# matiasrodlo/arxiv-rag

Measured on AMD Instinct MI355X. Metric: chunks embedded/sec + QPS@top-10, all-mpnet-base-v2 768-d, 1/2/4/8 MI355X, higher is better.
Workload: dtype bf16

## Files before the change

arxiv_rag_amd/_lib.py:

```python
from __future__ import annotations

import ctypes as C
import os
from pathlib import Path

_HERE = Path(__file__).resolve().parent
LIB_PATH = Path(os.environ.get("ARX_LIB", _HERE / "libarx_hip.so"))

K_CLASSES = ["search_groupmax", "gemm_qkv", "gemm_oproj", "gemm_fc1", "gemm_fc2", "attention",
             "layernorm", "embed", "pool", "search_select", "search_rescore", "gemm_raw"]


class EncoderConfigC(C.Structure):
    _fields_ = [(n, C.c_int32) for n in ("arch", "vocab_size", "hidden", "layers", "heads", "ffn", "max_pos",
                                         "pool", "pad_id", "rel_buckets", "rel_max_distance")] + [("ln_eps", C.c_float)]


class LayerWeightsC(C.Structure):
    _fields_ = [(n, C.c_void_p) for n in ("w_qkv", "b_qkv", "w_o", "b_o", "ln1_g", "ln1_b",
                                          "w_fc1", "b_fc1", "w_fc2", "b_fc2", "ln2_g", "ln2_b")]


class EncoderWeightsC(C.Structure):
    _fields_ = [(n, C.c_void_p) for n in ("word_emb", "pos_emb", "type_emb", "emb_ln_g", "emb_ln_b", "rel_bias")] \
               + [("layers", C.POINTER(LayerWeightsC))]


class TopkOptionsC(C.Structure):
    _fields_ = [("struct_bytes", C.c_int32), ("i8_max_queries", C.c_int32), ("max_row_norm", C.c_float), ("cu_limit", C.c_int32),
                ("flags", C.c_int32), ("debug_tau_mult", C.c_float), ("debug_drop_best", C.c_int32)]

    def __init__(self, **kw):
        super().__init__(**kw)
        self.struct_bytes = C.sizeof(TopkOptionsC)


class EncoderOptionsC(C.Structure):
    _fields_ = [("struct_bytes", C.c_int32), ("gemm_schedule", C.c_int32), ("attn_kernel", C.c_int32), ("flags", C.c_int32)]

    def __init__(self, **kw):
        super().__init__(**kw)
        self.struct_bytes = C.sizeof(EncoderOptionsC)


class PairHeadC(C.Structure):
    _fields_ = [("struct_bytes", C.c_int32), ("n_labels", C.c_int32)] \
               + [(n, C.c_void_p) for n in ("type_emb", "pooler_w", "pooler_b", "cls_w", "cls_b")]

    def __init__(self, **kw):
        super().__init__(**kw)
        self.struct_bytes = C.sizeof(PairHeadC)


class GemmEpilogueC(C.Structure):
    _fields_ = [("struct_bytes", C.c_int32), ("mode", C.c_int32), ("variant", C.c_int32), ("eps", C.c_float)] \
               + [(n, C.c_void_p) for n in ("bias", "resid", "a_mean", "a_rstd", "s_vec", "r_mean", "r_rstd", "r_gamma", "r_beta")] \
               + [("row_cap", C.c_int64), ("part_sum", C.c_void_p), ("part_sq", C.c_void_p), ("part_ld", C.c_int64),
                  ("out_mean", C.c_void_p), ("out_rstd", C.c_void_p), ("n_rows", C.c_void_p)]

    def __init__(self, **kw):
        super().__init__(**kw)
        self.struct_bytes = C.sizeof(GemmEpilogueC)


TOPK_NO_PERSISTENT, TOPK_SCAN_ONLY, TOPK_TAIL_ONLY, TOPK_NO_SINGLE_ROW_TAIL, TOPK_I8_CENTRE_QUERY = 1, 2, 4, 8, 16
GEMM_DEFAULT, GEMM_PER_TILE, GEMM_PERSISTENT, GEMM_2STAGE, GEMM_SPLIT_K, GEMM_TILE_128 = 89, 8, 9, 13, 70, 71
ATTN_TRANSPOSED, ATTN_RING, ATTN_RING16, ATTN_STAGED = 1, 2, 4, 8
ENC_EXPLICIT_LAYERNORM = 1


EXPORTS = {
    "arx_version": (C.c_int32, []),
    "arx_last_error": (C.c_char_p, []),
    "arx_build_info": (C.c_int32, []),
    "arx_mpnet_bucket": (C.c_int32, [C.c_int32, C.c_int32, C.c_int32]),
    "arx_encoder_workspace_bytes": (C.c_int64, [C.POINTER(EncoderConfigC), C.c_int32, C.c_int32]),
    "arx_encoder_create": (C.c_int32, [C.POINTER(EncoderConfigC), C.POINTER(EncoderWeightsC), C.c_int32, C.c_int32,
                                       C.POINTER(C.c_void_p)]),
    "arx_encoder_create_opt": (C.c_int32, [C.POINTER(EncoderConfigC), C.POINTER(EncoderWeightsC), C.c_int32, C.c_int32,
                                           C.POINTER(EncoderOptionsC), C.POINTER(C.c_void_p)]),
    "arx_encoder_destroy": (None, [C.c_void_p]),
    "arx_encoder_forward": (C.c_int32, [C.c_void_p, C.c_void_p, C.c_int32, C.c_void_p, C.c_int32, C.c_int32, C.c_int32,
                                        C.c_void_p, C.c_int64, C.c_void_p, C.c_int64, C.c_int32, C.c_void_p]),
    "arx_encoder_attention": (C.c_int32, [C.c_void_p, C.c_void_p, C.c_void_p, C.c_int32, C.c_int32, C.c_void_p, C.c_void_p]),
    "arx_encoder_set_tap": (C.c_int32, [C.c_void_p, C.c_int32]),
    "arx_encoder_set_low_latency": (C.c_int32, [C.c_void_p, C.c_int32]),
    "arx_encoder_debug_hidden": (C.c_int32, [C.c_void_p, C.c_int32, C.c_void_p, C.c_int32, C.c_void_p]),
    "arx_encoder_set_pair_head": (C.c_int32, [C.c_void_p, C.POINTER(PairHeadC)]),
    "arx_encoder_score_pairs": (C.c_int32, [C.c_void_p, C.c_void_p, C.c_int32, C.c_void_p, C.c_void_p, C.c_int32, C.c_int32, C.c_int32,
                                            C.c_void_p, C.c_int64, C.c_void_p]),
    "arx_encoder_debug_cls": (C.c_int32, [C.c_void_p, C.c_void_p, C.c_int32, C.c_void_p]),
    "arx_pair_head_forward": (C.c_int32, [C.c_void_p, C.c_int64, C.c_int32, C.c_int32, C.POINTER(PairHeadC), C.c_void_p, C.c_int64,
                                          C.c_void_p]),
    "arx_topk_workspace_bytes": (C.c_int64, [C.c_int64, C.c_int32, C.c_int32, C.c_int32]),
    "arx_topk_search": (C.c_int32, [C.c_void_p, C.c_int64, C.c_void_p, C.c_int32, C.c_int32, C.c_int32, C.c_void_p,
                                    C.c_void_p, C.c_int64, C.c_void_p, C.c_int64, C.c_void_p]),
    "arx_topk_i8_index_bytes": (C.c_int64, [C.c_int64, C.c_int32]),
    "arx_topk_i8_index_info": (C.c_int32, [C.c_void_p, C.c_int64, C.c_int32, C.POINTER(C.c_float), C.c_void_p]),
    "arx_topk_build_i8": (C.c_int32, [C.c_void_p, C.c_int64, C.c_int32, C.c_void_p, C.c_void_p]),
    "arx_topk_search_i8": (C.c_int32, [C.c_void_p, C.c_void_p, C.c_int64, C.c_void_p, C.c_int32, C.c_int32, C.c_int32, C.c_void_p,
                                       C.c_void_p, C.c_int64, C.c_void_p, C.c_int64, C.c_void_p]),
    "arx_topk_workspace_bytes_i8": (C.c_int64, [C.c_int64, C.c_int32, C.c_int32, C.c_int32]),
    "arx_topk_search_opt": (C.c_int32, [C.c_void_p, C.c_void_p, C.c_int64, C.c_void_p, C.c_int32, C.c_int32, C.c_int32, C.c_void_p,
                                        C.c_void_p, C.c_int64, C.c_void_p, C.c_int64, C.POINTER(TopkOptionsC), C.c_void_p]),
    "arx_rows_max_norm_f16": (C.c_int32, [C.c_void_p, C.c_int64, C.c_int32, C.c_void_p, C.c_void_p]),
    "arx_stream_create_cu_mask": (C.c_int32, [C.POINTER(C.c_uint32), C.c_int32, C.POINTER(C.c_void_p)]),
    "arx_stream_destroy": (C.c_int32, [C.c_void_p]),
    "arx_device_cu_count": (C.c_int32, []),
    "arx_debug_cu_census": (C.c_int32, [C.c_void_p, C.c_int32, C.c_int32, C.c_void_p]),
    "arx_topk_stats": (C.c_int32, [C.c_void_p, C.POINTER(C.c_int64), C.POINTER(C.c_int64), C.c_void_p]),
    "arx_topk_merge": (C.c_int32, [C.c_void_p, C.c_void_p, C.c_int32, C.c_int32, C.c_int32, C.c_void_p, C.c_void_p,
                                   C.c_void_p]),
    "arx_topk_filtered_workspace_bytes": (C.c_int64, [C.c_int64, C.c_int32, C.c_int32, C.c_int32]),
    "arx_topk_search_filtered": (C.c_int32, [C.c_void_p, C.c_int64, C.c_void_p, C.c_int64, C.c_void_p, C.c_int32, C.c_int32, C.c_int32,
                                             C.c_void_p, C.c_void_p, C.c_int64, C.c_float, C.c_void_p, C.c_int64, C.c_void_p]),
    "arx_topk_search_filtered_tuned": (C.c_int32, [C.c_void_p, C.c_int64, C.c_void_p, C.c_int64, C.c_void_p, C.c_int32, C.c_int32, C.c_int32,
                                                   C.c_void_p, C.c_void_p, C.c_int64, C.c_float, C.c_void_p, C.c_int64, C.c_int32, C.c_int32,
                                                   C.c_void_p]),
    "arx_topk_filtered_stats": (C.c_int32, [C.c_void_p, C.POINTER(C.c_int64), C.POINTER(C.c_int64), C.c_void_p]),
    "arx_topk_filtered_multi_workspace_bytes": (C.c_int64, [C.c_int64, C.c_int32, C.c_int32, C.c_int32, C.c_int32]),
    "arx_topk_search_filtered_multi": (C.c_int32, [C.c_void_p, C.c_int64, C.c_void_p, C.c_int32, C.c_void_p, C.c_void_p, C.c_void_p, C.c_int32,
                                                   C.c_int32, C.c_int32, C.c_void_p, C.c_void_p, C.c_int64, C.c_float, C.c_void_p, C.c_int64,
                                                   C.c_void_p]),
    "arx_topk_search_filtered_multi_tuned": (C.c_int32, [C.c_void_p, C.c_int64, C.c_void_p, C.c_int32, C.c_void_p, C.c_void_p, C.c_void_p,
                                                         C.c_int32, C.c_int32, C.c_int32, C.c_void_p, C.c_void_p, C.c_int64, C.c_float,
                                                         C.c_void_p, C.c_int64, C.c_int32, C.c_int32, C.c_void_p]),
    "arx_topk_filtered_multi_stats": (C.c_int32, [C.c_void_p, C.POINTER(C.c_int64), C.POINTER(C.c_int64), C.c_void_p]),
    "arx_topk_prefix_workspace_bytes": (C.c_int64, [C.c_int64, C.c_int32, C.c_int32, C.c_int32]),
    "arx_topk_search_prefix": (C.c_int32, [C.c_void_p, C.c_int64, C.c_void_p, C.c_void_p, C.c_int32, C.c_int32, C.c_int32, C.c_void_p,
                                           C.c_void_p, C.c_int64, C.c_float, C.c_void_p, C.c_int64, C.c_void_p]),
    "arx_topk_search_prefix_tuned": (C.c_int32, [C.c_void_p, C.c_int64, C.c_void_p, C.c_void_p, C.c_int32, C.c_int32, C.c_int32, C.c_void_p,
                                                 C.c_void_p, C.c_int64, C.c_float, C.c_void_p, C.c_int64, C.c_int32, C.c_int32, C.c_void_p]),
    "arx_topk_prefix_stats": (C.c_int32, [C.c_void_p, C.POINTER(C.c_int64), C.POINTER(C.c_int64), C.c_void_p]),
    "arx_topk_grouped_workspace_bytes": (C.c_int64, [C.c_int64, C.c_int32, C.c_int32, C.c_int32, C.c_int32]),
    "arx_topk_search_grouped": (C.c_int32, [C.c_void_p, C.c_int64, C.c_void_p, C.c_int64, C.c_void_p, C.c_int64, C.c_void_p, C.c_int32,
                                            C.c_int32, C.c_int32, C.c_int32, C.c_void_p, C.c_void_p, C.c_void_p, C.c_int64, C.c_float,
                                            C.c_void_p, C.c_int64, C.c_void_p]),
    "arx_topk_search_grouped_tuned": (C.c_int32, [C.c_void_p, C.c_int64, C.c_void_p, C.c_int64, C.c_void_p, C.c_int64, C.c_void_p, C.c_int32,
                                                  C.c_int32, C.c_int32, C.c_int32, C.c_void_p, C.c_void_p, C.c_void_p, C.c_int64, C.c_float,
                                                  C.c_void_p, C.c_int64, C.c_int32, C.c_int32, C.c_void_p]),
    "arx_topk_grouped_stats": (C.c_int32, [C.c_void_p, C.POINTER(C.c_int64), C.POINTER(C.c_int64), C.c_void_p]),
    "arx_group_runs_info": (C.c_int32, [C.c_void_p, C.c_int64, C.c_void_p, C.c_void_p]),
    "arx_range_workspace_bytes": (C.c_int64, [C.c_int64, C.c_int32, C.c_int32, C.c_int32]),
    "arx_range_search": (C.c_int32, [C.c_void_p, C.c_int64, C.c_void_p, C.c_int64, C.c_void_p, C.c_void_p, C.c_int32, C.c_int32, C.c_int32,
                                     C.c_void_p, C.c_void_p, C.c_void_p, C.c_int64, C.c_float, C.c_void_p, C.c_int64, C.c_void_p]),
    "arx_range_search_tuned": (C.c_int32, [C.c_void_p, C.c_int64, C.c_void_p, C.c_int64, C.c_void_p, C.c_void_p, C.c_int32, C.c_int32,
                                           C.c_int32, C.c_void_p, C.c_void_p, C.c_void_p, C.c_int64, C.c_float, C.c_void_p, C.c_int64,
                                           C.c_int32, C.c_int32, C.c_void_p]),
    "arx_range_stats": (C.c_int32, [C.c_void_p, C.POINTER(C.c_int64), C.POINTER(C.c_int64), C.c_void_p]),
    "arx_text_contains":(C.c_int32, [C.c_void_p, C.c_void_p, C.c_int64, C.c_void_p, C.c_void_p, C.c_int32, C.c_void_p, C.c_void_p]),
    "arx_bitmap_count": (C.c_int32, [C.c_void_p, C.c_int64, C.c_void_p, C.c_void_p]),
# ... 92 lines not shown
```

arxiv_rag_amd/csrc/arx_common.h:

```cpp
#pragma once
#include <hip/hip_runtime.h>
#include <stdint.h>
#include <stdio.h>
#include <string>

#include "../../include/arx.h"

typedef __bf16 bf16_t;
typedef _Float16 f16_t;
typedef __bf16 bf16x8 __attribute__((ext_vector_type(8)));
typedef __bf16 bf16x4 __attribute__((ext_vector_type(4)));
typedef _Float16 f16x8 __attribute__((ext_vector_type(8)));
typedef float f32x4 __attribute__((ext_vector_type(4)));
typedef float f32x16 __attribute__((ext_vector_type(16)));
typedef uint32_t u32x4 __attribute__((ext_vector_type(4)));
typedef uint32_t u32x2 __attribute__((ext_vector_type(2)));

void arx_set_error(const char* fmt, ...);
int arx_prof_begin(int cls, hipStream_t st);
void arx_prof_end(int cls, int token, hipStream_t st);
hipError_t arx_func_smem(const void* kernel, int bytes);
int arx_device_cus();
struct ProfScope {
    int cls, tok; hipStream_t st;
    ProfScope(int c, hipStream_t s) : cls(c), tok(arx_prof_begin(c, s)), st(s) {}
    ~ProfScope() { arx_prof_end(cls, tok, st); }
};

#define ARX_HIP_CHECK(expr)                                                              \
    do {                                                                                 \
        hipError_t _e = (expr);                                                          \
        if (_e != hipSuccess) {                                                          \
            arx_set_error("%s:%d: %s -> %s", __FILE__, __LINE__, #expr, hipGetErrorString(_e)); \
            return ARX_ERR_HIP;                                                          \
        }                                                                                \
    } while (0)

#define ARX_REQUIRE(cond, ...)                \
    do {                                      \
        if (!(cond)) {                        \
            arx_set_error(__VA_ARGS__);       \
            return ARX_ERR_ARG;               \
        }                                     \
    } while (0)

static inline int64_t round_up64(int64_t x, int64_t m) { return (x + m - 1) / m * m; }
static inline int cdiv(int64_t a, int64_t b) { return (int)((a + b - 1) / b); }

__device__ __forceinline__ float bf16_bits_to_f32(uint16_t b) { return __uint_as_float(((uint32_t)b) << 16); }

typedef __bf16 bf16x2 __attribute__((ext_vector_type(2)));
typedef float f32x2 __attribute__((ext_vector_type(2)));
__device__ __forceinline__ uint32_t pack_bf16x2(float lo, float hi) {
    const f32x2 f = {lo, hi};
    return __builtin_bit_cast(uint32_t, __builtin_convertvector(f, bf16x2));
}

__device__ __forceinline__ void unpack_bf16x2(uint32_t v, float& lo, float& hi) {
    lo = __uint_as_float(v << 16);
    hi = __uint_as_float(v & 0xffff0000u);
}

__device__ __forceinline__ float wave_sum(float v) {
#pragma unroll
    for (int o = 32; o > 0; o >>= 1) v += __shfl_xor(v, o);
    return v;
}
__device__ __forceinline__ float wave_max(float v) {
#pragma unroll
    for (int o = 32; o > 0; o >>= 1) v = fmaxf(v, __shfl_xor(v, o));
    return v;
}

__device__ __forceinline__ int xcd_remap(int bid, int nwg) {
    const int q = nwg >> 3, r = nwg & 7, xcd = bid & 7, idx = bid >> 3;
    const int base = (xcd < r) ? xcd * (q + 1) : r * (q + 1) + (xcd - r) * q;
    return base + idx;
}
```

arxiv_rag_amd/csrc/encoder.hip:

```cpp
#include <math.h>
#include <stdlib.h>
#include <string.h>

#include <mutex>
#include <vector>

#include "arx_common.h"
#include "encoder_kernels.h"
#include "gemm.h"
#include "gemm8.h"
#include "gemm_small.h"

extern "C" int32_t arx_mpnet_bucket(int32_t rel, int32_t num_buckets, int32_t max_distance) {
    int n = -rel;
    const int nb = num_buckets / 2;
    int ret = 0;
    if (n < 0) { ret = nb; n = -n; }
    const int max_exact = nb / 2;
    if (n < max_exact) return ret + n;
    int v = max_exact + (int)floor(log((double)n / max_exact) / log((double)max_distance / max_exact) * (nb - max_exact) + 1e-6);
    if (v > nb - 1) v = nb - 1;
    return ret + v;
}

struct arx_encoder {
    arx_encoder_config cfg;
    arx_encoder_weights w;
    std::vector<arx_layer_weights> layers;
    int max_tokens, max_seqs, tok_pad;
    char* ws = nullptr;
    int64_t ws_bytes = 0;
    int32_t* cu = nullptr;
    uint16_t *x = nullptr, *x1 = nullptr, *qkv = nullptr, *ctx = nullptr, *y = nullptr, *hbuf = nullptr;
    float* bias_tbl = nullptr;
    uint16_t* tap = nullptr;
    int tap_layer = -1;
    int ln_fold = 1;
    char* fold_ws = nullptr;
    std::vector<uint16_t*> wqkv_f, wfc1_f;
    std::vector<float*> s_qkv, c_qkv, s_fc1, c_fc1;
    float *st1_sum = nullptr, *st1_sq = nullptr, *st2_sum = nullptr, *st2_sq = nullptr;
    float *part_s = nullptr, *part_q = nullptr;
    int variant = ARX_GEMM_DEFAULT;
    int low_latency = 0;
    float* small_ws = nullptr;
    int attn_variant = ARX_ATTN_TRANSPOSED;
    int attn_dev_word = 0;
    unsigned long long* attn_stamps = nullptr;
    arx_pair_head pair{};
    int has_pair = 0;
    float* cls_ws = nullptr;
};

struct WsLayout {
    int64_t cu, x, x1, qkv, ctx, y, hbuf, bias, stats, total;
};
static WsLayout ws_layout(const arx_encoder_config& c, int max_tokens, int max_seqs) {
    const int64_t tp = round_up64(max_tokens, 256);
    WsLayout l;
    int64_t o = 0;
    auto take = [&](int64_t bytes) { int64_t r = o; o += round_up64(bytes, 256); return r; };
    l.cu = take((int64_t)(max_seqs + 1) * 4);
    l.x = take(tp * c.hidden * 2);
    l.x1 = take(tp * c.hidden * 2);
    l.qkv = take(tp * c.hidden * 3 * 2);
    l.ctx = take(tp * c.hidden * 2);
    l.y = take(tp * c.hidden * 2);
    l.hbuf = take(tp * c.ffn * 2);
    l.bias = take((int64_t)c.heads * ARX_BIAS_ROW * 4);
    l.stats = take(tp * 4 * 4 + 2 * (int64_t)(c.hidden / 64) * tp * 4);
    l.total = o;
    return l;
}

static int check_cfg(const arx_encoder_config* c) {
    ARX_REQUIRE(c != nullptr, "cfg is null");
    ARX_REQUIRE(c->arch == ARX_ARCH_MPNET || c->arch == ARX_ARCH_BERT, "unknown arch %d", c->arch);
    ARX_REQUIRE(c->hidden > 0 && c->hidden % 64 == 0 && c->hidden <= 1024, "hidden=%d must be a multiple of 64, <= 1024", c->hidden);
    ARX_REQUIRE(c->heads > 0 && c->hidden % c->heads == 0, "hidden %% heads != 0");
    const int dh = c->hidden / c->heads;
    ARX_REQUIRE(dh == 32 || dh == 64, "head_dim=%d unsupported (32 or 64)", dh);
    ARX_REQUIRE(c->ffn > 0 && c->ffn % 64 == 0, "ffn=%d must be a multiple of 64", c->ffn);
    ARX_REQUIRE(c->layers > 0 && c->vocab_size > 0 && c->max_pos > 0, "bad layers/vocab/max_pos");
    ARX_REQUIRE(c->pool == ARX_POOL_MEAN || c->pool == ARX_POOL_CLS, "unknown pool %d", c->pool);
    return ARX_OK;
}

extern "C" int64_t arx_encoder_workspace_bytes(const arx_encoder_config* cfg, int32_t max_tokens, int32_t max_seqs) {
    if (check_cfg(cfg) != ARX_OK || max_tokens <= 0 || max_seqs <= 0) return -1;
    return ws_layout(*cfg, max_tokens, max_seqs).total;
}

static int check_options(const arx_encoder_options* o) {
    if (!o) return ARX_OK;
    ARX_REQUIRE(o->struct_bytes == (int32_t)sizeof(arx_encoder_options), "arx_encoder_options: struct_bytes=%d, this library expects %d",
                o->struct_bytes, (int)sizeof(arx_encoder_options));
    const int g = o->gemm_schedule, a = o->attn_kernel;
    bool gemm_ok = g == 0 || g == ARX_GEMM_DEFAULT || g == ARX_GEMM_PER_TILE || g == ARX_GEMM_PERSISTENT || g == ARX_GEMM_2STAGE || g == ARX_GEMM_TILE_128;
    bool attn_ok = a == 0 || a == ARX_ATTN_TRANSPOSED || a == ARX_ATTN_STAGED;
#ifdef ARX_DEV_VARIANTS
    gemm_ok = gemm_ok || g == 1 || g == 2 || g == 3 || g == 4 || g == 15 || g == 33 || g == 34;
    attn_ok = attn_ok || a == ARX_ATTN_RING || a == ARX_ATTN_RING16;
#endif
    ARX_REQUIRE(gemm_ok, "arx_encoder_options.gemm_schedule=%d is not a whole-forward GEMM schedule of this build (ARX_GEMM_* in arx.h)", g);
    ARX_REQUIRE(attn_ok, "arx_encoder_options.attn_kernel=%d is not an attention kernel of this build (ARX_ATTN_* in arx.h)", a);
    ARX_REQUIRE((o->flags & ~ARX_ENC_EXPLICIT_LAYERNORM) == 0, "arx_encoder_options.flags=0x%x has unknown bits", o->flags);
    return ARX_OK;
}

extern "C" int32_t arx_encoder_create(const arx_encoder_config* cfg, const arx_encoder_weights* w, int32_t max_tokens,
                                      int32_t max_seqs, arx_encoder** out) {
    return arx_encoder_create_opt(cfg, w, max_tokens, max_seqs, nullptr, out);
}

extern "C" int32_t arx_encoder_create_opt(const arx_encoder_config* cfg, const arx_encoder_weights* w, int32_t max_tokens,
                                          int32_t max_seqs, const arx_encoder_options* opt, arx_encoder** out) {
    int rc = check_cfg(cfg);
    if (rc != ARX_OK) return rc;
    if ((rc = check_options(opt)) != ARX_OK) return rc;
    ARX_REQUIRE(w && out, "null weights/out");
    ARX_REQUIRE(max_tokens > 0 && max_seqs > 0, "max_tokens/max_seqs must be positive");
    ARX_REQUIRE(w->word_emb && w->pos_emb && w->emb_ln_g && w->emb_ln_b && w->layers, "missing embedding weights");
    ARX_REQUIRE(cfg->arch != ARX_ARCH_BERT || w->type_emb, "BERT needs type_emb");
    ARX_REQUIRE(cfg->arch != ARX_ARCH_MPNET || w->rel_bias, "MPNet needs rel_bias");
    for (int i = 0; i < cfg->layers; ++i) {
        const arx_layer_weights& L = w->layers[i];
        ARX_REQUIRE(L.w_qkv && L.b_qkv && L.w_o && L.b_o && L.ln1_g && L.ln1_b && L.w_fc1 && L.b_fc1 && L.w_fc2 &&
                        L.b_fc2 && L.ln2_g && L.ln2_b, "layer %d: missing weights", i);
    }
    arx_encoder* h = new arx_encoder();
    auto fail = [&](int code) {
        if (h->ws) (void)hipFree(h->ws);
        if (h->fold_ws) (void)hipFree(h->fold_ws);
        delete h;
        return code;
    };
    h->cfg = *cfg;
    h->w = *w;
    h->layers.assign(w->layers, w->layers + cfg->layers);
    h->w.layers = h->layers.data();
    h->max_tokens = max_tokens;
    h->max_seqs = max_seqs;
    h->tok_pad = (int)round_up64(max_tokens, 256);
    if (opt && opt->gemm_schedule) h->variant = opt->gemm_schedule;
    if (opt && opt->attn_kernel) h->attn_variant = opt->attn_kernel;
    h->ln_fold = !(opt && (opt->flags & ARX_ENC_EXPLICIT_LAYERNORM));
    const WsLayout l = ws_layout(*cfg, max_tokens, max_seqs);
    hipError_t he = hipMalloc((void**)&h->ws, l.total);
    if (he != hipSuccess) {
        arx_set_error("hipMalloc(%lld bytes workspace): %s", (long long)l.total, hipGetErrorString(he));
        h->ws = nullptr;
        return fail(ARX_ERR_HIP);
    }
    h->ws_bytes = l.total;
    (void)hipMemset(h->ws, 0, l.total);
    h->cu = (int32_t*)(h->ws + l.cu);
    h->x = (uint16_t*)(h->ws + l.x);
    h->x1 = (uint16_t*)(h->ws + l.x1);
    h->qkv = (uint16_t*)(h->ws + l.qkv);
    h->ctx = (uint16_t*)(h->ws + l.ctx);
    h->y = (uint16_t*)(h->ws + l.y);
    h->hbuf = (uint16_t*)(h->ws + l.hbuf);
    h->bias_tbl = (float*)(h->ws + l.bias);
    {
        const int64_t tp = round_up64(max_tokens, 256);
        float* st = (float*)(h->ws + l.stats);
        h->st1_sum = st; h->st1_sq = st + tp; h->st2_sum = st + 2 * tp; h->st2_sq = st + 3 * tp;
        h->part_s = st + 4 * tp; h->part_q = h->part_s + (int64_t)(cfg->hidden / 64) * tp;
    }
    if (h->ln_fold) {
        const int64_t H = cfg->hidden, F = cfg->ffn, Lc = cfg->layers;
        const int64_t per = round_up64(3 * H * H * 2, 256) + round_up64(F * H * 2, 256) + 2 * round_up64(3 * H * 4, 256) + 2 * round_up64(F * 4, 256);
        he = hipMalloc((void**)&h->fold_ws, per * Lc);
        if (he != hipSuccess) {
            arx_set_error("hipMalloc(folded weights): %s", hipGetErrorString(he));
            h->fold_ws = nullptr;
            return fail(ARX_ERR_HIP);
        }
        char* pws = h->fold_ws;
        auto takep = [&](int64_t bytes) { char* r = pws; pws += round_up64(bytes, 256); return r; };
        for (int i = 0; i < Lc; ++i) {
            const arx_layer_weights& L = h->layers[i];
            uint16_t* wq = (uint16_t*)takep(3 * H * H * 2); uint16_t* w1 = (uint16_t*)takep(F * H * 2);
            float* sq = (float*)takep(3 * H * 4); float* cq = (float*)takep(3 * H * 4);
            float* s1 = (float*)takep(F * 4); float* c1 = (float*)takep(F * 4);
            h->wqkv_f.push_back(wq); h->wfc1_f.push_back(w1);
            h->s_qkv.push_back(sq); h->c_qkv.push_back(cq); h->s_fc1.push_back(s1); h->c_fc1.push_back(c1);
            fold_ln_kernel<<<cdiv(F, 4), 256>>>((const uint16_t*)L.w_fc1, L.ln1_g, L.ln1_b, L.b_fc1, w1, s1, c1, (int)F, (int)H);
            if (i > 0) {
                const arx_layer_weights& P = h->layers[i - 1];
                fold_ln_kernel<<<cdiv(3 * H, 4), 256>>>((const uint16_t*)L.w_qkv, P.ln2_g, P.ln2_b, L.b_qkv, wq, sq, cq, (int)(3 * H), (int)H);
            }
        }
        he = hipDeviceSynchronize();
        if (he != hipSuccess) {
            arx_set_error("fold_ln_kernel: %s", hipGetErrorString(he));
            return fail(ARX_ERR_HIP);
        }
    }
    if (cfg->arch == ARX_ARCH_MPNET) {
        std::vector<float> rb((size_t)cfg->rel_buckets * cfg->heads);
        he = hipMemcpy(rb.data(), w->rel_bias, rb.size() * 4, hipMemcpyDeviceToHost);
        if (he != hipSuccess) {
            arx_set_error("copy rel_bias: %s", hipGetErrorString(he));
            return fail(ARX_ERR_HIP);
        }
        std::vector<float> tbl((size_t)cfg->heads * ARX_BIAS_ROW);
        const float log2e = 1.4426950408889634f;
        for (int d = -ARX_BIAS_CENTER; d <= ARX_BIAS_CENTER; ++d) {
            const int bk = arx_mpnet_bucket(d, cfg->rel_buckets, cfg->rel_max_distance);
            for (int hd = 0; hd < cfg->heads; ++hd)
                tbl[(size_t)hd * ARX_BIAS_ROW + d + ARX_BIAS_CENTER] = rb[(size_t)bk * cfg->heads + hd] * log2e;
        }
        he = hipMemcpy(h->bias_tbl, tbl.data(), tbl.size() * 4, hipMemcpyHostToDevice);
        if (he != hipSuccess) {
            arx_set_error("upload bias table: %s", hipGetErrorString(he));
            return fail(ARX_ERR_HIP);
        }
    }
    *out = h;
    return ARX_OK;
}

extern "C" void arx_encoder_destroy(arx_encoder* h) {
    if (!h) return;
    if (h->ws) (void)hipFree(h->ws);
    if (h->tap) (void)hipFree(h->tap);
    if (h->fold_ws) (void)hipFree(h->fold_ws);
    if (h->small_ws) (void)hipFree(h->small_ws);
    if (h->cls_ws) (void)hipFree(h->cls_ws);
    delete h;
}

extern "C" int32_t arx_encoder_set_low_latency(arx_encoder* h, int32_t on) {
    ARX_REQUIRE(h, "null handle");
    if (on && !h->small_ws) ARX_HIP_CHECK(hipMalloc((void**)&h->small_ws, ARX_SMALL_WS_BYTES));
    h->low_latency = on ? 1 : 0;
    return ARX_OK;
}

extern "C" int32_t arx_encoder_set_tap(arx_encoder* h, int32_t layer) {
    ARX_REQUIRE(h, "null handle");
    ARX_REQUIRE(layer >= -1 && layer <= h->cfg.layers, "tap layer out of range");
    if (layer >= 0 && !h->tap) ARX_HIP_CHECK(hipMalloc((void**)&h->tap, (int64_t)h->tok_pad * h->cfg.hidden * 2));
    h->tap_layer = layer;
    return ARX_OK;
}

extern "C" int32_t arx_encoder_debug_hidden(arx_encoder* h, int32_t , float* dst, int32_t n_tokens, void* stream) {
    ARX_REQUIRE(h && h->tap && dst, "no tap recorded");
    ARX_REQUIRE(n_tokens > 0 && n_tokens <= h->max_tokens, "n_tokens out of range");
    const int64_t n = (int64_t)n_tokens * h->cfg.hidden;
    bf16_to_f32_kernel<<<cdiv(n, 256), 256, 0, (hipStream_t)stream>>>(h->tap, dst, n);
    ARX_HIP_CHECK(hipGetLastError());
    return ARX_OK;
}

template <typename Kern>
static int launch_gemm_kernel(Kern kern, int smem, int threads, int BM, int BN, const uint16_t* A, int64_t lda,
                              const uint16_t* W, int64_t ldw, int M, int N, int K, const EpiParams& ep, hipStream_t st) {
    ARX_HIP_CHECK(arx_func_smem((const void*)kern, smem));
    const int tm = cdiv(M, BM), tn = cdiv(N, BN);
    kern<<<tm * tn, threads, smem, st>>>((const bf16_t*)A, lda, (const bf16_t*)W, ldw, M, N, K, tm, tn, ep);
    ARX_HIP_CHECK(hipGetLastError());
    return ARX_OK;
}

static bool fits_u32_offsets(int64_t M, int64_t lda, int64_t N, int64_t ldw, const EpiParams& ep) {
    return M * lda < (1ll << 31) && N * ldw < (1ll << 31) && M * ep.ldc < (1ll << 32) && (!ep.resid || M * ep.ldr < (1ll << 32));
}

template <int MODE>
int arx_launch_gemm(int variant, const uint16_t* A, int64_t lda, const uint16_t* W, int64_t ldw, int M, int N, int K,
                    const EpiParams& ep, hipStream_t st) {
    if (K % 64 != 0 || N % 8 != 0) {
        arx_set_error("gemm: K=%d must be a multiple of 64 and N=%d of 8", K, N);
        return ARX_ERR_ARG;
    }
    const bool wide = (N % 256 == 0);
    const bool wide8 = (N % 128 == 0 && N >= 256);
#ifdef ARX_DEV_VARIANTS
    if constexpr (MODE <= EPI_BIAS_RESID) {
        if (variant == 0) {
            if (wide) return launch_gemm_kernel(gemm_bf16_kernel<256, 256, 2, 4, true, MODE>, GemmMainloop<bf16_t, 256, 256, 2, 4, true>::SMEM_BYTES, 512, 256, 256, A, lda, W, ldw, M, N, K, ep, st);
            return launch_gemm_kernel(gemm_bf16_kernel<256, 128, 4, 2, true, MODE>, GemmMainloop<bf16_t, 256, 128, 4, 2, true>::SMEM_BYTES, 512, 256, 128, A, lda, W, ldw, M, N, K, ep, st);
        }
        if (variant == 4) {
            if (wide) return launch_gemm_kernel(gemm_bf16_kernel<256, 256, 2, 4, false, MODE>, GemmMainloop<bf16_t, 256, 256, 2, 4, false>::SMEM_BYTES, 512, 256, 256, A, lda, W, ldw, M, N, K, ep, st);
            return launch_gemm_kernel(gemm_bf16_kernel<256, 128, 4, 2, false, MODE>, GemmMainloop<bf16_t, 256, 128, 4, 2, false>::SMEM_BYTES, 512, 256, 128, A, lda, W, ldw, M, N, K, ep, st);
        }
    }
#endif
    if (variant == ARX_GEMM_TILE_128)
        return launch_gemm_kernel(gemm_v0e2_kernel<128, 128, 2, 2, MODE, 67>, GemmMainloop<bf16_t, 128, 128, 2, 2, true, 67>::SMEM_BYTES, 256, 128, 128, A, lda, W, ldw, M, N, K, ep, st);
    if (variant == ARX_GEMM_DEFAULT) variant = (K <= 1024) ? ARX_GEMM_PERSISTENT : ARX_GEMM_PER_TILE;
    if (variant == ARX_GEMM_PERSISTENT && (K / 64) % 2 != 0) variant = ARX_GEMM_PER_TILE;
    if ((variant == ARX_GEMM_PER_TILE || variant == ARX_GEMM_PERSISTENT) && wide8 && !fits_u32_offsets(M, lda, N, ldw, ep)) {
        static bool said = false;
        if (!said) {
            said = true;
            fprintf(stderr, "[arx] gemm M=%d N=%d K=%d: operand or output offsets exceed 32 bits, using the 2-stage kernel (64-bit offsets)\n", M, N, K);
        }
        variant = ARX_GEMM_2STAGE;
    }
    if (variant == ARX_GEMM_PERSISTENT && wide8) {
        auto kern = gemm_8phase_persistent_kernel<MODE>;
        ARX_HIP_CHECK(arx_func_smem((const void*)kern, Gemm8Phase<bf16_t, 0>::SMEM_BYTES));
        const int n_cu = arx_device_cus();
        const int tm = cdiv(M, 256), tn = cdiv(N, 256);
        int grid = TileWalk::grid(tm, tn) < n_cu ? TileWalk::grid(tm, tn) : n_cu;
        grid = grid / 8 * 8 > 0 ? grid / 8 * 8 : grid;
        kern<<<grid, 512, Gemm8Phase<bf16_t, 0>::SMEM_BYTES, st>>>((const bf16_t*)A, lda, (const bf16_t*)W, ldw, M, N, K, tm, tn, ep);
        ARX_HIP_CHECK(hipGetLastError());
        return ARX_OK;
    }
    if (variant == ARX_GEMM_PER_TILE && wide8) {
        auto kern = gemm_8phase_kernel<MODE>;
        ARX_HIP_CHECK(arx_func_smem((const void*)kern, Gemm8Phase<bf16_t, 0>::SMEM_BYTES));
        const int tm = cdiv(M, 256), tn = cdiv(N, 256);
        kern<<<TileWalk::grid(tm, tn), 512, Gemm8Phase<bf16_t, 0>::SMEM_BYTES, st>>>((const bf16_t*)A, lda, (const bf16_t*)W, ldw, M, N, K, tm, tn, ep);
        ARX_HIP_CHECK(hipGetLastError());
        return ARX_OK;
    }
#ifdef ARX_DEV_VARIANTS
    if (variant == 34 && wide)
        return launch_gemm_kernel(gemm_v0e2_kernel<256, 256, 2, 4, MODE, 64 + 4096>, GemmMainloop<bf16_t, 256, 256, 2, 4, true, 64 + 4096>::SMEM_BYTES, 512, 256, 256, A, lda, W, ldw, M, N, K, ep, st);
    if (variant == 33 && wide)
        return launch_gemm_kernel(gemm_a3w2_kernel<256, 256, 2, 4, MODE>, 3 * 256 * 128 + 2 * 256 * 128, 512, 256, 256, A, lda, W, ldw, M, N, K, ep, st);
    if (variant == 1) {
        if (wide) return launch_gemm_kernel(gemm_v0e2_kernel<256, 256, 2, 4, MODE>, GemmMainloop<bf16_t, 256, 256, 2, 4, true>::SMEM_BYTES, 512, 256, 256, A, lda, W, ldw, M, N, K, ep, st);
        return launch_gemm_kernel(gemm_v0e2_kernel<256, 128, 4, 2, MODE>, GemmMainloop<bf16_t, 256, 128, 4, 2, true>::SMEM_BYTES, 512, 256, 128, A, lda, W, ldw, M, N, K, ep, st);
    }
    if (variant == 15 && wide)
        return launch_gemm_kernel(gemm_v0e2_kernel<256, 256, 2, 4, MODE, 3>, GemmMainloop<bf16_t, 256, 256, 2, 4, true, 3>::SMEM_BYTES, 512, 256, 256, A, lda, W, ldw, M, N, K, ep, st);
    if (variant == 3 && wide)
        return launch_gemm_kernel(gemm_ring_kernel<256, 256, 2, 4, 4, MODE>, GemmRing<bf16_t, 256, 256, 2, 4, 4>::SMEM_BYTES, 512, 256, 256, A, lda, W, ldw, M, N, K, ep, st);
    if (variant == 2 || variant == 3)
        return launch_gemm_kernel(gemm_ring_kernel<256, 128, 2, 2, 3, MODE>, GemmRing<bf16_t, 256, 128, 2, 2, 3>::SMEM_BYTES, 256, 256, 128, A, lda, W, ldw, M, N, K, ep, st);
#endif
    if (!wide) return launch_gemm_kernel(gemm_v0e2_kernel<256, 128, 4, 2, MODE, 67>, GemmMainloop<bf16_t, 256, 128, 4, 2, true, 67>::SMEM_BYTES, 512, 256, 128, A, lda, W, ldw, M, N, K, ep, st);
    return launch_gemm_kernel(gemm_v0e2_kernel<256, 256, 2, 4, MODE, 67>, GemmMainloop<bf16_t, 256, 256, 2, 4, true, 67>::SMEM_BYTES, 512, 256, 256, A, lda, W, ldw, M, N, K, ep, st);
}

template <int MODE>
static int launch_gemm(int cls, int variant, const uint16_t* A, int64_t lda, const uint16_t* W, int64_t ldw, int M, int N, int K,
                       const EpiParams& ep, hipStream_t st, float* small_ws = nullptr) {
    ProfScope ps(cls, st);
    if (variant == ARX_GEMM_SPLIT_K) return launch_gemm_small<MODE>(A, lda, W, ldw, M, N, K, ep, small_ws, st);
#ifdef ARX_DEV_VARIANTS
    static const int dev_bw = getenv("ARX_DEV_BW") ? atoi(getenv("ARX_DEV_BW")) : 0;
    const char* stg = getenv("ARX_DEV_STAGGER");
    if (dev_bw || stg) {
        EpiParams e2 = ep; e2.dev_bw = dev_bw;
        if (stg) { int a = 0, b = 8, c = 0; sscanf(stg, "%d,%d,%d", &a, &b, &c); e2.dev_stagger = a; e2.dev_slots = b > 0 ? b : 8; e2.dev_store = c; }
        return arx_launch_gemm<MODE>(variant, A, lda, W, ldw, M, N, K, e2, st);
    }
#endif
    return arx_launch_gemm<MODE>(variant, A, lda, W, ldw, M, N, K, ep, st);
}

extern "C" int32_t arx_gemm_bf16(const void* A, const void* W, const float* bias, const void* resid, void* C, int32_t M,
                                 int32_t N, int32_t K, int32_t mode, int32_t variant, void* stream) {
    ARX_REQUIRE(A && W && bias && C, "null pointer argument");
    ARX_REQUIRE(M > 0 && N > 0 && K > 0, "bad sizes");
    ARX_REQUIRE(mode != EPI_BIAS_RESID || resid, "mode 2 needs resid");
    EpiParams ep{(uint16_t*)C, N, bias, (const uint16_t*)resid, N};
    hipStream_t st = (hipStream_t)stream;
#ifdef ARX_DEV_VARIANTS
    ep.dev_store = (variant / 100) % 10; ep.dev_bw = variant / 1000; variant %= 100;
    if (const char* stg = getenv("ARX_DEV_STAGGER")) { int a = 0, b = 8; sscanf(stg, "%d,%d", &a, &b); ep.dev_stagger = a; ep.dev_slots = b > 0 ? b : 8; }
#endif
#ifdef ARX_STAMP
    {
        static unsigned long long* d = nullptr;
        const int tiles = cdiv(M, 256) * cdiv(N, 256);
        if (!d) ARX_HIP_CHECK(hipMalloc(&d, (size_t)8 * 32 * 2 * 16384));
        if (getenv("ARX_STAMP_DUMP") && tiles <= 16384) {
            ep.stamps = d;
            int rc = ARX_ERR_ARG;
            if (mode == EPI_BIAS) rc = arx_launch_gemm<EPI_BIAS>(variant, (const uint16_t*)A, K, (const uint16_t*)W, K, M, N, K, ep, st);
            if (mode == EPI_BIAS_GELU) rc = arx_launch_gemm<EPI_BIAS_GELU>(variant, (const uint16_t*)A, K, (const uint16_t*)W, K, M, N, K, ep, st);
            if (mode == EPI_BIAS_RESID) rc = arx_launch_gemm<EPI_BIAS_RESID>(variant, (const uint16_t*)A, K, (const uint16_t*)W, K, M, N, K, ep, st);
            ARX_HIP_CHECK(hipStreamSynchronize(st));
            std::vector<unsigned long long> hbuf((size_t)tiles * 64);
            ARX_HIP_CHECK(hipMemcpy(hbuf.data(), d, hbuf.size() * 8, hipMemcpyDeviceToHost));
            double loop[2] = {0, 0}, epi[2] = {0, 0}, pro[2] = {0, 0}, x45[2] = {0, 0}, x67[2] = {0, 0};
            unsigned long long tmin = ~0ull, tmax = 0;
            for (int t = 0; t < tiles; ++t)
                for (int g = 0; g < 2; ++g) {
                    const unsigned long long* o = &hbuf[((size_t)t * 2 + g) * 32];
                    loop[g] += (double)(o[1] - o[3]); epi[g] += (double)(o[2] - o[1]); pro[g] += (double)(o[3] - o[0]);
                    if (variant == 9) { x45[g] += (double)(o[5] - o[4]); x67[g] += (double)(o[7] - o[6]); }
                    else x45[g] += (double)(o[4] - o[2]);
                    tmin = o[0] < tmin ? o[0] : tmin; tmax = o[2] > tmax ? o[2] : tmax;
                }
            if (variant == 9) {
                double gap = 0, period = 0; int n = 0;
                for (int t = 0; t + 256 < tiles; ++t) { const unsigned long long* a = &hbuf[(size_t)t * 64]; const unsigned long long* b = &hbuf[(size_t)(t + 256) * 64];
                    gap += (double)(b[0] - a[2]); period += (double)(b[0] - a[0]); ++n; }
                if (n) fprintf(stderr, "[stamp] persistent: g0 tile period %.0f clk, epilogue-end -> next loop start %.0f clk\n", period / n, gap / n);
            }
            if (const char* sf = getenv("ARX_STAMP_FILE")) {
                if (FILE* f = fopen(sf, "wb")) { fwrite(hbuf.data(), 8, hbuf.size(), f); fclose(f); }
// ... 63 lines not shown
    return ARX_OK;
}

#ifdef ARX_DEV_VARIANTS
template <int DH, bool HB, int NSLOT>
static int launch_attn_ring_cfg(arx_encoder* h, int n_seqs, int max_len, hipStream_t st) {
    auto kern = attention_ring_kernel<DH, HB, NSLOT>;
    const int C0 = (max_len + 31) & ~31;
    const int smem = AttnRing<DH, NSLOT>::total(C0, HB);
    ARX_HIP_CHECK(arx_func_smem((const void*)kern, smem));
    int G = arx_device_cus() / h->cfg.heads;
    G = G < 1 ? 1 : (G > n_seqs ? n_seqs : G);
    const float scale_log2e = 1.4426950408889634f / sqrtf((float)DH);
    ProfScope ps(ARX_K_ATTENTION, st);
    kern<<<G * h->cfg.heads, 512, smem, st>>>(h->qkv, h->ctx, h->cu, h->bias_tbl, h->cfg.hidden, n_seqs, C0, scale_log2e);
    ARX_HIP_CHECK(hipGetLastError());
    return ARX_OK;
}

template <bool HB>
static int launch_attn_ring16_cfg(arx_encoder* h, int n_seqs, int max_len, hipStream_t st) {
    auto kern = attention_ring16_kernel<HB>;
    const int C0 = (max_len + 31) & ~31;
    const int smem = AttnRing16<8>::total(C0, HB);
    ARX_HIP_CHECK(arx_func_smem((const void*)kern, smem));
    int G = arx_device_cus() / h->cfg.heads;
    G = G < 1 ? 1 : (G > n_seqs ? n_seqs : G);
    const float scale_log2e = 1.4426950408889634f / sqrtf(64.0f);
    ProfScope ps(ARX_K_ATTENTION, st);
    kern<<<G * h->cfg.heads, 1024, smem, st>>>(h->qkv, h->ctx, h->cu, h->bias_tbl, h->cfg.hidden, n_seqs, C0, scale_log2e);
    ARX_HIP_CHECK(hipGetLastError());
    return ARX_OK;
}

#endif

static int launch_attn(arx_encoder* h, int n_seqs, int max_len, hipStream_t st) {
    const int dh = h->cfg.hidden / h->cfg.heads;
    const bool hb = h->cfg.arch == ARX_ARCH_MPNET;
#ifdef ARX_DEV_VARIANTS
    if (h->attn_variant == ARX_ATTN_RING16 && dh == 64 && max_len > 128 && max_len <= 256)
        return hb ? launch_attn_ring16_cfg<true>(h, n_seqs, max_len, st) : launch_attn_ring16_cfg<false>(h, n_seqs, max_len, st);
    if (h->attn_variant == ARX_ATTN_RING && max_len > 128 && max_len <= 256) {
        if (dh == 64) return hb ? launch_attn_ring_cfg<64, true, 8>(h, n_seqs, max_len, st) : launch_attn_ring_cfg<64, false, 8>(h, n_seqs, max_len, st);
        return hb ? launch_attn_ring_cfg<32, true, 8>(h, n_seqs, max_len, st) : launch_attn_ring_cfg<32, false, 8>(h, n_seqs, max_len, st);
    }
#endif
    if (h->attn_variant != ARX_ATTN_STAGED) {
        const bool w8 = max_len > 128;
        if (dh == 64) {
            if (hb) return w8 ? launch_attn_tr_cfg<64, true, 8>(h, n_seqs, max_len, st) : launch_attn_tr_cfg<64, true, 4>(h, n_seqs, max_len, st);
            return w8 ? launch_attn_tr_cfg<64, false, 8>(h, n_seqs, max_len, st) : launch_attn_tr_cfg<64, false, 4>(h, n_seqs, max_len, st);
        }
        if (hb) return w8 ? launch_attn_tr_cfg<32, true, 8>(h, n_seqs, max_len, st) : launch_attn_tr_cfg<32, true, 4>(h, n_seqs, max_len, st);
        return w8 ? launch_attn_tr_cfg<32, false, 8>(h, n_seqs, max_len, st) : launch_attn_tr_cfg<32, false, 4>(h, n_seqs, max_len, st);
    }
    const bool big = max_len > 256;
    if (dh == 64) {
        if (hb) return big ? launch_attn_cfg<64, true, 8>(h, n_seqs, max_len, st) : launch_attn_cfg<64, true, 4>(h, n_seqs, max_len, st);
        return big ? launch_attn_cfg<64, false, 8>(h, n_seqs, max_len, st) : launch_attn_cfg<64, false, 4>(h, n_seqs, max_len, st);
    }
    if (hb) return big ? launch_attn_cfg<32, true, 8>(h, n_seqs, max_len, st) : launch_attn_cfg<32, true, 4>(h, n_seqs, max_len, st);
    return big ? launch_attn_cfg<32, false, 8>(h, n_seqs, max_len, st) : launch_attn_cfg<32, false, 4>(h, n_seqs, max_len, st);
}

extern "C" int32_t arx_encoder_attention(arx_encoder* h, const void* qkv, const int32_t* lens, int32_t n_seqs, int32_t max_len,
                                         void* ctx, void* stream) {
    ARX_REQUIRE(h && qkv && lens && ctx, "null pointer argument");
    ARX_REQUIRE(n_seqs > 0 && n_seqs <= h->max_seqs && max_len > 0 && max_len <= 512, "bad n_seqs/max_len");
    hipStream_t st = (hipStream_t)stream;
    scan_lens_kernel<<<1, 256, 0, st>>>(lens, h->cu, n_seqs);
    ARX_HIP_CHECK(hipGetLastError());
    uint16_t* q0 = h->qkv; uint16_t* c0 = h->ctx;
    h->qkv = (uint16_t*)qkv; h->ctx = (uint16_t*)ctx;
    const int rc = launch_attn(h, n_seqs, max_len, st);
    h->qkv = q0; h->ctx = c0;
    return rc;
}

static void launch_ln_finalize(int T, int nparts, const float* ps, const float* pq, int64_t ld, const int32_t* n_rows, float inv_h,
                               float eps, float* mean, float* rstd, hipStream_t st) {
    const int grid = cdiv(T, 256);
    switch (nparts) {
    case 6: ln_finalize_kernel<6><<<grid, 256, 0, st>>>(ps, pq, ld, nparts, n_rows, inv_h, eps, mean, rstd); break;
    case 12: ln_finalize_kernel<12><<<grid, 256, 0, st>>>(ps, pq, ld, nparts, n_rows, inv_h, eps, mean, rstd); break;
    case 16: ln_finalize_kernel<16><<<grid, 256, 0, st>>>(ps, pq, ld, nparts, n_rows, inv_h, eps, mean, rstd); break;
    default: ln_finalize_kernel<0><<<grid, 256, 0, st>>>(ps, pq, ld, nparts, n_rows, inv_h, eps, mean, rstd); break;
    }
}

template <int MODE>
static int gemm_ex_run(int variant, const uint16_t* A, const uint16_t* W, int M, int N, int K, const EpiParams& ep, const arx_gemm_epilogue* e,
                       hipStream_t st) {
    constexpr bool STATS = (MODE == EPI_RESID_STATS || MODE == EPI_LNRESID_STATS);
    int rc;
    if (variant == ARX_GEMM_SPLIT_K) {
        float* ws = nullptr;
        ARX_HIP_CHECK(hipMallocAsync((void**)&ws, ARX_SMALL_WS_BYTES, st));
        rc = launch_gemm<MODE>(ARX_K_GEMM_RAW, variant, A, K, W, K, M, N, K, ep, st, ws);
        (void)hipFreeAsync(ws, st);
        return rc;
    }
    if ((rc = launch_gemm<MODE>(ARX_K_GEMM_RAW, variant, A, K, W, K, M, N, K, ep, st)) != ARX_OK) return rc;
    if (STATS) {
        launch_ln_finalize(M, N / 64, e->part_sum, e->part_sq, e->part_ld, e->n_rows, ep.inv_h, ep.eps, e->out_mean, e->out_rstd, st);
        ARX_HIP_CHECK(hipGetLastError());
    }
    return ARX_OK;
}

extern "C" int32_t arx_gemm_bf16_ex(const void* A, const void* W, void* C, int32_t M, int32_t N, int32_t K, const arx_gemm_epilogue* e,
                                    void* stream) {
    ARX_REQUIRE(A && W && C && e, "null pointer argument");
    ARX_REQUIRE(e->struct_bytes == (int32_t)sizeof(arx_gemm_epilogue), "arx_gemm_epilogue: struct_bytes=%d, this library expects %d",
                e->struct_bytes, (int)sizeof(arx_gemm_epilogue));
    ARX_REQUIRE(M > 0 && N > 0 && K > 0, "bad sizes");
    ARX_REQUIRE(K % 64 == 0 && N % 8 == 0, "gemm: K=%d must be a multiple of 64 and N=%d of 8", K, N);
    const int mode = e->mode, variant = e->variant;
    ARX_REQUIRE(mode >= EPI_BIAS && mode <= EPI_LNRESID_STATS, "unknown gemm mode %d", mode);
    ARX_REQUIRE(variant == ARX_GEMM_DEFAULT || variant == ARX_GEMM_PER_TILE || variant == ARX_GEMM_PERSISTENT || variant == ARX_GEMM_2STAGE ||
                    variant == ARX_GEMM_SPLIT_K || variant == ARX_GEMM_TILE_128,
                "gemm variant %d is not a shipped schedule (89, 8, 9, 13, 70, 71)", variant);
    const bool ln_in = (mode == EPI_LN_BIAS || mode == EPI_LN_BIAS_GELU), stats = (mode == EPI_RESID_STATS || mode == EPI_LNRESID_STATS);
    const bool staged = (variant == ARX_GEMM_DEFAULT || variant == ARX_GEMM_PER_TILE || variant == ARX_GEMM_PERSISTENT);
    ARX_REQUIRE(e->bias, "mode %d needs bias", mode);
    ARX_REQUIRE(!(mode == EPI_BIAS_RESID || stats) || e->resid, "mode %d needs resid", mode);
    ARX_REQUIRE(!ln_in || (e->a_mean && e->a_rstd && e->s_vec), "mode %d needs a_mean, a_rstd and s_vec", mode);
    ARX_REQUIRE(mode != EPI_LNRESID_STATS || (e->r_mean && e->r_rstd && e->r_gamma && e->r_beta), "mode 6 needs r_mean, r_rstd, r_gamma and r_beta");
    if (ln_in || mode == EPI_LNRESID_STATS)
        ARX_REQUIRE(e->row_cap >= (staged ? round_up64(M, 256) : (int64_t)M),
                    "row_cap=%lld: the row vectors must be readable up to row %lld (M=%d%s)", (long long)e->row_cap,
                    (long long)(staged ? round_up64(M, 256) : (int64_t)M), M, staged ? " rounded up to 256: variants 89, 8, 9 stage whole tiles" : "");
    if (stats) {
        ARX_REQUIRE(N % 64 == 0, "statistics modes need N %% 64 == 0 (one partial per 64-column slice), N=%d", N);
        ARX_REQUIRE(e->out_mean && e->out_rstd, "mode %d needs out_mean and out_rstd", mode);
        if (variant != ARX_GEMM_SPLIT_K) ARX_REQUIRE(e->part_sum && e->part_sq && e->part_ld >= M && e->n_rows,
                                       "mode %d on a tile kernel needs part_sum, part_sq, part_ld >= M and n_rows", mode);
    }
    if (variant == ARX_GEMM_SPLIT_K) {
        ARX_REQUIRE(M <= ARX_SMALL_M && N % 64 == 0, "small-batch gemm: M=%d (<= %d) N=%d (%% 64)", M, ARX_SMALL_M, N);
        ARX_REQUIRE(!stats || N <= 1024, "small-batch gemm: statistics modes take N <= 1024, N=%d", N);
    }
    EpiParams ep{(uint16_t*)C, N, e->bias, (const uint16_t*)e->resid, N};
    ep.a_sum = e->a_mean; ep.a_sq = e->a_rstd; ep.s_vec = e->s_vec;
    ep.r_sum = e->r_mean; ep.r_sq = e->r_rstd; ep.r_gamma = e->r_gamma; ep.r_beta = e->r_beta;
    ep.o_sum = e->part_sum; ep.o_sq = e->part_sq; ep.o_ld = e->part_ld;
    ep.fin_mean = e->out_mean; ep.fin_rstd = e->out_rstd;
    ep.inv_h = 1.0f / (float)N; ep.eps = e->eps;
    hipStream_t st = (hipStream_t)stream;
    const uint16_t* a = (const uint16_t*)A; const uint16_t* w = (const uint16_t*)W;
    switch (mode) {
    case EPI_BIAS: return gemm_ex_run<EPI_BIAS>(variant, a, w, M, N, K, ep, e, st);
    case EPI_BIAS_GELU: return gemm_ex_run<EPI_BIAS_GELU>(variant, a, w, M, N, K, ep, e, st);
    case EPI_BIAS_RESID: return gemm_ex_run<EPI_BIAS_RESID>(variant, a, w, M, N, K, ep, e, st);
    case EPI_LN_BIAS: return gemm_ex_run<EPI_LN_BIAS>(variant, a, w, M, N, K, ep, e, st);
    case EPI_LN_BIAS_GELU: return gemm_ex_run<EPI_LN_BIAS_GELU>(variant, a, w, M, N, K, ep, e, st);
    case EPI_RESID_STATS: return gemm_ex_run<EPI_RESID_STATS>(variant, a, w, M, N, K, ep, e, st);
    default: return gemm_ex_run<EPI_LNRESID_STATS>(variant, a, w, M, N, K, ep, e, st);
    }
}

extern "C" int32_t arx_fold_ln(const void* W, const float* gamma, const float* beta, const float* bias, void* Wf, float* s, float* c,
                               int32_t N, int32_t K, void* stream) {
    ARX_REQUIRE(W && gamma && beta && bias && Wf && s && c, "null pointer argument");
    ARX_REQUIRE(N > 0 && K > 0, "bad sizes");
    fold_ln_kernel<<<cdiv(N, 4), 256, 0, (hipStream_t)stream>>>((const uint16_t*)W, gamma, beta, bias, (uint16_t*)Wf, s, c, (int)N, (int)K);
    ARX_HIP_CHECK(hipGetLastError());
    return ARX_OK;
}

static int32_t encoder_run(arx_encoder* h, const int32_t* ids, int32_t seq_stride, const int32_t* lens, const int32_t* seg_b,
                           int32_t n_seqs, int32_t max_len, int32_t total_tokens, float* out_f32,
                           int64_t out_stride, void* out_f16, int64_t out16_stride, int32_t normalize,
                           void* stream) {
    ARX_REQUIRE(h && ids && lens, "null handle/ids/lens");
    ARX_REQUIRE(out_f32 || out_f16, "no output buffer");
    ARX_REQUIRE(n_seqs > 0 && max_len > 0 && max_len <= 512, "n_seqs=%d max_len=%d (max_len must be in 1..512)", n_seqs, max_len);
    ARX_REQUIRE(seq_stride >= max_len, "seq_stride < max_len");
    ARX_REQUIRE(total_tokens > 0 && (int64_t)total_tokens <= (int64_t)n_seqs * max_len, "total_tokens out of range");
    if (n_seqs > h->max_seqs || total_tokens > h->max_tokens) {
        arx_set_error("batch (%d seqs, %d tokens) exceeds handle capacity (%d, %d)", n_seqs, total_tokens, h->max_seqs, h->max_tokens);
        return ARX_ERR_CAPACITY;
    }
    ARX_REQUIRE(!out_f32 || out_stride >= h->cfg.hidden, "out_stride < hidden");
    ARX_REQUIRE(!out_f16 || out16_stride >= h->cfg.hidden, "out16_stride < hidden");
    hipStream_t st = (hipStream_t)stream;
    const arx_encoder_config& c = h->cfg;
    const int H = c.hidden, F = c.ffn, T = total_tokens;
    int rc;

    scan_lens_kernel<<<1, 256, 0, st>>>(lens, h->cu, n_seqs);
    ARX_HIP_CHECK(hipGetLastError());
    {
        ProfScope ps(ARX_K_EMBED, st);
        dim3 grid(cdiv(max_len, 4), n_seqs);
        if (c.arch == ARX_ARCH_MPNET)
            embed_ln_kernel<ARX_ARCH_MPNET><<<grid, 256, 0, st>>>(ids, seq_stride, lens, h->cu, h->w.word_emb, h->w.pos_emb, nullptr,
                                                                  h->w.emb_ln_g, h->w.emb_ln_b, h->x, H, c.vocab_size, c.max_pos, c.pad_id, c.ln_eps);
        else if (seg_b)
            embed_ln_kernel<ARX_ARCH_BERT, true><<<grid, 256, 0, st>>>(ids, seq_stride, lens, h->cu, h->w.word_emb, h->w.pos_emb,
                                                                       h->pair.type_emb, h->w.emb_ln_g, h->w.emb_ln_b, h->x, H,
                                                                       c.vocab_size, c.max_pos, c.pad_id, c.ln_eps, seg_b);
        else
            embed_ln_kernel<ARX_ARCH_BERT><<<grid, 256, 0, st>>>(ids, seq_stride, lens, h->cu, h->w.word_emb, h->w.pos_emb, h->w.type_emb,
                                                                 h->w.emb_ln_g, h->w.emb_ln_b, h->x, H, c.vocab_size, c.max_pos, c.pad_id, c.ln_eps);
        ARX_HIP_CHECK(hipGetLastError());
    }
    const int ln_grid = cdiv(T, 4);
    const int64_t tp = round_up64(h->max_tokens, 256);
    if (!h->ln_fold) {
        auto tap = [&](int layer) -> int {
            if (h->tap_layer == layer && h->tap) ARX_HIP_CHECK(hipMemcpyAsync(h->tap, h->x, (int64_t)T * H * 2, hipMemcpyDeviceToDevice, st));
            return ARX_OK;
        };
        if ((rc = tap(0)) != ARX_OK) return rc;
        for (int li = 0; li < c.layers; ++li) {
            const arx_layer_weights& L = h->layers[li];
            EpiParams ep;
            ep = EpiParams{h->qkv, 3 * (int64_t)H, L.b_qkv, nullptr, 0};
            if ((rc = launch_gemm<EPI_BIAS>(ARX_K_GEMM_QKV, h->variant, h->x, H, (const uint16_t*)L.w_qkv, H, T, 3 * H, H, ep, st)) != ARX_OK) return rc;
            if ((rc = launch_attn(h, n_seqs, max_len, st)) != ARX_OK) return rc;
            ep = EpiParams{h->y, H, L.b_o, h->x, H};
            if ((rc = launch_gemm<EPI_BIAS_RESID>(ARX_K_GEMM_OPROJ, h->variant, h->ctx, H, (const uint16_t*)L.w_o, H, T, H, H, ep, st)) != ARX_OK) return rc;
            { ProfScope ps(ARX_K_LAYERNORM, st);
              layernorm_kernel<<<ln_grid, 256, 0, st>>>(h->y, h->x1, L.ln1_g, L.ln1_b, h->cu + n_seqs, H, c.ln_eps); }
            ARX_HIP_CHECK(hipGetLastError());
            ep = EpiParams{h->hbuf, F, L.b_fc1, nullptr, 0};
            if ((rc = launch_gemm<EPI_BIAS_GELU>(ARX_K_GEMM_FC1, h->variant, h->x1, H, (const uint16_t*)L.w_fc1, H, T, F, H, ep, st)) != ARX_OK) return rc;
            ep = EpiParams{h->y, H, L.b_fc2, h->x1, H};
            if ((rc = launch_gemm<EPI_BIAS_RESID>(ARX_K_GEMM_FC2, h->variant, h->hbuf, F, (const uint16_t*)L.w_fc2, F, T, H, F, ep, st)) != ARX_OK) return rc;
            { ProfScope ps(ARX_K_LAYERNORM, st);
              layernorm_kernel<<<ln_grid, 256, 0, st>>>(h->y, h->x, L.ln2_g, L.ln2_b, h->cu + n_seqs, H, c.ln_eps); }
            ARX_HIP_CHECK(hipGetLastError());
            if ((rc = tap(li + 1)) != ARX_OK) return rc;
        }
        ProfScope pps(ARX_K_POOL, st);
        pool_norm_kernel<<<n_seqs, 256, 0, st>>>(h->x, h->cu, H, c.pool, normalize, out_f32, out_stride, (f16_t*)out_f16, out16_stride,
                                                 nullptr, nullptr, nullptr, nullptr, 0.f);
        ARX_HIP_CHECK(hipGetLastError());
        return ARX_OK;
    }

    const float inv_h = 1.0f / (float)H;
    const int gv = !h->low_latency ? h->variant : (T <= ARX_SMALL_M ? ARX_GEMM_SPLIT_K : (T <= ARX_MEDIUM_M ? ARX_GEMM_TILE_128 : h->variant));
    if (h->tap_layer == 0 && h->tap) ARX_HIP_CHECK(hipMemcpyAsync(h->tap, h->x, (int64_t)T * H * 2, hipMemcpyDeviceToDevice, st));
    for (int li = 0; li < c.layers; ++li) {
        const arx_layer_weights& L = h->layers[li];
        EpiParams ep;
        if (li == 0) {
            ep = EpiParams{h->qkv, 3 * (int64_t)H, L.b_qkv, nullptr, 0};
            if ((rc = launch_gemm<EPI_BIAS>(ARX_K_GEMM_QKV, gv, h->x, H, (const uint16_t*)L.w_qkv, H, T, 3 * H, H, ep, st, h->small_ws)) != ARX_OK) return rc;
        } else {
            ep = EpiParams{h->qkv, 3 * (int64_t)H, h->c_qkv[li], nullptr, 0};
            ep.a_sum = h->st2_sum; ep.a_sq = h->st2_sq; ep.s_vec = h->s_qkv[li]; ep.inv_h = inv_h; ep.eps = c.ln_eps;
            if ((rc = launch_gemm<EPI_LN_BIAS>(ARX_K_GEMM_QKV, gv, h->x, H, h->wqkv_f[li], H, T, 3 * H, H, ep, st, h->small_ws)) != ARX_OK) return rc;
        }
        if ((rc = launch_attn(h, n_seqs, max_len, st)) != ARX_OK) return rc;
        ep = EpiParams{h->x1, H, L.b_o, h->x, H};
        ep.o_sum = h->part_s; ep.o_sq = h->part_q; ep.o_ld = tp; ep.inv_h = inv_h; ep.eps = c.ln_eps;
        ep.fin_mean = h->st1_sum; ep.fin_rstd = h->st1_sq;
        if (li == 0) {
            if ((rc = launch_gemm<EPI_RESID_STATS>(ARX_K_GEMM_OPROJ, gv, h->ctx, H, (const uint16_t*)L.w_o, H, T, H, H, ep, st, h->small_ws)) != ARX_OK) return rc;
        } else {
            const arx_layer_weights& P = h->layers[li - 1];
            ep.r_sum = h->st2_sum; ep.r_sq = h->st2_sq; ep.r_gamma = P.ln2_g; ep.r_beta = P.ln2_b;
            if ((rc = launch_gemm<EPI_LNRESID_STATS>(ARX_K_GEMM_OPROJ, gv, h->ctx, H, (const uint16_t*)L.w_o, H, T, H, H, ep, st, h->small_ws)) != ARX_OK) return rc;
        }
        if (gv != ARX_GEMM_SPLIT_K) { ProfScope ps(ARX_K_LAYERNORM, st);
          launch_ln_finalize(T, H / 64, h->part_s, h->part_q, tp, h->cu + n_seqs, inv_h, c.ln_eps, h->st1_sum, h->st1_sq, st); }
        ARX_HIP_CHECK(hipGetLastError());
        ep = EpiParams{h->hbuf, F, h->c_fc1[li], nullptr, 0};
        ep.a_sum = h->st1_sum; ep.a_sq = h->st1_sq; ep.s_vec = h->s_fc1[li]; ep.inv_h = inv_h; ep.eps = c.ln_eps;
        if ((rc = launch_gemm<EPI_LN_BIAS_GELU>(ARX_K_GEMM_FC1, gv, h->x1, H, h->wfc1_f[li], H, T, F, H, ep, st, h->small_ws)) != ARX_OK) return rc;
        ep = EpiParams{h->x, H, L.b_fc2, h->x1, H};
        ep.r_sum = h->st1_sum; ep.r_sq = h->st1_sq; ep.r_gamma = L.ln1_g; ep.r_beta = L.ln1_b;
        ep.o_sum = h->part_s; ep.o_sq = h->part_q; ep.o_ld = tp; ep.inv_h = inv_h; ep.eps = c.ln_eps;
        ep.fin_mean = h->st2_sum; ep.fin_rstd = h->st2_sq;
        if ((rc = launch_gemm<EPI_LNRESID_STATS>(ARX_K_GEMM_FC2, gv, h->hbuf, F, (const uint16_t*)L.w_fc2, F, T, H, F, ep, st, h->small_ws)) != ARX_OK) return rc;
        if (gv != ARX_GEMM_SPLIT_K) { ProfScope ps(ARX_K_LAYERNORM, st);
          launch_ln_finalize(T, H / 64, h->part_s, h->part_q, tp, h->cu + n_seqs, inv_h, c.ln_eps, h->st2_sum, h->st2_sq, st); }
        ARX_HIP_CHECK(hipGetLastError());
        if (h->tap_layer == li + 1 && h->tap) {
            layernorm_kernel<<<ln_grid, 256, 0, st>>>(h->x, h->tap, L.ln2_g, L.ln2_b, h->cu + n_seqs, H, c.ln_eps);
            ARX_HIP_CHECK(hipGetLastError());
        }
    }
    {
        const arx_layer_weights& Ll = h->layers[c.layers - 1];
        ProfScope pps(ARX_K_POOL, st);
        pool_norm_kernel<<<n_seqs, 256, 0, st>>>(h->x, h->cu, H, c.pool, normalize, out_f32, out_stride, (f16_t*)out_f16, out16_stride,
                                                 h->st2_sum, h->st2_sq, Ll.ln2_g, Ll.ln2_b, c.ln_eps);
        ARX_HIP_CHECK(hipGetLastError());
    }
    return ARX_OK;
}

extern "C" int32_t arx_encoder_forward(arx_encoder* h, const int32_t* ids, int32_t seq_stride, const int32_t* lens,
                                       int32_t n_seqs, int32_t max_len, int32_t total_tokens, float* out_f32,
                                       int64_t out_stride, void* out_f16, int64_t out16_stride, int32_t normalize,
                                       void* stream) {
    return encoder_run(h, ids, seq_stride, lens, nullptr, n_seqs, max_len, total_tokens, out_f32, out_stride, out_f16, out16_stride,
                       normalize, stream);
}

static int check_pair_head(const arx_pair_head* p, int hidden) {
    ARX_REQUIRE(p, "null pair head");
    ARX_REQUIRE(p->struct_bytes >= (int32_t)sizeof(arx_pair_head), "arx_pair_head.struct_bytes=%d < %d", p->struct_bytes,
                (int)sizeof(arx_pair_head));
    ARX_REQUIRE(p->n_labels >= 1 && p->n_labels <= 16, "n_labels=%d must be in 1..16", p->n_labels);
    ARX_REQUIRE(p->pooler_w && p->pooler_b && p->cls_w && p->cls_b, "pair head: missing pooler / classifier weights");
    ARX_REQUIRE(hidden > 0 && hidden <= 1024, "hidden=%d must be in 1..1024", hidden);
    return ARX_OK;
}

static int launch_pair_head(const float* cls, int64_t ld, int n, int H, const arx_pair_head& p, float* out, int64_t ld_out,
                            hipStream_t st) {
    const int smem = 2 * PH_ROWS * H * (int)sizeof(float);
    ARX_HIP_CHECK(arx_func_smem((const void*)pair_head_kernel, smem));
    pair_head_kernel<<<cdiv(n, PH_ROWS), 256, smem, st>>>(cls, ld, n, H, p.pooler_w, p.pooler_b, p.cls_w, p.cls_b, p.n_labels, out,
                                                            ld_out);
    ARX_HIP_CHECK(hipGetLastError());
    return ARX_OK;
}

extern "C" int32_t arx_encoder_set_pair_head(arx_encoder* h, const arx_pair_head* head) {
    ARX_REQUIRE(h, "null handle");
    ARX_REQUIRE(h->cfg.arch == ARX_ARCH_BERT && h->cfg.pool == ARX_POOL_CLS, "a pair head needs a BERT handle with CLS pooling");
    const int rc = check_pair_head(head, h->cfg.hidden);
    if (rc != ARX_OK) return rc;
    ARX_REQUIRE(head->type_emb, "pair head: missing token-type table");
    if (!h->cls_ws) ARX_HIP_CHECK(hipMalloc((void**)&h->cls_ws, (int64_t)h->max_seqs * h->cfg.hidden * sizeof(float)));
    h->pair = *head;
    h->has_pair = 1;
    return ARX_OK;
}

extern "C" int32_t arx_encoder_score_pairs(arx_encoder* h, const int32_t* ids, int32_t seq_stride, const int32_t* lens,
                                           const int32_t* seg_b, int32_t n_seqs, int32_t max_len, int32_t total_tokens,
                                           float* out_logits, int64_t out_stride, void* stream) {
    ARX_REQUIRE(h && out_logits, "null handle/out_logits");
    ARX_REQUIRE(h->has_pair, "no pair head set (arx_encoder_set_pair_head)");
    ARX_REQUIRE(out_stride >= h->pair.n_labels, "out_stride < n_labels");
    int rc = encoder_run(h, ids, seq_stride, lens, seg_b, n_seqs, max_len, total_tokens, h->cls_ws, h->cfg.hidden, nullptr, 0, 0,
                         stream);
    if (rc != ARX_OK) return rc;
    return launch_pair_head(h->cls_ws, h->cfg.hidden, n_seqs, h->cfg.hidden, h->pair, out_logits, out_stride, (hipStream_t)stream);
}

extern "C" int32_t arx_encoder_debug_cls(arx_encoder* h, float* dst, int32_t n, void* stream) {
    ARX_REQUIRE(h && h->cls_ws && dst, "no pair head set / null dst");
    ARX_REQUIRE(n > 0 && n <= h->max_seqs, "n out of range");
    ARX_HIP_CHECK(hipMemcpyAsync(dst, h->cls_ws, (int64_t)n * h->cfg.hidden * sizeof(float), hipMemcpyDeviceToDevice, (hipStream_t)stream));
    return ARX_OK;
}

extern "C" int32_t arx_pair_head_forward(const float* cls_rows, int64_t ld, int32_t n, int32_t hidden, const arx_pair_head* head,
                                         float* out_logits, int64_t out_stride, void* stream) {
    const int rc = check_pair_head(head, hidden);
    if (rc != ARX_OK) return rc;
    ARX_REQUIRE(n >= 0 && ld >= hidden && out_stride >= head->n_labels, "bad n / ld / out_stride");
    if (n == 0) return ARX_OK;
    ARX_REQUIRE(cls_rows && out_logits, "null cls_rows/out_logits");
    return launch_pair_head(cls_rows, ld, n, hidden, *head, out_logits, out_stride, (hipStream_t)stream);
// ... 35 lines not shown
```

arxiv_rag_amd/csrc/encoder_kernels.h:

```cpp
#pragma once
#include <type_traits>

#include "arx_common.h"

__global__ void scan_lens_kernel(const int32_t* __restrict__ lens, int32_t* __restrict__ cu, int n) {
    __shared__ int32_t part[1024];
    const int tid = threadIdx.x, nt = blockDim.x;
    const int per = (n + nt - 1) / nt;
    const int b0 = tid * per, b1 = min(n, b0 + per);
    int s = 0;
    for (int b = b0; b < b1; ++b) s += lens[b];
    part[tid] = s;
    __syncthreads();
    if (tid == 0) {
        int run = 0;
        for (int i = 0; i < nt; ++i) { int v = part[i]; part[i] = run; run += v; }
        cu[n] = run;
    }
    __syncthreads();
    int run = part[tid];
    for (int b = b0; b < b1; ++b) { cu[b] = run; run += lens[b]; }
}

template <int ARCH, bool SEG = false>
// ... 1206 lines not shown
    }
}

#endif

__global__ __launch_bounds__(256) void pool_norm_kernel(const uint16_t* __restrict__ x, const int32_t* __restrict__ cu,
                                                         int H, int pool_mode, int normalize,
                                                         float* __restrict__ out32, int64_t ld32,
                                                         f16_t* __restrict__ out16, int64_t ld16,
                                                         const float* __restrict__ ln_sum, const float* __restrict__ ln_sq,
                                                         const float* __restrict__ ln_g, const float* __restrict__ ln_b, float eps) {
    __shared__ float acc_s[4][1024];
    __shared__ float red[4];
    const int b = blockIdx.x, tid = threadIdx.x, lane = tid & 63, w = tid >> 6;
    const int t0 = cu[b], L = cu[b + 1] - t0;
    const int nch = H >> 3;
    float a[2][8];
#pragma unroll
    for (int c = 0; c < 2; ++c)
#pragma unroll
        for (int e = 0; e < 8; ++e) a[c][e] = 0.f;
    const int nrows = (pool_mode == ARX_POOL_CLS) ? (L > 0 ? 1 : 0) : L;
    for (int r = w; r < nrows; r += 4) {
        const uint16_t* in = x + (int64_t)(t0 + r) * H;
        float mu = 0.f, rs = 1.f;
        if (ln_sum) { mu = ln_sum[t0 + r]; rs = ln_sq[t0 + r]; }
#pragma unroll
        for (int c = 0; c < 2; ++c) {
            const int ch = lane + 64 * c;
            if (ch < nch) {
                const u32x4 q = *reinterpret_cast<const u32x4*>(in + ch * 8);
#pragma unroll
                for (int e = 0; e < 4; ++e) {
                    float lo, hi;
                    unpack_bf16x2(q[e], lo, hi);
                    a[c][2 * e] += (lo - mu) * rs; a[c][2 * e + 1] += (hi - mu) * rs;
                }
            }
        }
    }
#pragma unroll
    for (int c = 0; c < 2; ++c) {
        const int ch = lane + 64 * c;
        if (ch < nch)
#pragma unroll
            for (int e = 0; e < 8; ++e) acc_s[w][ch * 8 + e] = a[c][e];
    }
    __syncthreads();
    float v[4];
    float sq = 0.f;
    const float denom = (pool_mode == ARX_POOL_CLS) ? 1.0f : fmaxf((float)L, 1e-9f);
#pragma unroll
    for (int c = 0; c < 4; ++c) {
        const int col = tid + 256 * c;
        v[c] = 0.f;
        if (col < H) {
            v[c] = (acc_s[0][col] + acc_s[1][col] + acc_s[2][col] + acc_s[3][col]) / denom;
            if (ln_sum && L > 0) v[c] = fmaf(v[c], ln_g[col], ln_b[col]);
            sq += v[c] * v[c];
        }
    }
    sq = wave_sum(sq);
    if (lane == 0) red[w] = sq;
    __syncthreads();
    const float nrm = sqrtf(red[0] + red[1] + red[2] + red[3]);
    const float sc = normalize ? 1.0f / fmaxf(nrm, 1e-12f) : 1.0f;
#pragma unroll
    for (int c = 0; c < 4; ++c) {
        const int col = tid + 256 * c;
        if (col < H) {
            const float y = v[c] * sc;
            if (out32) out32[(int64_t)b * ld32 + col] = y;
            if (out16) out16[(int64_t)b * ld16 + col] = (f16_t)y;
        }
    }
}

template <int NP>
__global__ __launch_bounds__(256) void ln_finalize_kernel(const float* __restrict__ ps, const float* __restrict__ pq, int64_t ld,
                                                           int nparts, const int32_t* __restrict__ n_rows_ptr, float inv_h, float eps,
                                                           float* __restrict__ mean, float* __restrict__ rstd) {
    const int m = blockIdx.x * 256 + threadIdx.x;
    if (m >= *n_rows_ptr) return;
    float s = 0.f, q = 0.f;
    if constexpr (NP > 0) {
        float vs[NP], vq[NP];
#pragma unroll
        for (int p = 0; p < NP; ++p) { vs[p] = ps[p * ld + m]; vq[p] = pq[p * ld + m]; }
#pragma unroll
        for (int p = 0; p < NP; ++p) { s += vs[p]; q += vq[p]; }
    } else {
        for (int p = 0; p < nparts; ++p) { s += ps[p * ld + m]; q += pq[p * ld + m]; }
    }
    const float mu = s * inv_h;
    mean[m] = mu;
    rstd[m] = rsqrtf(fmaxf(q * inv_h - mu * mu, 0.f) + eps);
}

__global__ __launch_bounds__(256) void fold_ln_kernel(const uint16_t* __restrict__ W, const float* __restrict__ gamma,
                                                       const float* __restrict__ beta, const float* __restrict__ bias,
                                                       uint16_t* __restrict__ Wf, float* __restrict__ s, float* __restrict__ c,
                                                       int N, int K) {
    const int lane = threadIdx.x & 63;
    const int n = blockIdx.x * 4 + (threadIdx.x >> 6);
    if (n >= N) return;
    float ss = 0.f, cc = 0.f;
    for (int k = lane; k < K; k += 64) {
        const float w = bf16_bits_to_f32(W[(int64_t)n * K + k]);
        const bf16_t wf = (bf16_t)(w * gamma[k]);
        Wf[(int64_t)n * K + k] = __builtin_bit_cast(uint16_t, wf);
        ss += (float)wf;
        cc = fmaf(beta[k], w, cc);
    }
    ss = wave_sum(ss); cc = wave_sum(cc);
    if (lane == 0) { s[n] = ss; c[n] = bias[n] + cc; }
}

__global__ __launch_bounds__(256) void adjacent_cosine_kernel(const float* __restrict__ e, int64_t ld, int n, int D,
                                                               float* __restrict__ out) {
    const int lane = threadIdx.x & 63;
    const int i = blockIdx.x * 4 + (threadIdx.x >> 6);
    if (i + 1 >= n) return;
    const float* a = e + (int64_t)i * ld;
    const float* b = a + ld;
    float dot = 0.f, na = 0.f, nb = 0.f;
    for (int c = lane * 4; c < D; c += 256) {
        const f32x4 x = *reinterpret_cast<const f32x4*>(a + c), y = *reinterpret_cast<const f32x4*>(b + c);
#pragma unroll
        for (int r = 0; r < 4; ++r) { dot = fmaf(x[r], y[r], dot); na = fmaf(x[r], x[r], na); nb = fmaf(y[r], y[r], nb); }
    }
    dot = wave_sum(dot); na = wave_sum(na); nb = wave_sum(nb);
    if (lane == 0) out[i] = dot / (sqrtf(na) * sqrtf(nb));
}

constexpr int PH_ROWS = 16;
__global__ __launch_bounds__(256) void pair_head_kernel(const float* __restrict__ cls, int64_t ld, int n, int H,
                                                         const float* __restrict__ wp, const float* __restrict__ bp,
                                                         const float* __restrict__ wc, const float* __restrict__ bc, int n_labels,
                                                         float* __restrict__ out, int64_t ld_out) {
    extern __shared__ float ph_sm[];
    float* xs = ph_sm;
    float* ps = ph_sm + PH_ROWS * H;
    const int r0 = blockIdx.x * PH_ROWS, tid = threadIdx.x, lane = tid & 63, w = tid >> 6;
    const int nr = min(PH_ROWS, n - r0);
    for (int i = tid; i < PH_ROWS * H; i += 256) {
        const int r = i / H, k = i - r * H;
        xs[i] = r < nr ? cls[(int64_t)(r0 + r) * ld + k] : 0.f;
    }
    __syncthreads();
    for (int j = w; j < H; j += 4) {
        const float* wr = wp + (int64_t)j * H;
        float acc[PH_ROWS];
#pragma unroll
        for (int r = 0; r < PH_ROWS; ++r) acc[r] = 0.f;
        for (int k = lane; k < H; k += 64) {
            const float wv = wr[k];
#pragma unroll
            for (int r = 0; r < PH_ROWS; ++r) acc[r] = fmaf(wv, xs[r * H + k], acc[r]);
        }
        const float bj = bp[j];
#pragma unroll
        for (int r = 0; r < PH_ROWS; ++r) {
            const float v = wave_sum(acc[r]);
            if (lane == r) ps[r * H + j] = tanhf(v + bj);
        }
    }
    __syncthreads();
    for (int o = w; o < nr * n_labels; o += 4) {
        const int r = o / n_labels, l = o - r * n_labels;
        const float* wr = wc + (int64_t)l * H;
        float acc = 0.f;
        for (int k = lane; k < H; k += 64) acc = fmaf(wr[k], ps[r * H + k], acc);
        acc = wave_sum(acc);
        if (lane == 0) out[(int64_t)(r0 + r) * ld_out + l] = acc + bc[l];
    }
}

__global__ void bf16_to_f32_kernel(const uint16_t* __restrict__ src, float* __restrict__ dst, int64_t n) {
    const int64_t i = (int64_t)blockIdx.x * blockDim.x + threadIdx.x;
// ... 7 lines not shown
```

arxiv_rag_amd/csrc/epi3.h:

```cpp
#pragma once
#include "gemm.h"

struct EpiStage {
    enum { BIAS = 0, SVEC = 1, RGAMMA = 2, RBETA = 3, AMEAN = 4, ARSTD = 5, RMEAN = 6, RRSTD = 7, BYTES = 8 * 1024 };
};

template <int MODE>
__device__ __forceinline__ void epi_stage_issue(const EpiParams& p, int m0, int n0, char* stage, int wid, int lane, int N) {
    constexpr bool LN_IN = (MODE == EPI_LN_BIAS || MODE == EPI_LN_BIAS_GELU);
    constexpr bool LNR = (MODE == EPI_LNRESID_STATS);
    const int w = wid;
    const float* src = nullptr;
    if (w == EpiStage::BIAS) src = p.bias + n0;
    if constexpr (LN_IN) {
        if (w == EpiStage::SVEC) src = p.s_vec + n0;
        if (w == EpiStage::AMEAN) src = p.a_sum + m0;
        if (w == EpiStage::ARSTD) src = p.a_sq + m0;
    }
    if constexpr (LNR) {
        if (w == EpiStage::RGAMMA) src = p.r_gamma + n0;
        if (w == EpiStage::RBETA) src = p.r_beta + n0;
        if (w == EpiStage::RMEAN) src = p.r_sum + m0;
        if (w == EpiStage::RRSTD) src = p.r_sq + m0;
    }
    unsigned l = __builtin_amdgcn_mbcnt_hi(~0u, __builtin_amdgcn_mbcnt_lo(~0u, 0u));
    (void)lane;
    if (w < EpiStage::AMEAN && n0 + 256 > N) l &= 31;
    if (src) __builtin_amdgcn_global_load_lds((gbl_void_t*)(src + l * 4), (lds_void_t*)(stage + w * 1024), 16, 0, 0);
}

template <int MODE> struct EpiFullLine {
#if defined(ARX_FL_NONE)
    static constexpr bool value = false;
#else
    static constexpr bool value = true;
#endif
};
template <int MODE> struct EpiStoreNT {
#if defined(ARX_NT_NONE)
    static constexpr bool value = false;
#else
    static constexpr bool value = EpiFullLine<MODE>::value;
#endif
};

template <int MODE, bool CHECK, int DEPTH>
__device__ __forceinline__ void epilogue_store_v3_impl(const f32x4 (&acc)[4][8], const EpiParams& p, int m0, int n0, int wr, int wc,
                                                       int lane, int M, const char* stage) {
    constexpr int NI = 4, MI = 8, NS = (NI / 2) * MI;
    constexpr bool LN_IN = (MODE == EPI_LN_BIAS || MODE == EPI_LN_BIAS_GELU);
    constexpr bool STATS = (MODE == EPI_RESID_STATS || MODE == EPI_LNRESID_STATS);
    constexpr bool RESID = (MODE == EPI_BIAS_RESID || STATS);
    constexpr bool LNR = (MODE == EPI_LNRESID_STATS);
    constexpr bool FL = EpiFullLine<MODE>::value;
    const int mq = lane & 15, q = lane >> 4;
    const int m_base = m0 + wr * 128, n_base = n0 + wc * 64;
    const float* sf = reinterpret_cast<const float*>(stage);
    auto row_of = [&](int i) { int m = m_base + i * 16 + mq; if (CHECK) m = m < M ? m : M - 1; return m; };
    auto row_ok = [&](int i) { return !CHECK || (m_base + i * 16 + mq) < M; };
    auto col_of = [&](int jp) { return wc * 64 + jp * 32 + q * 8; };
    u32x4 rres[DEPTH];
    auto res_load = [&](int st) {
        const int i = st / (NI / 2), jp = st % (NI / 2);
        if (row_ok(i)) rres[st % DEPTH] = *reinterpret_cast<const u32x4*>(p.resid + (uint32_t)row_of(i) * (uint32_t)p.ldr + n0 + col_of(jp));
    };
    if constexpr (RESID) {
#pragma unroll
        for (int st = 0; st < DEPTH; ++st) res_load(st);
    }
    float st_s = 0.f, st_q = 0.f;
    f32x2 bb[4], ss[4], gg[4], ee[4];
    u32x4 opair[2];
#pragma unroll
    for (int st = 0; st < NS; ++st) {
        const int i = st / (NI / 2), jp = st % (NI / 2);
        const int cb = col_of(jp);
        {
            const f32x4 b0 = *reinterpret_cast<const f32x4*>(sf + EpiStage::BIAS * 256 + cb), b1 = *reinterpret_cast<const f32x4*>(sf + EpiStage::BIAS * 256 + cb + 4);
            bb[0] = f32x2{b0[0], b0[1]}; bb[1] = f32x2{b0[2], b0[3]}; bb[2] = f32x2{b1[0], b1[1]}; bb[3] = f32x2{b1[2], b1[3]};
            if constexpr (LN_IN) {
                const f32x4 s0 = *reinterpret_cast<const f32x4*>(sf + EpiStage::SVEC * 256 + cb), s1 = *reinterpret_cast<const f32x4*>(sf + EpiStage::SVEC * 256 + cb + 4);
                ss[0] = f32x2{s0[0], s0[1]}; ss[1] = f32x2{s0[2], s0[3]}; ss[2] = f32x2{s1[0], s1[1]}; ss[3] = f32x2{s1[2], s1[3]};
            }
            if constexpr (LNR) {
                const f32x4 g0 = *reinterpret_cast<const f32x4*>(sf + EpiStage::RGAMMA * 256 + cb), g1 = *reinterpret_cast<const f32x4*>(sf + EpiStage::RGAMMA * 256 + cb + 4);
                const f32x4 e0 = *reinterpret_cast<const f32x4*>(sf + EpiStage::RBETA * 256 + cb), e1 = *reinterpret_cast<const f32x4*>(sf + EpiStage::RBETA * 256 + cb + 4);
                gg[0] = f32x2{g0[0], g0[1]}; gg[1] = f32x2{g0[2], g0[3]}; gg[2] = f32x2{g1[0], g1[1]}; gg[3] = f32x2{g1[2], g1[3]};
                ee[0] = f32x2{e0[0], e0[1]}; ee[1] = f32x2{e0[2], e0[3]}; ee[2] = f32x2{e1[0], e1[1]}; ee[3] = f32x2{e1[2], e1[3]};
            }
        }
        const f32x4 lo = acc[2 * jp][i], hi = acc[2 * jp + 1][i];
        if (FL || row_ok(i)) {
            const int rb = wr * 128 + i * 16 + mq;
            f32x2 vv[4] = {f32x2{lo[0], lo[1]}, f32x2{lo[2], lo[3]}, f32x2{hi[0], hi[1]}, f32x2{hi[2], hi[3]}};
            if constexpr (LN_IN) {
                const float am = sf[EpiStage::AMEAN * 256 + rb], ar = sf[EpiStage::ARSTD * 256 + rb];
                const f32x2 nm = f32x2{-am, -am}, rs = f32x2{ar, ar};
#pragma unroll
                for (int pi = 0; pi < 4; ++pi) vv[pi] = rs * (nm * ss[pi] + vv[pi]) + bb[pi];
            } else {
#pragma unroll
                for (int pi = 0; pi < 4; ++pi) vv[pi] = vv[pi] + bb[pi];
            }
            if constexpr (MODE == EPI_BIAS_GELU || MODE == EPI_LN_BIAS_GELU) {
#pragma unroll
                for (int pi = 0; pi < 4; ++pi) vv[pi] = gelu_poly_pk(vv[pi]);
            }
            if constexpr (RESID) {
                const u32x4 rr = rres[st % DEPTH];
                float rm = 0.f, rsd = 1.f;
                if constexpr (LNR) { rm = sf[EpiStage::RMEAN * 256 + rb]; rsd = sf[EpiStage::RRSTD * 256 + rb]; }
#pragma unroll
                for (int pi = 0; pi < 4; ++pi) {
                    float r0, r1;
                    unpack_bf16x2(rr[pi], r0, r1);
                    f32x2 ra = f32x2{r0, r1};
                    if constexpr (LNR) ra = ((ra - f32x2{rm, rm}) * f32x2{rsd, rsd}) * gg[pi] + ee[pi];
                    vv[pi] = vv[pi] + ra;
                }
            }
            u32x4 o;
#pragma unroll
            for (int pi = 0; pi < 4; ++pi) o[pi] = pack_bf16x2(vv[pi].x, vv[pi].y);
            if constexpr (FL) {
              opair[jp] = o;
              if (jp == NI / 2 - 1) {
                const bool up = mq >= 8;
                u32x4 x = opair[0], y = opair[1];
#pragma unroll
                for (int r = 0; r < 4; ++r) {
                    x[r] = (uint32_t)__builtin_amdgcn_update_dpp((int)x[r], (int)opair[1][r], 0x128, 0xf, 0xc, false);
                    y[r] = (uint32_t)__builtin_amdgcn_update_dpp((int)y[r], (int)opair[0][r], 0x128, 0xf, 0x3, false);
                }
                const int cbs = col_of(up ? 1 : 0);
                const int rx = m_base + i * 16 + (mq & 7), ry = rx + 8;
                u32x4* dx = reinterpret_cast<u32x4*>(p.out + (uint32_t)rx * (uint32_t)p.ldc + n0 + cbs);
                u32x4* dy = reinterpret_cast<u32x4*>(p.out + (uint32_t)ry * (uint32_t)p.ldc + n0 + cbs);
#ifdef ARX_DEV_VARIANTS
                if (p.dev_store == 3) { asm volatile("" :: "v"(x), "v"(y), "v"(dx), "v"(dy)); if (p.ldc == 0x7fffffff) { *dx = x; *dy = y; } }
                else if (p.dev_store == 1) {
                    if (!CHECK || rx < M) asm volatile("global_store_dwordx4 %0, %1, off nt" :: "v"(dx), "v"(x) : "memory");
                    if (!CHECK || ry < M) asm volatile("global_store_dwordx4 %0, %1, off nt" :: "v"(dy), "v"(y) : "memory");
                }
                else
#endif
                if constexpr (EpiStoreNT<MODE>::value) {
                    if (!CHECK || rx < M) __builtin_nontemporal_store(x, dx);
                    if (!CHECK || ry < M) __builtin_nontemporal_store(y, dy);
                } else { if (!CHECK || rx < M) *dx = x; if (!CHECK || ry < M) *dy = y; }
              }
            } else {
                u32x4* dst = reinterpret_cast<u32x4*>(p.out + (uint32_t)row_of(i) * (uint32_t)p.ldc + n0 + cb);
#ifdef ARX_DEV_VARIANTS
                if (p.dev_store == 3) { asm volatile("" :: "v"(o), "v"(dst)); if (p.ldc == 0x7fffffff) *dst = o; }
                else if (p.dev_store == 1) __builtin_nontemporal_store(o, dst);
                else if (p.dev_store == 2) asm volatile("global_store_dwordx4 %0, %1, off sc1\n\ts_nop 1" :: "v"(dst), "v"(o) : "memory");
                else
#endif
                if constexpr (EpiStoreNT<MODE>::value) __builtin_nontemporal_store(o, dst);
                else *dst = o;
            }
            if constexpr (STATS) {
#pragma unroll
                for (int r = 0; r < 4; ++r) {
                    float x0, x1;
                    unpack_bf16x2(o[r], x0, x1);
                    st_s += x0 + x1;
                    st_q = fmaf(x0, x0, fmaf(x1, x1, st_q));
                }
            }
        }
        if constexpr (RESID) {
            if (st + DEPTH < NS) res_load(st + DEPTH);
        }
        if constexpr (STATS) {
            if (jp == NI / 2 - 1) {
                float a = st_s, b = st_q;
                a += __shfl_xor(a, 16); a += __shfl_xor(a, 32);
                b += __shfl_xor(b, 16); b += __shfl_xor(b, 32);
                const int m = m_base + i * 16 + mq;
                const int64_t part = n_base >> 6;
                if (q == 0 && m < M) { p.o_sum[part * p.o_ld + m] = a; p.o_sq[part * p.o_ld + m] = b; }
                st_s = 0.f; st_q = 0.f;
            }
        }
    }
}

template <int MODE, int DEPTH = 8>
__device__ __forceinline__ void epilogue_store_v3(const f32x4 (&acc)[4][8], const EpiParams& p, int m0, int n0, int wr, int wc,
                                                  int lane, int M, int N, const char* stage) {
    if (n0 + wc * 64 >= N) return;
    if (m0 + wr * 128 + 128 <= M) epilogue_store_v3_impl<MODE, false, DEPTH>(acc, p, m0, n0, wr, wc, lane, M, stage);
    else {
        epilogue_store_v3_impl<MODE, true, DEPTH>(acc, p, m0, n0, wr, wc, lane, M, stage);
        __builtin_amdgcn_s_waitcnt(0x0F70);
    }
}
```

arxiv_rag_amd/csrc/gemm.h:

```cpp
#pragma once
#include "arx_common.h"

template <typename T> struct Mfma;
template <> struct Mfma<bf16_t> {
    using vec = bf16x8;
    static __device__ __forceinline__ f32x4 mma(vec a, vec b, f32x4 c) {
        return __builtin_amdgcn_mfma_f32_16x16x32_bf16(a, b, c, 0, 0, 0);
    }
};
template <> struct Mfma<f16_t> {
    using vec = f16x8;
    static __device__ __forceinline__ f32x4 mma(vec a, vec b, f32x4 c) {
        return __builtin_amdgcn_mfma_f32_16x16x32_f16(a, b, c, 0, 0, 0);
    }
};

struct i8pair_t { uint16_t v; };
typedef int i32x4 __attribute__((ext_vector_type(4)));
template <> struct Mfma<i8pair_t> {
    using vec = i32x4;
    static __device__ __forceinline__ f32x4 mma(vec a, vec b, f32x4 c) {
        return __builtin_bit_cast(f32x4, __builtin_amdgcn_mfma_i32_16x16x64_i8(a, b, __builtin_bit_cast(i32x4, c), 0, 0, 0));
    }
};
// ... 81 lines not shown
                    for (int i = 0; i < MI; ++i) acc[j][i] = Mfma<T>::mma(wf[j], af[i], acc[j][i]);
                __builtin_amdgcn_s_setprio(0);
            };
            for (int kt = 0; kt < nk; ++kt) {
                const char* cur = smem + (kt & 1) * STAGE_BYTES;
                char* nxt = smem + ((kt + 1) & 1) * STAGE_BYTES;
                if (kt + 1 < nk) {
                    stage_issue<BM, NT, GLDS>(Ag, lda, m0, M - 1, kstep(kt + 1), nxt, tid, ra);
                    stage_issue<BN, NT, GLDS>(Wg, ldw, n0, N - 1, kstep(kt + 1), nxt + A_BYTES, tid, rw);
                }
                rd(cur, off0, af0, wf0);
                if (kt > 0) mm(af1, wf1);
                rd(cur, off1, af1, wf1);
                mm(af0, wf0);
                __syncthreads();
            }
            mm(af1, wf1);
            return;
        }
        for (int kt = 0; kt < nk; ++kt) {
            char* cur = smem + (kt & 1) * STAGE_BYTES;
            char* nxt = smem + ((kt + 1) & 1) * STAGE_BYTES;
            const bool late = (OPT & 1) && (__builtin_amdgcn_readfirstlane(wid) >= (WM * WN) / 2);
            if (kt + 1 < nk && !late) {
                stage_issue<BM, NT, GLDS>(Ag, lda, m0, M - 1, kstep(kt + 1), nxt, tid, ra);
                stage_issue<BN, NT, GLDS>(Wg, ldw, n0, N - 1, kstep(kt + 1), nxt + A_BYTES, tid, rw);
            }
            const char* As = cur + a_base;
            const char* Ws = cur + A_BYTES + w_base;
#pragma unroll
            for (int ks = 0; ks < 2; ++ks) {
                const int off = ks ? off1 : off0;
                vec af[MI], wf[NI];
#pragma unroll
                for (int i = 0; i < MI; ++i) af[i] = *reinterpret_cast<const vec*>(As + i * 2048 + off);
#pragma unroll
                for (int j = 0; j < NI; ++j) wf[j] = *reinterpret_cast<const vec*>(Ws + j * 2048 + off);
                if constexpr (OPT & 2) __builtin_amdgcn_s_setprio(1);
#pragma unroll
                for (int j = 0; j < NI; ++j)
#pragma unroll
                    for (int i = 0; i < MI; ++i) acc[j][i] = Mfma<T>::mma(wf[j], af[i], acc[j][i]);
                if constexpr (OPT & 2) __builtin_amdgcn_s_setprio(0);
                if (ks == 0 && late && kt + 1 < nk) {
                    stage_issue<BM, NT, GLDS>(Ag, lda, m0, M - 1, kstep(kt + 1), nxt, tid, ra);
                    stage_issue<BN, NT, GLDS>(Wg, ldw, n0, N - 1, kstep(kt + 1), nxt + A_BYTES, tid, rw);
                }
            }
            if constexpr (!GLDS) {
                if (kt + 1 < nk) {
                    stage_commit<BM, NT>(nxt, tid, ra);
                    stage_commit<BN, NT>(nxt + A_BYTES, tid, rw);
                }
            }
            __syncthreads();
        }
    }
};

__device__ __forceinline__ float gelu_erf(float x) { return 0.5f * x * (1.0f + erff(x * 0.70710678118654752f)); }

enum { EPI_BIAS = 0, EPI_BIAS_GELU = 1, EPI_BIAS_RESID = 2,
       EPI_LN_BIAS = 3,
       EPI_LN_BIAS_GELU = 4,
       EPI_RESID_STATS = 5,
       EPI_LNRESID_STATS = 6 };

struct EpiParams {
    uint16_t* out;
    int64_t ldc;
    const float* bias;
    const uint16_t* resid;
    int64_t ldr;
    const float* a_sum = nullptr;
    const float* a_sq = nullptr;
    const float* s_vec = nullptr;
    const float* r_sum = nullptr;
    const float* r_sq = nullptr;
    const float* r_gamma = nullptr;
    const float* r_beta = nullptr;
    float* o_sum = nullptr;
    float* o_sq = nullptr;
    int64_t o_ld = 0;
    float inv_h = 0.f, eps = 0.f;
    float* fin_mean = nullptr;
    float* fin_rstd = nullptr;
#ifdef ARX_DEV_VARIANTS
    int dev_store = 0;
    int dev_bw = 0;
    int dev_stagger = 0, dev_slots = 8;
#endif
#ifdef ARX_STAMP
    unsigned long long* stamps = nullptr;
#endif
};



template <int MODE, int NI, int MI>
__device__ __forceinline__ void epilogue_store(const f32x4 (&acc)[NI][MI], const EpiParams& p, int m_base, int n_base,
                                               int lane, int M, int N) {
    const int mq = lane & 15, nq = (lane >> 4) * 4;
#pragma unroll
    for (int j = 0; j < NI; ++j) {
        const int n = n_base + j * 16 + nq;
        if (n >= N) continue;
        const f32x4 b = *reinterpret_cast<const f32x4*>(p.bias + n);
#pragma unroll
        for (int i = 0; i < MI; ++i) {
            const int m = m_base + i * 16 + mq;
            if (m >= M) continue;
            float v0 = acc[j][i][0] + b[0], v1 = acc[j][i][1] + b[1];
            float v2 = acc[j][i][2] + b[2], v3 = acc[j][i][3] + b[3];
            if constexpr (MODE == EPI_BIAS_GELU) {
                v0 = gelu_erf(v0); v1 = gelu_erf(v1); v2 = gelu_erf(v2); v3 = gelu_erf(v3);
            }
            if constexpr (MODE == EPI_BIAS_RESID) {
                const u32x2 r = *reinterpret_cast<const u32x2*>(p.resid + (int64_t)m * p.ldr + n);
                float r0, r1, r2, r3;
                unpack_bf16x2(r[0], r0, r1); unpack_bf16x2(r[1], r2, r3);
                v0 += r0; v1 += r1; v2 += r2; v3 += r3;
            }
            u32x2 o;
            o[0] = pack_bf16x2(v0, v1); o[1] = pack_bf16x2(v2, v3);
            *reinterpret_cast<u32x2*>(p.out + (int64_t)m * p.ldc + n) = o;
        }
    }
}

template <int BM, int BN, int WM, int WN, bool GLDS, int MODE>
__global__ __launch_bounds__(WM * WN * 64) void gemm_bf16_kernel(const bf16_t* __restrict__ A, int64_t lda,
                                                                   const bf16_t* __restrict__ W, int64_t ldw,
                                                                   int M, int N, int K, int tiles_m, int tiles_n,
                                                                   EpiParams ep) {
    using ML = GemmMainloop<bf16_t, BM, BN, WM, WN, GLDS>;
    extern __shared__ __attribute__((aligned(16))) char smem[];
    const int t = xcd_remap(blockIdx.x, tiles_m * tiles_n);
    const int tile_m = t / tiles_n, tile_n = t % tiles_n;
    const int m0 = tile_m * BM, n0 = tile_n * BN;
    f32x4 acc[ML::NI][ML::MI];
    ML::run(A, lda, M, W, ldw, N, K, m0, n0, smem, acc);
    const int lane = threadIdx.x & 63, wid = threadIdx.x >> 6;
    epilogue_store<MODE, ML::NI, ML::MI>(acc, ep, m0 + (wid / WN) * ML::TM, n0 + (wid % WN) * ML::TN, lane, M, N);
}

template <int ROWS, int NT>
__device__ __forceinline__ void ring_stage(const uint16_t* __restrict__ G, int64_t ld, int row0, int row_max, int k0,
                                           char* tile, int tid) {
    constexpr int IT = ROWS * 4 / NT;
    static_assert(ROWS * 4 % NT == 0, "half-tile rows must fill whole passes");
#pragma unroll
    for (int it = 0; it < IT; ++it) {
        const int cid = it * NT + tid;
        const int row = cid >> 2, pc = cid & 3;
        const int c = pc ^ ((4 - ((row >> 2) & 3)) & 3);
        int grow = row0 + row;
        grow = grow < row_max ? grow : row_max;
        const uint16_t* src = G + (int64_t)grow * ld + k0 + c * 8;
        char* dst = tile + (it * NT + (tid & ~63)) * 16;
        __builtin_amdgcn_global_load_lds((gbl_void_t*)src, (lds_void_t*)dst, 16, 0, 0);
    }
}

template <int N> __device__ __forceinline__ void wait_vmcnt() {
    if constexpr (N == 0) asm volatile("s_waitcnt vmcnt(0)" ::: "memory");
    else if constexpr (N == 2) asm volatile("s_waitcnt vmcnt(2)" ::: "memory");
    else if constexpr (N == 3) asm volatile("s_waitcnt vmcnt(3)" ::: "memory");
    else if constexpr (N == 4) asm volatile("s_waitcnt vmcnt(4)" ::: "memory");
    else if constexpr (N == 6) asm volatile("s_waitcnt vmcnt(6)" ::: "memory");
    else if constexpr (N == 8) asm volatile("s_waitcnt vmcnt(8)" ::: "memory");
    else if constexpr (N == 9) asm volatile("s_waitcnt vmcnt(9)" ::: "memory");
    else if constexpr (N == 12) asm volatile("s_waitcnt vmcnt(12)" ::: "memory");
    else if constexpr (N == 16) asm volatile("s_waitcnt vmcnt(16)" ::: "memory");
    else if constexpr (N == 18) asm volatile("s_waitcnt vmcnt(18)" ::: "memory");
    else asm volatile("s_waitcnt vmcnt(%0)" :: "n"(N) : "memory");
}

template <typename T, int BM, int BN, int WM, int WN, int SLOTS, int OPT = 0>
struct GemmRing {
    static constexpr int NT = WM * WN * 64;
// ... 338 lines not shown
```

arxiv_rag_amd/csrc/gemm8.h:

```cpp
#pragma once
#include "gemm.h"
#include "epi3.h"

#ifdef ARX_STAMP
#define g_stamp1 stamp1_ref
#endif

struct TileWalk {
    int tiles_m, tiles_n, bw;
    __device__ __forceinline__ TileWalk(int tm, int tn, int K, int bw_override = 0) : tiles_m(tm), tiles_n(tn) {
        if (bw_override > 0) { bw = bw_override < tn ? bw_override : tn; return; }
        const int w_tile = 512 * K;
        const int total = tn * w_tile;
        bw = tn;
        if (total > (4 << 20) && K <= 1024) {
            const int nb = (total + (12 << 18) / 5 * 4 - 1) / ((12 << 18) / 5 * 4);
            bw = (tn + nb - 1) / nb;
        }
    }
    static int grid(int tm, int tn) { return 8 * ((tm + 7) / 8) * tn; }
    __device__ __forceinline__ bool coords(int id, int& tile_m, int& tile_n) const {
        const int x = id & 7;
        int L = id >> 3;
        const int pq = tiles_m >> 3, pr = tiles_m & 7;
        const int panels = pq + (x < pr ? 1 : 0), m_lo = x * pq + (x < pr ? x : pr);
        if (L >= panels * tiles_n) return false;
        int b = 0, w = bw < tiles_n ? bw : tiles_n;
        while (L >= panels * w) { L -= panels * w; ++b; w = tiles_n - b * bw; w = w < bw ? w : bw; }
        const int q = L / w;
        tile_m = m_lo + q; tile_n = b * bw + (L - q * w);
        return true;
    }
};
__device__ __forceinline__ int b_slice_col(int rho) { return ((rho & 15) >> 2) * 8 + (rho >> 4) * 4 + (rho & 3); }

template <typename T, int KROT, bool PERM = false>
struct Gemm8Phase {
    static constexpr int BM = 256, BN = 256, NT = 512, MI = 8, NI = 4;
    static constexpr int HALF_BYTES = 128 * 128, BUF_BYTES = 4 * HALF_BYTES, STAGE_OFF = 2 * BUF_BYTES;
#ifdef ARX_STAMP
    static constexpr int KT_STAMP_OFF = STAGE_OFF + 2 * EpiStage::BYTES;
    static constexpr int SMEM_BYTES = KT_STAMP_OFF + 256;
#else
    static constexpr int SMEM_BYTES = STAGE_OFF + 2 * EpiStage::BYTES;
#endif
    using vec = typename Mfma<T>::vec;

    static __device__ __forceinline__ void fence() { asm volatile("" ::: "memory"); }
    static __device__ __forceinline__ void bar() {
        fence(); __builtin_amdgcn_s_barrier(); fence();
    }

    static __device__ __forceinline__ void run(const T* __restrict__ A, int64_t lda, int M, const T* __restrict__ W,
                                               int64_t ldw, int N, int K, int m0, int n0, char* smem,
                                               f32x4 (&acc)[NI][MI], int koff
#ifdef ARX_STAMP
                                               , unsigned long long& stamp1_ref
#endif
                                               ) {
        const int tid = threadIdx.x, lane = tid & 63, wid = __builtin_amdgcn_readfirstlane(tid >> 6);
        const int wr = wid >> 2, wc = wid & 3;
        const uint16_t* Ag = reinterpret_cast<const uint16_t*>(A);
        const uint16_t* Wg = reinterpret_cast<const uint16_t*>(W);
#pragma unroll
        for (int j = 0; j < NI; ++j)
#pragma unroll
            for (int i = 0; i < MI; ++i) acc[j][i] = f32x4{0.f, 0.f, 0.f, 0.f};

        uint32_t aoff[2][2], boff[2][2];
#pragma unroll
        for (int it = 0; it < 2; ++it) {
            const int cid = it * NT + tid, r = cid >> 3, c = (cid & 7) ^ ((r >> 1) & 7);
#pragma unroll
            for (int h = 0; h < 2; ++h) {
                int gm = m0 + (r >> 6) * 128 + h * 64 + (r & 63);
                gm = gm < M ? gm : M - 1;
                aoff[h][it] = ((uint32_t)gm * (uint32_t)lda + c * 8) * 2u;
                int gn = n0 + (r >> 5) * 64 + h * 32 + (PERM ? b_slice_col(r & 31) : (r & 31));
                gn = gn < N ? gn : N - 1;
                boff[h][it] = ((uint32_t)gn * (uint32_t)ldw + c * 8) * 2u;
            }
        }
        const int nk = K >> 6;
        koff = koff % nk;
        auto kcol = [&](int kt) { int k = kt + koff; return (k >= nk ? k - nk : k) << 6; };
        char* const wave_dst = smem + wid * 1024;
        const __amdgpu_buffer_rsrc_t rsA = __builtin_amdgcn_make_buffer_rsrc((void*)Ag, 0, 0xffffffff, 0x00020000);
        const __amdgpu_buffer_rsrc_t rsW = __builtin_amdgcn_make_buffer_rsrc((void*)Wg, 0, 0xffffffff, 0x00020000);
        auto issue_a = [&](int h, int kt, int buf) {
            const int kb = kcol(kt) * 2;
            char* dst = wave_dst + buf * BUF_BYTES + h * HALF_BYTES;
            __builtin_amdgcn_raw_ptr_buffer_load_lds(rsA, (lds_void_t*)dst, 16, aoff[h][0], kb, 0, 0);
            __builtin_amdgcn_raw_ptr_buffer_load_lds(rsA, (lds_void_t*)(dst + 8192), 16, aoff[h][1], kb, 0, 0);
        };
        auto issue_b = [&](int g, int kt, int buf) {
            const int kb = kcol(kt) * 2;
            char* dst = wave_dst + buf * BUF_BYTES + (2 + g) * HALF_BYTES;
            __builtin_amdgcn_raw_ptr_buffer_load_lds(rsW, (lds_void_t*)dst, 16, boff[g][0], kb, 0, 0);
            __builtin_amdgcn_raw_ptr_buffer_load_lds(rsW, (lds_void_t*)(dst + 8192), 16, boff[g][1], kb, 0, 0);
        };

        const int frow = lane & 15, fq = lane >> 4, sw = (lane >> 1) & 7;
        const int fo0 = frow * 128 + (((0 + fq) ^ sw) << 4), fo1 = frow * 128 + (((4 + fq) ^ sw) << 4);
        const int a_row = wr * 64 * 128, b_row = wc * 32 * 128;

        vec af[4][2], wf0[2][2], wf1[2][2];
        auto read_a = [&](const char* buf, int h) {
            const char* p = buf + h * HALF_BYTES + a_row;
#pragma unroll
            for (int i = 0; i < 4; ++i) {
                af[i][0] = *reinterpret_cast<const vec*>(p + i * 2048 + fo0);
                af[i][1] = *reinterpret_cast<const vec*>(p + i * 2048 + fo1);
            }
        };
        auto read_b = [&](const char* buf, int g, vec (&wf)[2][2]) {
            const char* p = buf + (2 + g) * HALF_BYTES + b_row;
#pragma unroll
            for (int j = 0; j < 2; ++j) {
                wf[j][0] = *reinterpret_cast<const vec*>(p + j * 2048 + fo0);
                wf[j][1] = *reinterpret_cast<const vec*>(p + j * 2048 + fo1);
            }
        };
        auto quad = [&](int h, int g, const vec (&wf)[2][2]) {
            __builtin_amdgcn_s_setprio(1);
#pragma unroll
            for (int ks = 0; ks < 2; ++ks)
#pragma unroll
                for (int j = 0; j < 2; ++j)
#pragma unroll
                    for (int i = 0; i < 4; ++i)
                        acc[g * 2 + j][h * 4 + i] = Mfma<T>::mma(wf[j][ks], af[i][ks], acc[g * 2 + j][h * 4 + i]);
            __builtin_amdgcn_s_setprio(0);
        };

        issue_b(0, 0, 0); issue_a(0, 0, 0); issue_b(1, 0, 0); issue_a(1, 0, 0);
        if (nk > 1) {
            issue_b(0, 1, 1); issue_a(0, 1, 1); issue_b(1, 1, 1);
            wait_vmcnt<6>();
        } else {
            wait_vmcnt<0>();
        }
        bar();
#ifdef ARX_STAMP
        g_stamp1 = __builtin_readcyclecounter();
#endif
        if (wr == 1) bar();

        for (int kt = 0; kt < nk; ++kt) {
            const int b = kt & 1;
            const char* cur = smem + b * BUF_BYTES;
            const bool more1 = kt + 1 < nk, more2 = kt + 2 < nk;
            read_b(cur, 0, wf0);
            __builtin_amdgcn_sched_barrier(0);
            read_a(cur, 0);
            if (more1) issue_a(1, kt + 1, b ^ 1);
            asm volatile("s_waitcnt lgkmcnt(8)" ::: "memory");
            bar();
            asm volatile("s_waitcnt lgkmcnt(0)" ::: "memory");
            quad(0, 0, wf0);
            bar();
            read_b(cur, 1, wf1);
            if (more2) issue_b(0, kt + 2, b);
            bar();
            asm volatile("s_waitcnt lgkmcnt(0)" ::: "memory");
            quad(0, 1, wf1);
            bar();
            read_a(cur, 1);
            if (more2) issue_a(0, kt + 2, b);
            bar();
            asm volatile("s_waitcnt lgkmcnt(0)" ::: "memory");
            quad(1, 1, wf1);
            bar();
            if (more2) { issue_b(1, kt + 2, b); wait_vmcnt<6>(); }
            else wait_vmcnt<0>();
            bar();
            quad(1, 0, wf0);
            if (more1 || wr == 0) bar();
        }
    }
};

template <int MODE, int KROT = 0>
__global__ __launch_bounds__(512) void gemm_8phase_kernel(const bf16_t* __restrict__ A, int64_t lda,
                                                           const bf16_t* __restrict__ W, int64_t ldw,
                                                           int M, int N, int K, int tiles_m, int tiles_n, EpiParams ep) {
    using ML = Gemm8Phase<bf16_t, KROT, true>;
    extern __shared__ __attribute__((aligned(16))) char smem[];
#ifdef ARX_DEV_VARIANTS
    const TileWalk walk(tiles_m, tiles_n, K, ep.dev_bw);
#else
    const TileWalk walk(tiles_m, tiles_n, K);
#endif
    int tile_m, tile_n;
    if (!walk.coords(blockIdx.x, tile_m, tile_n)) return;
    const int m0 = tile_m * 256, n0 = tile_n * 256;
    f32x4 acc[ML::NI][ML::MI];
#ifdef ARX_STAMP
    const unsigned long long ts0 = __builtin_readcyclecounter();
#endif
    epi_stage_issue<MODE>(ep, m0, n0, smem + ML::STAGE_OFF, __builtin_amdgcn_readfirstlane(threadIdx.x >> 6), threadIdx.x & 63, N);
#ifdef ARX_STAMP
    unsigned long long ts1 = 0;
    ML::run(A, lda, M, W, ldw, N, K, m0, n0, smem, acc, tile_n * KROT, ts1);
#else
    ML::run(A, lda, M, W, ldw, N, K, m0, n0, smem, acc, tile_n * KROT);
#endif
    const int lane = threadIdx.x & 63, wid = __builtin_amdgcn_readfirstlane(threadIdx.x >> 6);
#ifdef ARX_STAMP
    const unsigned long long ts2 = __builtin_readcyclecounter();
#endif
    epilogue_store_v3<MODE>(acc, ep, m0, n0, wid >> 2, wid & 3, lane, M, N, smem + ML::STAGE_OFF);
#ifdef ARX_STAMP
    const unsigned long long ts3 = __builtin_readcyclecounter();
    asm volatile("s_waitcnt vmcnt(0)" ::: "memory");
    const unsigned long long ts4 = __builtin_readcyclecounter();
    if (ep.stamps && (threadIdx.x == 0 || threadIdx.x == 256)) {
        unsigned long long* o = ep.stamps + ((size_t)blockIdx.x * 2 + (threadIdx.x >> 8)) * 32;
        o[0] = ts0; o[1] = ts2; o[2] = ts3;
        o[3] = ts1; o[4] = ts4; o[5] = 0; o[6] = 0; o[7] = 0;
    }
#endif
}

template <typename T, typename Pol>
__device__ __forceinline__ void gemm8_persistent_body(const T* __restrict__ A, int64_t lda, const T* __restrict__ W, int64_t ldw,
                                                      int M, int N, int K, const Pol& pol, char* smem) {
    using ML = Gemm8Phase<T, 0>;
    using vec = typename ML::vec;
    constexpr int HALF_BYTES = ML::HALF_BYTES, BUF_BYTES = ML::BUF_BYTES;
    const int tid = threadIdx.x, lane = tid & 63, wid = __builtin_amdgcn_readfirstlane(tid >> 6);
    const int wr = wid >> 2, wc = wid & 3;
    const uint16_t* Ag = reinterpret_cast<const uint16_t*>(A);
    const uint16_t* Wg = reinterpret_cast<const uint16_t*>(W);
    const int stride = gridDim.x, nk = K >> 6;
    auto kcol = [&](int kt, int ko) { int k = kt + ko; return (k >= nk ? k - nk : k) << 6; };

    uint32_t aoff[2][2], boff[2][2];
    auto set_aoff = [&](int h, int m0) {
#pragma unroll
        for (int it = 0; it < 2; ++it) {
            const int cid = it * 512 + tid, r = cid >> 3, c = (cid & 7) ^ ((r >> 1) & 7);
            int gm = m0 + (r >> 6) * 128 + h * 64 + (r & 63);
            gm = gm < M ? gm : M - 1;
            aoff[h][it] = ((uint32_t)gm * (uint32_t)lda + c * 8) * 2u;
        }
    };
    auto set_boff = [&](int g, int n0) {
#pragma unroll
        for (int it = 0; it < 2; ++it) {
            const int cid = it * 512 + tid, r = cid >> 3, c = (cid & 7) ^ ((r >> 1) & 7);
            int gn = n0 + (r >> 5) * 64 + g * 32 + (Pol::PERMUTE_B ? b_slice_col(r & 31) : (r & 31));
            gn = gn < N ? gn : N - 1;
            if constexpr (Pol::REBASE_W) gn -= n0;
            boff[g][it] = ((uint32_t)gn * (uint32_t)ldw + c * 8) * 2u;
        }
    };
    char* const wave_dst = smem + wid * 1024;
    const __amdgpu_buffer_rsrc_t rsA = __builtin_amdgcn_make_buffer_rsrc((void*)Ag, 0, 0xffffffff, 0x00020000);
    auto w_rsrc = [&](int n0) {
        return __builtin_amdgcn_make_buffer_rsrc((void*)(Wg + (Pol::REBASE_W ? (int64_t)n0 * ldw : (int64_t)0)), 0, 0xffffffff, 0x00020000);
    };
    __amdgpu_buffer_rsrc_t rsW = w_rsrc(0);
    auto issue_a = [&](int h, int kc, int buf) {
        char* dst = wave_dst + buf * BUF_BYTES + h * HALF_BYTES;
        __builtin_amdgcn_raw_ptr_buffer_load_lds(rsA, (lds_void_t*)dst, 16, aoff[h][0], kc * 2, 0, 0);
        __builtin_amdgcn_raw_ptr_buffer_load_lds(rsA, (lds_void_t*)(dst + 8192), 16, aoff[h][1], kc * 2, 0, 0);
    };
    auto issue_b = [&](int g, int kc, int buf) {
        char* dst = wave_dst + buf * BUF_BYTES + (2 + g) * HALF_BYTES;
        __builtin_amdgcn_raw_ptr_buffer_load_lds(rsW, (lds_void_t*)dst, 16, boff[g][0], kc * 2, 0, 0);
        __builtin_amdgcn_raw_ptr_buffer_load_lds(rsW, (lds_void_t*)(dst + 8192), 16, boff[g][1], kc * 2, 0, 0);
    };
    const int frow = lane & 15, fq = lane >> 4, sw = (lane >> 1) & 7;
    const int fo0 = frow * 128 + (((0 + fq) ^ sw) << 4), fo1 = frow * 128 + (((4 + fq) ^ sw) << 4);
    const int a_row = wr * 64 * 128, b_row = wc * 32 * 128;

    f32x4 acc[4][8];
    vec af[4][2], wf0[2][2], wf1[2][2];
    auto read_a = [&](const char* buf, int h) {
        const char* p = buf + h * HALF_BYTES + a_row;
#pragma unroll
        for (int i = 0; i < 4; ++i) {
            af[i][0] = *reinterpret_cast<const vec*>(p + i * 2048 + fo0);
            af[i][1] = *reinterpret_cast<const vec*>(p + i * 2048 + fo1);
        }
    };
    auto read_b = [&](const char* buf, int g, vec (&wf)[2][2]) {
        const char* p = buf + (2 + g) * HALF_BYTES + b_row;
#pragma unroll
        for (int j = 0; j < 2; ++j) {
            wf[j][0] = *reinterpret_cast<const vec*>(p + j * 2048 + fo0);
            wf[j][1] = *reinterpret_cast<const vec*>(p + j * 2048 + fo1);
        }
    };
// ... 43 lines not shown
            const char* cur = smem + b * BUF_BYTES;
            const bool more1 = kt + 1 < nk, more2 = kt + 2 < nk;
            const bool go1 = more1 || has_next, go2 = more2 || has_next;
            const int kc1 = more1 ? kcol(kt + 1, ko) : kcol(0, kon);
            const int kc2 = more2 ? kcol(kt + 2, ko) : kcol(kt + 2 - nk, kon);
#ifdef ARX_STAMP
            if (kt < 16 && (tid & 255) == 0) *reinterpret_cast<volatile unsigned long long*>(smem + ML::KT_STAMP_OFF + (tid >> 8) * 128 + kt * 8) = __builtin_readcyclecounter();
#endif
            read_b(cur, 0, wf0);
            __builtin_amdgcn_sched_barrier(0);
            read_a(cur, 0);
            if (kt == nk - 1 && has_next)
                pol.stage_issue(m0n, n0n, smem + ML::STAGE_OFF + (sbuf ^ 1) * EpiStage::BYTES, wid, lane);
            if (!more1 && has_next) {
                if (edge) { asm volatile("" : "+s"(m0n)); set_aoff(1, m0n); }
                else { aoff[1][0] += d_a; aoff[1][1] += d_a; }
            }
            if (go1) issue_a(1, kc1, b ^ 1);
            asm volatile("s_waitcnt lgkmcnt(8)" ::: "memory");
            ML::bar();
            asm volatile("s_waitcnt lgkmcnt(0)" ::: "memory");
            quad(0, 0, wf0);
            ML::bar();
            read_b(cur, 1, wf1);
            if (kt == nk - 2 && has_next) {
                if constexpr (Pol::REBASE_W) {
                    rsW = w_rsrc(n0n);
                    if (nclamp) { asm volatile("" : "+s"(n0n)); set_boff(0, n0n); set_boff(1, n0n); }
                } else {
                    if (nclamp) { asm volatile("" : "+s"(n0n)); set_boff(0, n0n); set_boff(1, n0n); }
                    else { boff[0][0] += d_b; boff[0][1] += d_b; boff[1][0] += d_b; boff[1][1] += d_b; }
                }
                if (edge) { asm volatile("" : "+s"(m0n)); set_aoff(0, m0n); }
                else { aoff[0][0] += d_a; aoff[0][1] += d_a; }
            }
            if (go2) issue_b(0, kc2, b);
            ML::bar();
            asm volatile("s_waitcnt lgkmcnt(0)" ::: "memory");
            quad(0, 1, wf1);
            ML::bar();
            read_a(cur, 1);
            if (go2) issue_a(0, kc2, b);
            ML::bar();
            asm volatile("s_waitcnt lgkmcnt(0)" ::: "memory");
            quad(1, 1, wf1);
            ML::bar();
#ifdef ARX_STAMP
#ifdef ARX_STAMP_WAITS
            if (kt == 0) wst[0] = __builtin_readcyclecounter(); else if (kt == 1) wst[2] = __builtin_readcyclecounter();
#endif
#endif
            if (go2) { issue_b(1, kc2, b); wait_vmcnt<6>(); }
            else wait_vmcnt<0>();
#ifdef ARX_STAMP
#ifdef ARX_STAMP_WAITS
            if (kt == 0) wst[1] = __builtin_readcyclecounter(); else if (kt == 1) wst[3] = __builtin_readcyclecounter();
#endif
#endif
            ML::bar();
            quad(1, 0, wf0);
            if (go1 || wr == 0) ML::bar();
        }
        if (has_next && wr == 0) ML::bar();
#ifdef ARX_STAMP
        const unsigned long long pts1 = __builtin_readcyclecounter();
#endif
        pol.epilogue(acc, m0, n0, wr, wc, lane, smem + ML::STAGE_OFF + sbuf * EpiStage::BYTES);
        if (has_next && wr == 1) ML::bar();
#ifdef ARX_STAMP
        pol.stamp(orig, tid, pts0, pts1, wst, smem + ML::KT_STAMP_OFF);
#endif
        if (!has_next) break;
        orig = onext; m0 = m0n; n0 = n0n; ko = kon; sbuf ^= 1;
    }
}

template <int MODE, int KROT>
struct EncoderTilePolicy {
    static constexpr bool REBASE_W = false;
    static constexpr bool PERMUTE_B = true;
    TileWalk walk;
    const EpiParams& ep;
    int M, N, nk;
    __device__ __forceinline__ bool tile(int o, int& m0, int& n0, int& ko) const {
        int tm = 0, tn = 0;
        const bool ok = walk.coords(o, tm, tn);
        m0 = tm * 256; n0 = tn * 256; ko = (tn * KROT) % nk;
        return ok;
    }
    __device__ __forceinline__ void stage_issue(int m0, int n0, char* stage, int wid, int lane) const {
        epi_stage_issue<MODE>(ep, m0, n0, stage, wid, lane, N);
    }
    __device__ __forceinline__ void epilogue(const f32x4 (&acc)[4][8], int m0, int n0, int wr, int wc, int lane, const char* stage) const {
        epilogue_store_v3<MODE, (MODE == EPI_RESID_STATS || MODE == EPI_LNRESID_STATS) ? 4 : 8>(acc, ep, m0, n0, wr, wc, lane, M, N, stage);
    }
#ifdef ARX_STAMP
    __device__ __forceinline__ void stamp(int orig, int tid, unsigned long long pts0, unsigned long long pts1, const unsigned long long (&wst)[4], const char* kts) const {
        if (ep.stamps && (tid == 0 || tid == 256)) {
            unsigned long long* o = ep.stamps + ((size_t)orig * 2 + (tid >> 8)) * 32;
            o[0] = pts0; o[1] = pts1; o[2] = __builtin_readcyclecounter(); o[3] = pts0;
            o[4] = wst[0]; o[5] = wst[1]; o[6] = wst[2]; o[7] = wst[3];
#pragma unroll 1
            for (int k = 0; k < 16; ++k) o[8 + k] = *reinterpret_cast<const volatile unsigned long long*>(kts + (tid >> 8) * 128 + k * 8);
        }
    }
#endif
};

template <int MODE, int KROT = 0>
__global__ __launch_bounds__(512) void gemm_8phase_persistent_kernel(const bf16_t* __restrict__ A, int64_t lda,
                                                                      const bf16_t* __restrict__ W, int64_t ldw,
                                                                      int M, int N, int K, int tiles_m, int tiles_n, EpiParams ep) {
    extern __shared__ __attribute__((aligned(16))) char smem[];
#ifdef ARX_DEV_VARIANTS
    const TileWalk walk(tiles_m, tiles_n, K, ep.dev_bw);
#else
    const TileWalk walk(tiles_m, tiles_n, K);
#endif
    const EncoderTilePolicy<MODE, KROT> pol{walk, ep, M, N, K >> 6};
#ifdef ARX_DEV_VARIANTS
    if (ep.dev_stagger > 0) {
        const long long wait = (long long)((blockIdx.x >> 3) % ep.dev_slots) * ep.dev_stagger, t0 = clock64();
        while (clock64() - t0 < wait) __builtin_amdgcn_s_sleep(16);
    }
#endif
    gemm8_persistent_body<bf16_t>(A, lda, W, ldw, M, N, K, pol, smem);
}
```

arxiv_rag_amd/encoder.py:

```python
from __future__ import annotations

import ctypes as C
from typing import Dict, List, Optional, Sequence, Union

import numpy as np
import torch

from . import _lib
from .config import ARCH_MPNET, EncoderConfig
from .weights import layer_keys


def _dev_ptr(t: Optional[torch.Tensor]) -> Optional[int]:
    return None if t is None else t.data_ptr()


class HipEncoder:

    def __init__(self, cfg: EncoderConfig, state_dict: Dict[str, np.ndarray], device: Union[str, torch.device] = "cuda:0",
                 max_tokens: int = 32 * 512, max_seqs: int = 32, *, gemm_schedule: int = _lib.GEMM_DEFAULT,
                 attn_kernel: int = _lib.ATTN_TRANSPOSED, ln_fold: bool = True):
        self.lib = _lib.load()
        if not torch.cuda.is_available():
            raise _lib.ArxError("no HIP device visible: the encoder has no CPU path")
        self.cfg = cfg
        self.gemm_schedule, self.attn_kernel, self.ln_fold = int(gemm_schedule), int(attn_kernel), bool(ln_fold)
        self.device = torch.device(device)
        torch.cuda.set_device(self.device)
        self._w: List[torch.Tensor] = []
        self._handle = C.c_void_p(None)
        self._cap = (0, 0)
        self._upload(state_dict)
        self._ensure_capacity(max_tokens, max_seqs)

    def _f32(self, a: np.ndarray) -> torch.Tensor:
        t = torch.from_numpy(np.ascontiguousarray(a, dtype=np.float32)).to(self.device)
        self._w.append(t)
        return t

    def _bf16(self, a: np.ndarray) -> torch.Tensor:
        src = torch.from_numpy(np.ascontiguousarray(a, dtype=np.float32)).to(self.device)
        dst = torch.empty(src.shape, dtype=torch.bfloat16, device=self.device)
        _lib.check(self.lib.arx_f32_to_bf16(src.data_ptr(), dst.data_ptr(), src.numel(),
                                            torch.cuda.current_stream().cuda_stream), "arx_f32_to_bf16")
        self._w.append(dst)
        return dst

    def _upload(self, sd: Dict[str, np.ndarray]):
        cfg = self.cfg
        self._layers_c = (_lib.LayerWeightsC * cfg.layers)()
        for i in range(cfg.layers):
            k = layer_keys(cfg, i)
            wqkv = np.concatenate([sd[k["q"] + ".weight"], sd[k["k"] + ".weight"], sd[k["v"] + ".weight"]], 0)
            bqkv = np.concatenate([sd[k["q"] + ".bias"], sd[k["k"] + ".bias"], sd[k["v"] + ".bias"]], 0)
            L = self._layers_c[i]
            L.w_qkv = self._bf16(wqkv).data_ptr(); L.b_qkv = self._f32(bqkv).data_ptr()
            L.w_o = self._bf16(sd[k["o"] + ".weight"]).data_ptr(); L.b_o = self._f32(sd[k["o"] + ".bias"]).data_ptr()
            L.ln1_g = self._f32(sd[k["ln1"] + ".weight"]).data_ptr(); L.ln1_b = self._f32(sd[k["ln1"] + ".bias"]).data_ptr()
            L.w_fc1 = self._bf16(sd[k["fc1"] + ".weight"]).data_ptr(); L.b_fc1 = self._f32(sd[k["fc1"] + ".bias"]).data_ptr()
            L.w_fc2 = self._bf16(sd[k["fc2"] + ".weight"]).data_ptr(); L.b_fc2 = self._f32(sd[k["fc2"] + ".bias"]).data_ptr()
            L.ln2_g = self._f32(sd[k["ln2"] + ".weight"]).data_ptr(); L.ln2_b = self._f32(sd[k["ln2"] + ".bias"]).data_ptr()
        w = _lib.EncoderWeightsC()
        w.word_emb = self._f32(sd["embeddings.word_embeddings.weight"]).data_ptr()
        w.pos_emb = self._f32(sd["embeddings.position_embeddings.weight"]).data_ptr()
        w.emb_ln_g = self._f32(sd["embeddings.LayerNorm.weight"]).data_ptr()
        w.emb_ln_b = self._f32(sd["embeddings.LayerNorm.bias"]).data_ptr()
        if cfg.arch == ARCH_MPNET:
            w.type_emb = None
            w.rel_bias = self._f32(sd["encoder.relative_attention_bias.weight"]).data_ptr()
        else:
            w.type_emb = self._f32(sd["embeddings.token_type_embeddings.weight"][0]).data_ptr()
            w.rel_bias = None
        w.layers = C.cast(self._layers_c, C.POINTER(_lib.LayerWeightsC))
        self._weights_c = w
        c = _lib.EncoderConfigC(cfg.arch, cfg.vocab_size, cfg.hidden, cfg.layers, cfg.heads, cfg.ffn, cfg.max_pos,
                                cfg.pool, cfg.pad_id, cfg.rel_buckets, cfg.rel_max_distance, cfg.ln_eps)
        self._cfg_c = c
        torch.cuda.synchronize(self.device)

    def _ensure_capacity(self, max_tokens: int, max_seqs: int):
        if max_tokens <= self._cap[0] and max_seqs <= self._cap[1]:
            return
        max_tokens = max(max_tokens, self._cap[0]); max_seqs = max(max_seqs, self._cap[1])
        self.close()
        h = C.c_void_p(None)
        opt = _lib.EncoderOptionsC(gemm_schedule=self.gemm_schedule, attn_kernel=self.attn_kernel,
                                   flags=0 if self.ln_fold else _lib.ENC_EXPLICIT_LAYERNORM)
        _lib.check(self.lib.arx_encoder_create_opt(C.byref(self._cfg_c), C.byref(self._weights_c), max_tokens, max_seqs,
                                                   C.byref(opt), C.byref(h)), "arx_encoder_create_opt")
        self._handle = h
        self._cap = (max_tokens, max_seqs)
        self._low_latency = False

    def close(self):
        if getattr(self, "_handle", None) is not None and self._handle.value:
            torch.cuda.synchronize(self.device)
            self.lib.arx_encoder_destroy(self._handle)
            self._handle = C.c_void_p(None)
            self._cap = (0, 0)

    def __del__(self):
        try:
            self.close()
        except Exception:
            pass

    def forward_tokens(self, ids: torch.Tensor, lens: torch.Tensor, max_len: int, total_tokens: int,
                       out: Optional[torch.Tensor] = None, out_f16: Optional[torch.Tensor] = None,
                       normalize: bool = True, low_latency: bool = False) -> Optional[torch.Tensor]:
        B, S = ids.shape
        assert ids.dtype == torch.int32 and lens.dtype == torch.int32 and ids.is_contiguous() and lens.is_contiguous()
        self._ensure_capacity(total_tokens, B)
        if bool(low_latency) != self._low_latency:
            _lib.check(self.lib.arx_encoder_set_low_latency(self._handle, 1 if low_latency else 0), "arx_encoder_set_low_latency")
            self._low_latency = bool(low_latency)
        if out is None and out_f16 is None:
            out = torch.empty((B, self.cfg.hidden), dtype=torch.float32, device=self.device)
        rc = self.lib.arx_encoder_forward(
            self._handle, ids.data_ptr(), S, lens.data_ptr(), B, max_len, total_tokens,
            _dev_ptr(out), 0 if out is None else out.stride(0),
            _dev_ptr(out_f16), 0 if out_f16 is None else out_f16.stride(0),
            1 if normalize else 0, torch.cuda.current_stream().cuda_stream)
        _lib.check(rc, "arx_encoder_forward")
        return out

    def encode_tokens(self, ids: np.ndarray, lens: np.ndarray, normalize: bool = True, low_latency: bool = False) -> torch.Tensor:
        ids = np.ascontiguousarray(ids, dtype=np.int32)
        lens = np.ascontiguousarray(lens, dtype=np.int32)
        if ids.shape[0] == 0:
            return torch.empty((0, self.cfg.hidden), dtype=torch.float32, device=self.device)
        max_len = max(int(lens.max()), 1)
        total = max(int(lens.sum()), 1)
        d_ids = torch.from_numpy(ids).to(self.device, non_blocking=True)
        d_lens = torch.from_numpy(lens).to(self.device, non_blocking=True)
        return self.forward_tokens(d_ids, d_lens, max_len, total, normalize=normalize, low_latency=low_latency)

    @staticmethod
    def _pad_batch(seqs: Sequence[Sequence[int]], idx: Sequence[int], pad_id: int):
        lens = np.fromiter((len(seqs[i]) for i in idx), np.int32, len(idx))
        S = max(int(lens.max()) if len(idx) else 1, 1)
        ids = np.full((len(idx), S), pad_id, np.int32)
        tot = int(lens.sum())
        if tot:
            flat = np.concatenate([np.asarray(seqs[i], np.int32) for i in idx if len(seqs[i])])
            rows = np.repeat(np.arange(len(idx)), lens)
            starts = np.cumsum(lens) - lens
            cols = np.arange(tot) - np.repeat(starts, lens)
            ids[rows, cols] = flat
        return ids, lens

    def encode_ragged(self, seqs: Sequence[Sequence[int]], batch_size: int = 256, normalize: bool = True,
                      on_device: bool = False, out_f16: Optional[torch.Tensor] = None, low_latency: bool = False):
        n = len(seqs)
        if n == 0:
            return (torch.zeros((0, self.cfg.hidden), dtype=torch.float32, device=self.device) if on_device
                    else np.zeros((0, self.cfg.hidden), np.float32))
        order = sorted(range(n), key=lambda i: -len(seqs[i]))
        dev_out = torch.empty((n, self.cfg.hidden), dtype=torch.float32, device=self.device)
        dev16 = self._f16_stage(n, out_f16)
        for s0 in range(0, n, batch_size):
            idx = order[s0:s0 + batch_size]
            ids, lens = self._pad_batch(seqs, idx, self.cfg.pad_id)
            d_ids = torch.from_numpy(ids).to(self.device, non_blocking=True)
            d_lens = torch.from_numpy(lens).to(self.device, non_blocking=True)
            self.forward_tokens(d_ids, d_lens, ids.shape[1], max(int(lens.sum()), 1), out=dev_out[s0:s0 + len(idx)],
                                out_f16=None if dev16 is None else dev16[s0:s0 + len(idx)], normalize=normalize,
                                low_latency=low_latency)
        order_t = torch.as_tensor(order, device=self.device) if (on_device or dev16 is not None) else None
        if dev16 is not None:
# ... 137 lines not shown
```

include/arx.h:

```cpp
#ifndef ARX_H
#define ARX_H

#include <stdint.h>

#ifdef __cplusplus
extern "C" {
#endif

#define ARX_VERSION 112

#define ARX_OK            0
#define ARX_ERR_ARG      -1
#define ARX_ERR_HIP      -2
#define ARX_ERR_CAPACITY -3

#define ARX_ARCH_MPNET 0
#define ARX_ARCH_BERT  1
#define ARX_POOL_MEAN  0
#define ARX_POOL_CLS   1

typedef struct {
    int32_t arch;
    int32_t vocab_size;
    int32_t hidden;
    int32_t layers;
    int32_t heads;
    int32_t ffn;
    int32_t max_pos;
    int32_t pool;
    int32_t pad_id;
    int32_t rel_buckets;
    int32_t rel_max_distance;
    float   ln_eps;
} arx_encoder_config;

typedef struct {
    const void*  w_qkv;
    const float* b_qkv;
    const void*  w_o;
    const float* b_o;
    const float* ln1_g; const float* ln1_b;
    const void*  w_fc1;
    const float* b_fc1;
    const void*  w_fc2;
    const float* b_fc2;
    const float* ln2_g; const float* ln2_b;
} arx_layer_weights;

typedef struct {
    const float* word_emb;
    const float* pos_emb;
    const float* type_emb;
    const float* emb_ln_g; const float* emb_ln_b;
    const float* rel_bias;
    const arx_layer_weights* layers;
} arx_encoder_weights;

typedef struct arx_encoder arx_encoder;

int32_t     arx_version(void);
const char* arx_last_error(void);

int32_t arx_mpnet_bucket(int32_t relative_position, int32_t num_buckets, int32_t max_distance);

int64_t arx_encoder_workspace_bytes(const arx_encoder_config* cfg, int32_t max_tokens, int32_t max_seqs);

int32_t arx_encoder_create(const arx_encoder_config* cfg, const arx_encoder_weights* w,
                           int32_t max_tokens, int32_t max_seqs, arx_encoder** out);
void    arx_encoder_destroy(arx_encoder* h);

#define ARX_GEMM_DEFAULT    89
#define ARX_GEMM_PER_TILE    8
#define ARX_GEMM_PERSISTENT  9
#define ARX_GEMM_2STAGE     13
#define ARX_GEMM_SPLIT_K    70
#define ARX_GEMM_TILE_128   71
#define ARX_ATTN_TRANSPOSED  1
#define ARX_ATTN_RING        2
#define ARX_ATTN_RING16      4
#define ARX_ATTN_STAGED      8
#define ARX_ENC_EXPLICIT_LAYERNORM 1
typedef struct {
    int32_t struct_bytes;
    int32_t gemm_schedule;
    int32_t attn_kernel;
    int32_t flags;
} arx_encoder_options;
int32_t arx_encoder_create_opt(const arx_encoder_config* cfg, const arx_encoder_weights* w, int32_t max_tokens, int32_t max_seqs,
                               const arx_encoder_options* opt, arx_encoder** out);

int32_t arx_encoder_forward(arx_encoder* h, const int32_t* ids, int32_t seq_stride,
                            const int32_t* lens, int32_t n_seqs, int32_t max_len, int32_t total_tokens,
                            float* out_f32, int64_t out_stride,
                            void* out_f16, int64_t out16_stride,
                            int32_t normalize, void* stream);

int32_t arx_encoder_attention(arx_encoder* h, const void* qkv, const int32_t* lens, int32_t n_seqs, int32_t max_len,
                              void* ctx, void* stream);

int32_t arx_encoder_debug_hidden(arx_encoder* h, int32_t layer_slot, float* dst, int32_t n_tokens, void* stream);

int32_t arx_encoder_set_low_latency(arx_encoder* h, int32_t on);

int32_t arx_encoder_set_tap(arx_encoder* h, int32_t layer);

typedef struct {
    int32_t struct_bytes;
    int32_t n_labels;
    const float* type_emb;
    const float* pooler_w; const float* pooler_b;
    const float* cls_w;    const float* cls_b;
} arx_pair_head;

int32_t arx_encoder_set_pair_head(arx_encoder* h, const arx_pair_head* head);
int32_t arx_encoder_score_pairs(arx_encoder* h, const int32_t* ids, int32_t seq_stride, const int32_t* lens, const int32_t* seg_b,
                                int32_t n_seqs, int32_t max_len, int32_t total_tokens, float* out_logits, int64_t out_stride,
                                void* stream);
int32_t arx_encoder_debug_cls(arx_encoder* h, float* dst, int32_t n, void* stream);
int32_t arx_pair_head_forward(const float* cls_rows, int64_t ld, int32_t n, int32_t hidden, const arx_pair_head* head,
                              float* out_logits, int64_t out_stride, void* stream);

int32_t arx_build_info(void);

int64_t arx_topk_workspace_bytes(int64_t n_rows, int32_t n_queries, int32_t dim, int32_t k);
int32_t arx_topk_search(const void* corpus, int64_t n_rows, const void* queries, int32_t n_queries,
                        int32_t dim, int32_t k, float* out_scores, int64_t* out_ids, int64_t idx_base,
                        void* ws, int64_t ws_bytes, void* stream);

int64_t arx_topk_i8_index_bytes(int64_t n_rows, int32_t dim);
int64_t arx_topk_workspace_bytes_i8(int64_t n_rows, int32_t n_queries, int32_t dim, int32_t k);
int32_t arx_topk_build_i8(const void* corpus, int64_t n_rows, int32_t dim, void* index_i8, void* stream);
int32_t arx_topk_i8_index_info(const void* index_i8, int64_t n_rows, int32_t dim, float* host_out, void* stream);
int32_t arx_topk_search_i8(const void* corpus, const void* index_i8, int64_t n_rows, const void* queries, int32_t n_queries,
                           int32_t dim, int32_t k, float* out_scores, int64_t* out_ids, int64_t idx_base,
                           void* ws, int64_t ws_bytes, void* stream);

#define ARX_TOPK_NO_PERSISTENT 1
#define ARX_TOPK_NO_SINGLE_ROW_TAIL 8
#define ARX_TOPK_I8_CENTRE_QUERY 16
#define ARX_TOPK_SCAN_ONLY     2
#define ARX_TOPK_TAIL_ONLY     4
typedef struct {
    int32_t struct_bytes;
    int32_t i8_max_queries;
    float   max_row_norm;
    int32_t cu_limit;
    int32_t flags;
    float   debug_tau_mult;
    int32_t debug_drop_best;
} arx_topk_options;
int32_t arx_topk_search_opt(const void* corpus, const void* index_i8, int64_t n_rows, const void* queries, int32_t n_queries,
                            int32_t dim, int32_t k, float* out_scores, int64_t* out_ids, int64_t idx_base,
                            void* ws, int64_t ws_bytes, const arx_topk_options* opt, void* stream);

int32_t arx_rows_max_norm_f16(const void* rows, int64_t n_rows, int32_t dim, float* out_max, void* stream);

int32_t arx_topk_stats(const void* ws, int64_t* flagged_queries, int64_t* extra_groups, void* stream);

int32_t arx_stream_create_cu_mask(const uint32_t* cu_mask, int32_t n_words, void** out);
int32_t arx_stream_destroy(void* stream);
int32_t arx_device_cu_count(void);
int32_t arx_debug_cu_census(uint32_t* out, int32_t n_blocks, int32_t spin_cycles, void* stream);

int32_t arx_topk_merge(const float* scores, const int64_t* ids, int32_t n_parts, int32_t n_queries,
                       int32_t k, float* out_scores, int64_t* out_ids, void* stream);

int64_t arx_topk_filtered_workspace_bytes(int64_t n_rows, int32_t n_queries, int32_t dim, int32_t k);
int32_t arx_topk_search_filtered(const void* corpus, int64_t n_rows, const uint64_t* allow, int64_t n_allowed, const void* queries,
                                 int32_t n_queries, int32_t dim, int32_t k, float* out_scores, int64_t* out_ids, int64_t idx_base,
// ... 23 lines not shown
                                     void* ws, int64_t ws_bytes, int32_t path, int32_t cand_cap, void* stream);
int32_t arx_topk_prefix_stats(const void* ws, int64_t* overflowed_queries, int64_t* candidate_groups, void* stream);

int64_t arx_topk_grouped_workspace_bytes(int64_t n_rows, int32_t n_queries, int32_t dim, int32_t n_groups, int32_t chunks_per_group);
int32_t arx_topk_search_grouped(const void* corpus, int64_t n_rows, const int32_t* group_of, int64_t max_run_rows, const uint64_t* allow,
                                int64_t n_allowed, const void* queries, int32_t n_queries, int32_t dim, int32_t n_groups,
                                int32_t chunks_per_group, float* out_scores, int64_t* out_ids, int32_t* out_groups, int64_t idx_base,
                                float max_row_norm, void* ws, int64_t ws_bytes, void* stream);
int32_t arx_topk_search_grouped_tuned(const void* corpus, int64_t n_rows, const int32_t* group_of, int64_t max_run_rows,
                                      const uint64_t* allow, int64_t n_allowed, const void* queries, int32_t n_queries, int32_t dim,
                                      int32_t n_groups, int32_t chunks_per_group, float* out_scores, int64_t* out_ids, int32_t* out_groups,
                                      int64_t idx_base, float max_row_norm, void* ws, int64_t ws_bytes, int32_t path, int32_t cand_cap,
                                      void* stream);
int32_t arx_topk_grouped_stats(const void* ws, int64_t* overflowed_queries, int64_t* candidate_groups, void* stream);
int32_t arx_group_runs_info(const int32_t* group_of, int64_t n_rows, int64_t* out, void* stream);

int64_t arx_range_workspace_bytes(int64_t n_rows, int32_t n_queries, int32_t dim, int32_t max_results);
int32_t arx_range_search(const void* corpus, int64_t n_rows, const uint64_t* allow, int64_t n_allowed, const void* queries,
                         const float* min_score, int32_t n_queries, int32_t dim, int32_t max_results, float* out_scores, int64_t* out_ids,
                         int32_t* out_counts, int64_t idx_base, float max_row_norm, void* ws, int64_t ws_bytes, void* stream);
int32_t arx_range_search_tuned(const void* corpus, int64_t n_rows, const uint64_t* allow, int64_t n_allowed, const void* queries,
                               const float* min_score, int32_t n_queries, int32_t dim, int32_t max_results, float* out_scores,
                               int64_t* out_ids, int32_t* out_counts, int64_t idx_base, float max_row_norm, void* ws, int64_t ws_bytes,
                               int32_t path, int32_t cand_cap, void* stream);
int32_t arx_range_stats(const void* ws, int64_t* overflowed_queries, int64_t* candidate_groups, void* stream);

int32_t arx_text_contains(const uint8_t* blob, const int64_t* row_off, int64_t n_rows,
                          const uint8_t* pat_blob, const int32_t* pat_off, int32_t n_pat,
                          uint64_t* out_bits, void* stream);
int32_t arx_bitmap_count(const uint64_t* bits, int64_t n_rows, int64_t* out_count, void* stream);

typedef struct {
    double  operand;
    int32_t column;
    int32_t want_kind;
    int32_t op;
    int32_t negate;
    int32_t set_off;
    int32_t set_len;
} arx_where_leaf;
int32_t arx_where_eval(const int64_t* col_table, int32_t n_cols, int64_t n_rows,
                       const arx_where_leaf* leaves, const int32_t* leaf_off,
                       const int32_t* tokens, const int32_t* token_off,
                       const double* set_vals, int64_t n_set_vals, int32_t n_filters,
                       const uint64_t* and_with, int64_t and_stride,
                       uint64_t* out_bits, int64_t* out_counts, void* stream);

int32_t arx_gather_rows(const void* shard, int64_t n_rows, int32_t dim, int64_t idx_base, const int64_t* ids, int64_t count,
                        void* out, void* stream);
int32_t arx_mmr_select(const void* q, const void* cand, const int64_t* ids, int32_t n_queries, int32_t n, int32_t dim, int32_t m,
                       float lambda, int32_t* order, float* mmr, void* stream);

int64_t arx_bm25_workspace_bytes(int64_t n_rows, int32_t n_queries, int32_t n);
int32_t arx_bm25_search(const int64_t* term_ptr, const uint32_t* post_row, const float* post_w, int32_t vocab, int64_t n_rows,
                        const int32_t* q_terms, const int32_t* q_nterms, int32_t n_queries, int32_t n, float* out_scores,
                        int64_t* out_ids, int64_t idx_base, void* ws, int64_t ws_bytes, void* stream);
int32_t arx_bm25_search_tuned(const int64_t* term_ptr, const uint32_t* post_row, const float* post_w, int32_t vocab, int64_t n_rows,
                              const int32_t* q_terms, const int32_t* q_nterms, int32_t n_queries, int32_t n, float* out_scores,
                              int64_t* out_ids, int64_t idx_base, void* ws, int64_t ws_bytes, int32_t tile_rows, int32_t max_blocks,
                              void* stream);
int32_t arx_bm25_scores(const int64_t* term_ptr, const uint32_t* post_row, const float* post_w, int32_t vocab, int64_t n_rows,
                        const int32_t* q_terms, int32_t n_terms, int64_t row_lo, int64_t row_hi, int32_t tile_rows, float* out,
                        void* stream);

int32_t arx_gemm_bf16(const void* A, const void* W, const float* bias, const void* resid, void* C,
                      int32_t M, int32_t N, int32_t K, int32_t mode, int32_t variant, void* stream);

typedef struct {
    int32_t struct_bytes;
    int32_t mode;
    int32_t variant;
    float eps;
    const float* bias;
    const void* resid;
    const float *a_mean, *a_rstd;
    const float* s_vec;
    const float *r_mean, *r_rstd;
    const float *r_gamma, *r_beta;
    int64_t row_cap;
    float *part_sum, *part_sq;
    int64_t part_ld;
    float *out_mean, *out_rstd;
    const int32_t* n_rows;
} arx_gemm_epilogue;
int32_t arx_gemm_bf16_ex(const void* A, const void* W, void* C, int32_t M, int32_t N, int32_t K, const arx_gemm_epilogue* e, void* stream);

int32_t arx_fold_ln(const void* W, const float* gamma, const float* beta, const float* bias, void* Wf, float* s, float* c,
                    int32_t N, int32_t K, void* stream);

int32_t arx_adjacent_cosine(const float* emb, int64_t ld, int32_t n, int32_t dim, float* out, void* stream);

int32_t arx_wp_create(const char* vocab_blob, const int64_t* vocab_off , int32_t n_vocab, int32_t unk_id,
                      int32_t bos_id, int32_t eos_id, int32_t pad_id, int32_t lowercase, int32_t max_chars_per_word,
                      const char* trigger_blob, const int64_t* trigger_off , int32_t n_triggers, void** out);
void arx_wp_destroy(void* tokenizer);
int32_t arx_wp_encode(void* tokenizer, const char* text_blob, const int64_t* text_off , int64_t n, int32_t max_len,
                      int32_t* ids, int32_t* lens, uint8_t* fallback, int32_t n_threads);
int32_t arx_wp_miss_count(void* tokenizer, int64_t* n_strings, int64_t* n_bytes);
int32_t arx_wp_miss_fetch(void* tokenizer, char* blob, int64_t* off );
int32_t arx_wp_cache_add(void* tokenizer, const char* seg_blob, const int64_t* seg_off , int64_t n, const int32_t* ids,
                         const int64_t* ids_off );
int64_t arx_wp_cache_size(void* tokenizer);
int32_t arx_wp_version(void);

int32_t arx_f32_to_bf16(const float* src, void* dst, int64_t n, void* stream);
int32_t arx_fill_unit_rows_f16(void* dst, int64_t n_rows, int32_t dim, uint64_t seed, void* stream);
int32_t arx_fill_unit_rows_f16_at(void* dst, int64_t n_rows, int32_t dim, uint64_t seed, int64_t row_base, void* stream);
int32_t arx_fill_clustered_rows_f16_at(void* dst, int64_t n_rows, int32_t dim, uint64_t seed, int64_t row_base, int32_t n_clusters,
                                       float spread, int32_t n_hot_dims, float hot_gain, void* stream);

#define ARX_K_SEARCH_GROUPMAX 0
#define ARX_K_GEMM_QKV        1
#define ARX_K_GEMM_OPROJ      2
#define ARX_K_GEMM_FC1        3
#define ARX_K_GEMM_FC2        4
#define ARX_K_ATTENTION       5
#define ARX_K_LAYERNORM       6
#define ARX_K_EMBED           7
#define ARX_K_POOL            8
#define ARX_K_SEARCH_SELECT   9
#define ARX_K_SEARCH_RESCORE 10
#define ARX_K_GEMM_RAW       11
#define ARX_K_CLASSES        12
int32_t arx_prof_enable(int32_t on);
int32_t arx_prof_classes(uint32_t mask);
int32_t arx_prof_reset(void);
int32_t arx_prof_read(int32_t kernel_class, float* total_ms, int32_t* launches);

#ifdef __cplusplus
}
#endif
#endif
```

Baseline: 22110.

## Fuse LayerNorm statistics finalize into consumer GEMM prologue via per-tile partials

Residual-statistics GEMMs now reduce row sums and squares across the four column waves in LDS and write one partial per 256-wide n-tile, replacing the finer 64-column partials. The following LN-folded GEMM (QKV or FC1) combines those partials in its epilogue to get mean and rstd, so the separate ln_finalize launches between layers are skipped except after the last layer. This removes two small kernel launches per layer and shrinks the partial slabs. In exchange it adds an LDS reduction buffer and a barrier to the stats epilogues, and repeats the finalize work in every consumer tile.

Result: no change. 21930 (-0.8%).

```diff
diff --git a/arxiv_rag_amd/_lib.py b/arxiv_rag_amd/_lib.py
--- a/arxiv_rag_amd/_lib.py
+++ b/arxiv_rag_amd/_lib.py
@@ -36,7 +36,8 @@
 
 
 class EncoderOptionsC(C.Structure):
-    _fields_ = [("struct_bytes", C.c_int32), ("gemm_schedule", C.c_int32), ("attn_kernel", C.c_int32), ("flags", C.c_int32)]
+    _fields_ = [("struct_bytes", C.c_int32), ("gemm_schedule", C.c_int32), ("attn_kernel", C.c_int32), ("flags", C.c_int32),
+                ("ln_stats", C.c_int32)]
 
     def __init__(self, **kw):
         super().__init__(**kw)
@@ -56,7 +57,8 @@
     _fields_ = [("struct_bytes", C.c_int32), ("mode", C.c_int32), ("variant", C.c_int32), ("eps", C.c_float)] \
                + [(n, C.c_void_p) for n in ("bias", "resid", "a_mean", "a_rstd", "s_vec", "r_mean", "r_rstd", "r_gamma", "r_beta")] \
                + [("row_cap", C.c_int64), ("part_sum", C.c_void_p), ("part_sq", C.c_void_p), ("part_ld", C.c_int64),
-                  ("out_mean", C.c_void_p), ("out_rstd", C.c_void_p), ("n_rows", C.c_void_p)]
+                  ("out_mean", C.c_void_p), ("out_rstd", C.c_void_p), ("n_rows", C.c_void_p),
+                  ("tile_sum", C.c_void_p), ("tile_sq", C.c_void_p), ("a_parts", C.c_int32), ("reserved", C.c_int32)]
 
     def __init__(self, **kw):
         super().__init__(**kw)
@@ -67,6 +69,7 @@
 GEMM_DEFAULT, GEMM_PER_TILE, GEMM_PERSISTENT, GEMM_2STAGE, GEMM_SPLIT_K, GEMM_TILE_128 = 89, 8, 9, 13, 70, 71
 ATTN_TRANSPOSED, ATTN_RING, ATTN_RING16, ATTN_STAGED = 1, 2, 4, 8
 ENC_EXPLICIT_LAYERNORM = 1
+LN_STATS_FUSED, LN_STATS_LAUNCH = 1, 2
 
 
 EXPORTS = {
diff --git a/arxiv_rag_amd/csrc/arx_common.h b/arxiv_rag_amd/csrc/arx_common.h
--- a/arxiv_rag_amd/csrc/arx_common.h
+++ b/arxiv_rag_amd/csrc/arx_common.h
@@ -72,6 +72,14 @@
     return v;
 }
 
+template <typename Load>
+__device__ __forceinline__ void ln_stats_finish(int np, Load&& load, float inv_h, float eps, float& mean, float& rstd) {
+    float s = 0.f, q = 0.f;
+    for (int t = 0; t < np; ++t) { float a, b; load(t, a, b); s += a; q += b; }
+    mean = s * inv_h;
+    rstd = rsqrtf(fmaxf(fmaf(q, inv_h, -(mean * mean)), 0.f) + eps);
+}
+
 __device__ __forceinline__ int xcd_remap(int bid, int nwg) {
     const int q = nwg >> 3, r = nwg & 7, xcd = bid & 7, idx = bid >> 3;
     const int base = (xcd < r) ? xcd * (q + 1) : r * (q + 1) + (xcd - r) * q;
diff --git a/arxiv_rag_amd/csrc/encoder.hip b/arxiv_rag_amd/csrc/encoder.hip
--- a/arxiv_rag_amd/csrc/encoder.hip
+++ b/arxiv_rag_amd/csrc/encoder.hip
@@ -41,6 +41,7 @@
     std::vector<float*> s_qkv, c_qkv, s_fc1, c_fc1;
     float *st1_sum = nullptr, *st1_sq = nullptr, *st2_sum = nullptr, *st2_sq = nullptr;
     float *part_s = nullptr, *part_q = nullptr;
+    int ln_stats_launch = 0;
     int variant = ARX_GEMM_DEFAULT;
     int low_latency = 0;
     float* small_ws = nullptr;
@@ -104,6 +105,8 @@
 #endif
     ARX_REQUIRE(gemm_ok, "arx_encoder_options.gemm_schedule=%d is not a whole-forward GEMM schedule of this build (ARX_GEMM_* in arx.h)", g);
     ARX_REQUIRE(attn_ok, "arx_encoder_options.attn_kernel=%d is not an attention kernel of this build (ARX_ATTN_* in arx.h)", a);
+    ARX_REQUIRE(o->ln_stats == 0 || o->ln_stats == ARX_LN_STATS_FUSED || o->ln_stats == ARX_LN_STATS_LAUNCH,
+                "arx_encoder_options.ln_stats=%d is not a statistics schedule (ARX_LN_STATS_* in arx.h)", o->ln_stats);
     ARX_REQUIRE((o->flags & ~ARX_ENC_EXPLICIT_LAYERNORM) == 0, "arx_encoder_options.flags=0x%x has unknown bits", o->flags);
     return ARX_OK;
 }
@@ -145,6 +148,7 @@
     if (opt && opt->gemm_schedule) h->variant = opt->gemm_schedule;
     if (opt && opt->attn_kernel) h->attn_variant = opt->attn_kernel;
     h->ln_fold = !(opt && (opt->flags & ARX_ENC_EXPLICIT_LAYERNORM));
+    h->ln_stats_launch = opt && opt->ln_stats == ARX_LN_STATS_LAUNCH;
     const WsLayout l = ws_layout(*cfg, max_tokens, max_seqs);
     hipError_t he = hipMalloc((void**)&h->ws, l.total);
     if (he != hipSuccess) {
@@ -270,6 +274,11 @@
     return M * lda < (1ll << 31) && N * ldw < (1ll << 31) && M * ep.ldc < (1ll << 32) && (!ep.resid || M * ep.ldr < (1ll << 32));
 }
 
+static bool gemm_on_256_tiles(int variant, int64_t M, int64_t lda, int64_t N, int64_t ldw, const EpiParams& ep) {
+    return (variant == ARX_GEMM_DEFAULT || variant == ARX_GEMM_PER_TILE || variant == ARX_GEMM_PERSISTENT) && N % 128 == 0 && N >= 256 &&
+           fits_u32_offsets(M, lda, N, ldw, ep);
+}
+
 template <int MODE>
 int arx_launch_gemm(int variant, const uint16_t* A, int64_t lda, const uint16_t* W, int64_t ldw, int M, int N, int K,
                     const EpiParams& ep, hipStream_t st) {
@@ -277,6 +286,15 @@
         arx_set_error("gemm: K=%d must be a multiple of 64 and N=%d of 8", K, N);
         return ARX_ERR_ARG;
     }
+    constexpr bool STATS = (MODE == EPI_RESID_STATS || MODE == EPI_LNRESID_STATS);
+    if (gemm_on_256_tiles(variant, M, lda, N, ldw, ep)) {
+        ARX_REQUIRE(!STATS || (ep.t_sum && ep.t_sq), "gemm mode %d on a 256-wide kernel needs the per-n-tile statistics slabs", MODE);
+        ARX_REQUIRE(ep.a_parts == 0 || (ep.a_parts <= EpiStage::MAX_PARTS && ep.ap_sum && ep.ap_sq && ep.fin_mean && ep.fin_rstd),
+                    "gemm mode %d: a_parts=%d needs 1..%d partial slabs and the mean / rstd outputs", MODE, ep.a_parts, (int)EpiStage::MAX_PARTS);
+    } else {
+        ARX_REQUIRE(ep.a_parts == 0 && !ep.t_sum, "gemm M=%d N=%d K=%d variant %d: per-n-tile statistics need a 256-wide 4-phase kernel", M, N, K, variant);
+    }
+    constexpr int smem8 = Gemm8Phase<bf16_t, 0>::smem_bytes(MODE);
     const bool wide = (N % 256 == 0);
     const bool wide8 = (N % 128 == 0 && N >= 256);
 #ifdef ARX_DEV_VARIANTS
@@ -305,20 +323,20 @@
     }
     if (variant == ARX_GEMM_PERSISTENT && wide8) {
         auto kern = gemm_8phase_persistent_kernel<MODE>;
-        ARX_HIP_CHECK(arx_func_smem((const void*)kern, Gemm8Phase<bf16_t, 0>::SMEM_BYTES));
+        ARX_HIP_CHECK(arx_func_smem((const void*)kern, smem8));
         const int n_cu = arx_device_cus();
         const int tm = cdiv(M, 256), tn = cdiv(N, 256);
         int grid = TileWalk::grid(tm, tn) < n_cu ? TileWalk::grid(tm, tn) : n_cu;
         grid = grid / 8 * 8 > 0 ? grid / 8 * 8 : grid;
-        kern<<<grid, 512, Gemm8Phase<bf16_t, 0>::SMEM_BYTES, st>>>((const bf16_t*)A, lda, (const bf16_t*)W, ldw, M, N, K, tm, tn, ep);
+        kern<<<grid, 512, smem8, st>>>((const bf16_t*)A, lda, (const bf16_t*)W, ldw, M, N, K, tm, tn, ep);
         ARX_HIP_CHECK(hipGetLastError());
         return ARX_OK;
     }
     if (variant == ARX_GEMM_PER_TILE && wide8) {
         auto kern = gemm_8phase_kernel<MODE>;
-        ARX_HIP_CHECK(arx_func_smem((const void*)kern, Gemm8Phase<bf16_t, 0>::SMEM_BYTES));
+        ARX_HIP_CHECK(arx_func_smem((const void*)kern, smem8));
         const int tm = cdiv(M, 256), tn = cdiv(N, 256);
-        kern<<<TileWalk::grid(tm, tn), 512, Gemm8Phase<bf16_t, 0>::SMEM_BYTES, st>>>((const bf16_t*)A, lda, (const bf16_t*)W, ldw, M, N, K, tm, tn, ep);
+        kern<<<TileWalk::grid(tm, tn), 512, smem8, st>>>((const bf16_t*)A, lda, (const bf16_t*)W, ldw, M, N, K, tm, tn, ep);
         ARX_HIP_CHECK(hipGetLastError());
         return ARX_OK;
     }
@@ -548,6 +566,9 @@
                                float eps, float* mean, float* rstd, hipStream_t st) {
     const int grid = cdiv(T, 256);
     switch (nparts) {
+    case 2: ln_finalize_kernel<2><<<grid, 256, 0, st>>>(ps, pq, ld, nparts, n_rows, inv_h, eps, mean, rstd); break;
+    case 3: ln_finalize_kernel<3><<<grid, 256, 0, st>>>(ps, pq, ld, nparts, n_rows, inv_h, eps, mean, rstd); break;
+    case 4: ln_finalize_kernel<4><<<grid, 256, 0, st>>>(ps, pq, ld, nparts, n_rows, inv_h, eps, mean, rstd); break;
     case 6: ln_finalize_kernel<6><<<grid, 256, 0, st>>>(ps, pq, ld, nparts, n_rows, inv_h, eps, mean, rstd); break;
     case 12: ln_finalize_kernel<12><<<grid, 256, 0, st>>>(ps, pq, ld, nparts, n_rows, inv_h, eps, mean, rstd); break;
     case 16: ln_finalize_kernel<16><<<grid, 256, 0, st>>>(ps, pq, ld, nparts, n_rows, inv_h, eps, mean, rstd); break;
@@ -565,6 +586,20 @@
         ARX_HIP_CHECK(hipMallocAsync((void**)&ws, ARX_SMALL_WS_BYTES, st));
         rc = launch_gemm<MODE>(ARX_K_GEMM_RAW, variant, A, K, W, K, M, N, K, ep, st, ws);
         (void)hipFreeAsync(ws, st);
+        return rc;
+    }
+    if (STATS && gemm_on_256_tiles(variant, M, K, N, K, ep)) {
+        const int np = cdiv(N, 256);
+        EpiParams e2 = ep;
+        float* ws = nullptr;
+        if (!e2.t_sum) {
+            ARX_HIP_CHECK(hipMallocAsync((void**)&ws, (size_t)2 * np * e->part_ld * sizeof(float), st));
+            e2.t_sum = ws; e2.t_sq = ws + (int64_t)np * e->part_ld;
+        }
+        rc = launch_gemm<MODE>(ARX_K_GEMM_RAW, variant, A, K, W, K, M, N, K, e2, st);
+        if (rc == ARX_OK) launch_ln_finalize(M, np, e2.t_sum, e2.t_sq, e->part_ld, e->n_rows, ep.inv_h, ep.eps, e->out_mean, e->out_rstd, st);
+        if (ws) (void)hipFreeAsync(ws, st);
+        if (rc == ARX_OK) ARX_HIP_CHECK(hipGetLastError());
         return rc;
     }
     if ((rc = launch_gemm<MODE>(ARX_K_GEMM_RAW, variant, A, K, W, K, M, N, K, ep, st)) != ARX_OK) return rc;
@@ -591,9 +626,16 @@
     const bool staged = (variant == ARX_GEMM_DEFAULT || variant == ARX_GEMM_PER_TILE || variant == ARX_GEMM_PERSISTENT);
     ARX_REQUIRE(e->bias, "mode %d needs bias", mode);
     ARX_REQUIRE(!(mode == EPI_BIAS_RESID || stats) || e->resid, "mode %d needs resid", mode);
-    ARX_REQUIRE(!ln_in || (e->a_mean && e->a_rstd && e->s_vec), "mode %d needs a_mean, a_rstd and s_vec", mode);
+    const bool fused_in = ln_in && e->a_parts != 0;
+    ARX_REQUIRE(!ln_in || (((e->a_mean && e->a_rstd) || fused_in) && e->s_vec), "mode %d needs a_mean, a_rstd and s_vec", mode);
+    if (fused_in)
+        ARX_REQUIRE(e->a_parts == cdiv(K, 256) && e->a_parts <= EpiStage::MAX_PARTS && e->tile_sum && e->tile_sq && e->out_mean && e->out_rstd &&
+                        e->part_ld >= round_up64(M, 256),
+                    "mode %d with a_parts=%d needs a_parts == ceil(K / 256) <= %d, tile_sum, tile_sq, out_mean, out_rstd and part_ld >= M rounded up to 256",
+                    mode, e->a_parts, (int)EpiStage::MAX_PARTS);
+    ARX_REQUIRE(ln_in || e->a_parts == 0, "a_parts is an option of modes 3 and 4");
     ARX_REQUIRE(mode != EPI_LNRESID_STATS || (e->r_mean && e->r_rstd && e->r_gamma && e->r_beta), "mode 6 needs r_mean, r_rstd, r_gamma and r_beta");
-    if (ln_in || mode == EPI_LNRESID_STATS)
+    if ((ln_in && !fused_in) || mode == EPI_LNRESID_STATS)
         ARX_REQUIRE(e->row_cap >= (staged ? round_up64(M, 256) : (int64_t)M),
                     "row_cap=%lld: the row vectors must be readable up to row %lld (M=%d%s)", (long long)e->row_cap,
                     (long long)(staged ? round_up64(M, 256) : (int64_t)M), M, staged ? " rounded up to 256: variants 89, 8, 9 stage whole tiles" : "");
@@ -612,7 +654,10 @@
     ep.r_sum = e->r_mean; ep.r_sq = e->r_rstd; ep.r_gamma = e->r_gamma; ep.r_beta = e->r_beta;
     ep.o_sum = e->part_sum; ep.o_sq = e->part_sq; ep.o_ld = e->part_ld;
     ep.fin_mean = e->out_mean; ep.fin_rstd = e->out_rstd;
-    ep.inv_h = 1.0f / (float)N; ep.eps = e->eps;
+    ep.inv_h = 1.0f / (float)(ln_in ? K : N); ep.eps = e->eps;
+    if (stats) { ep.t_sum = e->tile_sum; ep.t_sq = e->tile_sq; }
+    if (fused_in) { ep.ap_sum = e->tile_sum; ep.ap_sq = e->tile_sq; ep.ap_ld = e->part_ld; ep.a_parts = e->a_parts; }
+    else if (ln_in) { ep.fin_mean = nullptr; ep.fin_rstd = nullptr; }
     hipStream_t st = (hipStream_t)stream;
     const uint16_t* a = (const uint16_t*)A; const uint16_t* w = (const uint16_t*)W;
     switch (mode) {
@@ -709,6 +754,19 @@
 
     const float inv_h = 1.0f / (float)H;
     const int gv = !h->low_latency ? h->variant : (T <= ARX_SMALL_M ? ARX_GEMM_SPLIT_K : (T <= ARX_MEDIUM_M ? ARX_GEMM_TILE_128 : h->variant));
+    bool tile_stats;
+    {
+        const EpiParams e1{h->qkv, 3 * (int64_t)H, nullptr, nullptr, 0}, e2{h->x1, H, nullptr, h->x, H}, e3{h->hbuf, F, nullptr, nullptr, 0};
+        tile_stats = gemm_on_256_tiles(gv, T, H, 3 * H, H, e1) && gemm_on_256_tiles(gv, T, H, H, H, e2) && gemm_on_256_tiles(gv, T, H, F, H, e3) &&
+                     gemm_on_256_tiles(gv, T, F, H, F, e2);
+    }
+    const bool fused = tile_stats && !h->ln_stats_launch;
+    const int n_parts = tile_stats ? cdiv(H, 256) : H / 64;
+    auto producer_stats = [&](EpiParams& e) { (tile_stats ? e.t_sum : e.o_sum) = h->part_s; (tile_stats ? e.t_sq : e.o_sq) = h->part_q; e.o_ld = tp; };
+    auto consumer_stats = [&](EpiParams& e, float* mean, float* rstd) {
+        if (fused) { e.ap_sum = h->part_s; e.ap_sq = h->part_q; e.ap_ld = tp; e.a_parts = n_parts; e.fin_mean = mean; e.fin_rstd = rstd; }
+        else { e.a_sum = mean; e.a_sq = rstd; }
+    };
     if (h->tap_layer == 0 && h->tap) ARX_HIP_CHECK(hipMemcpyAsync(h->tap, h->x, (int64_t)T * H * 2, hipMemcpyDeviceToDevice, st));
     for (int li = 0; li < c.layers; ++li) {
         const arx_layer_weights& L = h->layers[li];
@@ -718,12 +776,12 @@
             if ((rc = launch_gemm<EPI_BIAS>(ARX_K_GEMM_QKV, gv, h->x, H, (const uint16_t*)L.w_qkv, H, T, 3 * H, H, ep, st, h->small_ws)) != ARX_OK) return rc;
         } else {
             ep = EpiParams{h->qkv, 3 * (int64_t)H, h->c_qkv[li], nullptr, 0};
-            ep.a_sum = h->st2_sum; ep.a_sq = h->st2_sq; ep.s_vec = h->s_qkv[li]; ep.inv_h = inv_h; ep.eps = c.ln_eps;
+            consumer_stats(ep, h->st2_sum, h->st2_sq); ep.s_vec = h->s_qkv[li]; ep.inv_h = inv_h; ep.eps = c.ln_eps;
             if ((rc = launch_gemm<EPI_LN_BIAS>(ARX_K_GEMM_QKV, gv, h->x, H, h->wqkv_f[li], H, T, 3 * H, H, ep, st, h->small_ws)) != ARX_OK) return rc;
         }
         if ((rc = launch_attn(h, n_seqs, max_len, st)) != ARX_OK) return rc;
         ep = EpiParams{h->x1, H, L.b_o, h->x, H};
-        ep.o_sum = h->part_s; ep.o_sq = h->part_q; ep.o_ld = tp; ep.inv_h = inv_h; ep.eps = c.ln_eps;
+        producer_stats(ep); ep.inv_h = inv_h; ep.eps = c.ln_eps;
         ep.fin_mean = h->st1_sum; ep.fin_rstd = h->st1_sq;
         if (li == 0) {
             if ((rc = launch_gemm<EPI_RESID_STATS>(ARX_K_GEMM_OPROJ, gv, h->ctx, H, (const uint16_t*)L.w_o, H, T, H, H, ep, st, h->small_ws)) != ARX_OK) return rc;
@@ -732,19 +790,19 @@
             ep.r_sum = h->st2_sum; ep.r_sq = h->st2_sq; ep.r_gamma = P.ln2_g; ep.r_beta = P.ln2_b;
             if ((rc = launch_gemm<EPI_LNRESID_STATS>(ARX_K_GEMM_OPROJ, gv, h->ctx, H, (const uint16_t*)L.w_o, H, T, H, H, ep, st, h->small_ws)) != ARX_OK) return rc;
         }
-        if (gv != ARX_GEMM_SPLIT_K) { ProfScope ps(ARX_K_LAYERNORM, st);
-          launch_ln_finalize(T, H / 64, h->part_s, h->part_q, tp, h->cu + n_seqs, inv_h, c.ln_eps, h->st1_sum, h->st1_sq, st); }
+        if (gv != ARX_GEMM_SPLIT_K && !fused) { ProfScope ps(ARX_K_LAYERNORM, st);
+          launch_ln_finalize(T, n_parts, h->part_s, h->part_q, tp, h->cu + n_seqs, inv_h, c.ln_eps, h->st1_sum, h->st1_sq, st); }
         ARX_HIP_CHECK(hipGetLastError());
         ep = EpiParams{h->hbuf, F, h->c_fc1[li], nullptr, 0};
-        ep.a_sum = h->st1_sum; ep.a_sq = h->st1_sq; ep.s_vec = h->s_fc1[li]; ep.inv_h = inv_h; ep.eps = c.ln_eps;
+        consumer_stats(ep, h->st1_sum, h->st1_sq); ep.s_vec = h->s_fc1[li]; ep.inv_h = inv_h; ep.eps = c.ln_eps;
         if ((rc = launch_gemm<EPI_LN_BIAS_GELU>(ARX_K_GEMM_FC1, gv, h->x1, H, h->wfc1_f[li], H, T, F, H, ep, st, h->small_ws)) != ARX_OK) return rc;
         ep = EpiParams{h->x, H, L.b_fc2, h->x1, H};
         ep.r_sum = h->st1_sum; ep.r_sq = h->st1_sq; ep.r_gamma = L.ln1_g; ep.r_beta = L.ln1_b;
-        ep.o_sum = h->part_s; ep.o_sq = h->part_q; ep.o_ld = tp; ep.inv_h = inv_h; ep.eps = c.ln_eps;
+        producer_stats(ep); ep.inv_h = inv_h; ep.eps = c.ln_eps;
         ep.fin_mean = h->st2_sum; ep.fin_rstd = h->st2_sq;
         if ((rc = launch_gemm<EPI_LNRESID_STATS>(ARX_K_GEMM_FC2, gv, h->hbuf, F, (const uint16_t*)L.w_fc2, F, T, H, F, ep, st, h->small_ws)) != ARX_OK) return rc;
-        if (gv != ARX_GEMM_SPLIT_K) { ProfScope ps(ARX_K_LAYERNORM, st);
-          launch_ln_finalize(T, H / 64, h->part_s, h->part_q, tp, h->cu + n_seqs, inv_h, c.ln_eps, h->st2_sum, h->st2_sq, st); }
+        if (gv != ARX_GEMM_SPLIT_K && (!fused || li == c.layers - 1)) { ProfScope ps(ARX_K_LAYERNORM, st);
+          launch_ln_finalize(T, n_parts, h->part_s, h->part_q, tp, h->cu + n_seqs, inv_h, c.ln_eps, h->st2_sum, h->st2_sq, st); }
         ARX_HIP_CHECK(hipGetLastError());
         if (h->tap_layer == li + 1 && h->tap) {
             layernorm_kernel<<<ln_grid, 256, 0, st>>>(h->x, h->tap, L.ln2_g, L.ln2_b, h->cu + n_seqs, H, c.ln_eps);
diff --git a/arxiv_rag_amd/csrc/encoder_kernels.h b/arxiv_rag_amd/csrc/encoder_kernels.h
--- a/arxiv_rag_amd/csrc/encoder_kernels.h
+++ b/arxiv_rag_amd/csrc/encoder_kernels.h
@@ -1312,19 +1312,17 @@
                                                            float* __restrict__ mean, float* __restrict__ rstd) {
     const int m = blockIdx.x * 256 + threadIdx.x;
     if (m >= *n_rows_ptr) return;
-    float s = 0.f, q = 0.f;
+    float mu, rs;
     if constexpr (NP > 0) {
         float vs[NP], vq[NP];
 #pragma unroll
         for (int p = 0; p < NP; ++p) { vs[p] = ps[p * ld + m]; vq[p] = pq[p * ld + m]; }
-#pragma unroll
-        for (int p = 0; p < NP; ++p) { s += vs[p]; q += vq[p]; }
+        ln_stats_finish(NP, [&](int p, float& a, float& b) { a = vs[p]; b = vq[p]; }, inv_h, eps, mu, rs);
     } else {
-        for (int p = 0; p < nparts; ++p) { s += ps[p * ld + m]; q += pq[p * ld + m]; }
-    }
-    const float mu = s * inv_h;
+        ln_stats_finish(nparts, [&](int p, float& a, float& b) { a = ps[p * ld + m]; b = pq[p * ld + m]; }, inv_h, eps, mu, rs);
+    }
     mean[m] = mu;
-    rstd[m] = rsqrtf(fmaxf(q * inv_h - mu * mu, 0.f) + eps);
+    rstd[m] = rs;
 }
 
 __global__ __launch_bounds__(256) void fold_ln_kernel(const uint16_t* __restrict__ W, const float* __restrict__ gamma,
diff --git a/arxiv_rag_amd/csrc/epi3.h b/arxiv_rag_amd/csrc/epi3.h
--- a/arxiv_rag_amd/csrc/epi3.h
+++ b/arxiv_rag_amd/csrc/epi3.h
@@ -2,20 +2,28 @@
 #include "gemm.h"
 
 struct EpiStage {
-    enum { BIAS = 0, SVEC = 1, RGAMMA = 2, RBETA = 3, AMEAN = 4, ARSTD = 5, RMEAN = 6, RRSTD = 7, BYTES = 8 * 1024 };
+    enum { BIAS = 0, SVEC = 1, RGAMMA = 2, RBETA = 3, AMEAN = 4, ARSTD = 5, RMEAN = 6, RRSTD = 7, MAX_PARTS = 4, BYTES = 12 * 1024 };
+    static __device__ __forceinline__ constexpr int part_slot(int k) { return k < 2 ? 2 + k : 4 + k; }
 };
+struct EpiReduce { enum { BYTES = 4 * 256 * 8 }; };
 
 template <int MODE>
 __device__ __forceinline__ void epi_stage_issue(const EpiParams& p, int m0, int n0, char* stage, int wid, int lane, int N) {
     constexpr bool LN_IN = (MODE == EPI_LN_BIAS || MODE == EPI_LN_BIAS_GELU);
     constexpr bool LNR = (MODE == EPI_LNRESID_STATS);
     const int w = wid;
+    int slot = w;
     const float* src = nullptr;
     if (w == EpiStage::BIAS) src = p.bias + n0;
     if constexpr (LN_IN) {
         if (w == EpiStage::SVEC) src = p.s_vec + n0;
-        if (w == EpiStage::AMEAN) src = p.a_sum + m0;
-        if (w == EpiStage::ARSTD) src = p.a_sq + m0;
+        if (p.a_parts > 0) {
+            const int k = w - 2;
+            if (k >= 0 && k < 2 * p.a_parts) { src = ((k & 1) ? p.ap_sq : p.ap_sum) + (int64_t)(k >> 1) * p.ap_ld + m0; slot = EpiStage::part_slot(k); }
+        } else {
+            if (w == EpiStage::AMEAN) src = p.a_sum + m0;
+            if (w == EpiStage::ARSTD) src = p.a_sq + m0;
+        }
     }
     if constexpr (LNR) {
         if (w == EpiStage::RGAMMA) src = p.r_gamma + n0;
@@ -25,8 +33,14 @@
     }
     unsigned l = __builtin_amdgcn_mbcnt_hi(~0u, __builtin_amdgcn_mbcnt_lo(~0u, 0u));
     (void)lane;
-    if (w < EpiStage::AMEAN && n0 + 256 > N) l &= 31;
-    if (src) __builtin_amdgcn_global_load_lds((gbl_void_t*)(src + l * 4), (lds_void_t*)(stage + w * 1024), 16, 0, 0);
+    const unsigned l_row = l;
+    const bool col_vec = w < EpiStage::SVEC + 1 || (w < EpiStage::AMEAN && !(LN_IN && p.a_parts > 0));
+    if (col_vec && n0 + 256 > N) l &= 31;
+    if (src) __builtin_amdgcn_global_load_lds((gbl_void_t*)(src + l * 4), (lds_void_t*)(stage + slot * 1024), 16, 0, 0);
+    if constexpr (LN_IN) {
+        if (p.a_parts == EpiStage::MAX_PARTS && w < 2)
+            __builtin_amdgcn_global_load_lds((gbl_void_t*)((w ? p.ap_sq : p.ap_sum) + 3 * p.ap_ld + m0 + l_row * 4), (lds_void_t*)(stage + EpiStage::part_slot(6 + w) * 1024), 16, 0, 0);
+    }
 }
 
 template <int MODE> struct EpiFullLine {
@@ -46,7 +60,7 @@
 
 template <int MODE, bool CHECK, int DEPTH>
 __device__ __forceinline__ void epilogue_store_v3_impl(const f32x4 (&acc)[4][8], const EpiParams& p, int m0, int n0, int wr, int wc,
-                                                       int lane, int M, const char* stage) {
+                                                       int lane, int M, const char* stage, char* red) {
     constexpr int NI = 4, MI = 8, NS = (NI / 2) * MI;
     constexpr bool LN_IN = (MODE == EPI_LN_BIAS || MODE == EPI_LN_BIAS_GELU);
     constexpr bool STATS = (MODE == EPI_RESID_STATS || MODE == EPI_LNRESID_STATS);
@@ -178,9 +192,12 @@
                 float a = st_s, b = st_q;
                 a += __shfl_xor(a, 16); a += __shfl_xor(a, 32);
                 b += __shfl_xor(b, 16); b += __shfl_xor(b, 32);
-                const int m = m_base + i * 16 + mq;
-                const int64_t part = n_base >> 6;
-                if (q == 0 && m < M) { p.o_sum[part * p.o_ld + m] = a; p.o_sq[part * p.o_ld + m] = b; }
+                if (q == 0) {
+                    *reinterpret_cast<f32x2*>(red + (wc * 256 + wr * 128 + i * 16 + mq) * 8) = f32x2{a, b};
+                    const int m = m_base + i * 16 + mq;
+                    const int64_t part = n_base >> 6;
+                    if (p.o_sum && m < M) { p.o_sum[part * p.o_ld + m] = a; p.o_sq[part * p.o_ld + m] = b; }
+                }
                 st_s = 0.f; st_q = 0.f;
             }
         }
@@ -189,11 +206,45 @@
 
 template <int MODE, int DEPTH = 8>
 __device__ __forceinline__ void epilogue_store_v3(const f32x4 (&acc)[4][8], const EpiParams& p, int m0, int n0, int wr, int wc,
-                                                  int lane, int M, int N, const char* stage) {
-    if (n0 + wc * 64 >= N) return;
-    if (m0 + wr * 128 + 128 <= M) epilogue_store_v3_impl<MODE, false, DEPTH>(acc, p, m0, n0, wr, wc, lane, M, stage);
+                                                  int lane, int M, int N, const char* stage, char* red = nullptr) {
+    constexpr bool STATS = (MODE == EPI_RESID_STATS || MODE == EPI_LNRESID_STATS);
+    if constexpr (MODE == EPI_LN_BIAS || MODE == EPI_LN_BIAS_GELU) {
+        if (p.a_parts > 0 && n0 + wc * 64 < N) {
+            float* sfw = reinterpret_cast<float*>(const_cast<char*>(stage));
+#pragma unroll
+            for (int h = 0; h < 2; ++h) {
+                const int rb = wr * 128 + h * 64 + lane;
+                float mu, rs;
+                ln_stats_finish(p.a_parts, [&](int k, float& a, float& b) { a = sfw[EpiStage::part_slot(2 * k) * 256 + rb]; b = sfw[EpiStage::part_slot(2 * k + 1) * 256 + rb]; },
+                                p.inv_h, p.eps, mu, rs);
+                sfw[EpiStage::AMEAN * 256 + rb] = mu; sfw[EpiStage::ARSTD * 256 + rb] = rs;
+                if (n0 == 0 && wc == 0 && m0 + rb < M) { p.fin_mean[m0 + rb] = mu; p.fin_rstd[m0 + rb] = rs; }
+            }
+            asm volatile("s_waitcnt lgkmcnt(0)" ::: "memory");
+        }
+    }
+    if (n0 + wc * 64 >= N) {
+        if constexpr (!STATS) return;
+        else {
+            *reinterpret_cast<f32x2*>(red + (wc * 256 + wr * 128 + lane) * 8) = f32x2{0.f, 0.f};
+            *reinterpret_cast<f32x2*>(red + (wc * 256 + wr * 128 + 64 + lane) * 8) = f32x2{0.f, 0.f};
+        }
+    } else if (m0 + wr * 128 + 128 <= M) epilogue_store_v3_impl<MODE, false, DEPTH>(acc, p, m0, n0, wr, wc, lane, M, stage, red);
     else {
-        epilogue_store_v3_impl<MODE, true, DEPTH>(acc, p, m0, n0, wr, wc, lane, M, stage);
+        epilogue_store_v3_impl<MODE, true, DEPTH>(acc, p, m0, n0, wr, wc, lane, M, stage, red);
         __builtin_amdgcn_s_waitcnt(0x0F70);
     }
+    if constexpr (STATS) {
+        asm volatile("s_waitcnt lgkmcnt(0)" ::: "memory");
+        __builtin_amdgcn_s_barrier();
+        asm volatile("" ::: "memory");
+        if (wr == 0) {
+            const int r = wc * 64 + lane, m = m0 + r;
+            const f32x2 v0 = *reinterpret_cast<const f32x2*>(red + r * 8), v1 = *reinterpret_cast<const f32x2*>(red + (256 + r) * 8);
+            const f32x2 v2 = *reinterpret_cast<const f32x2*>(red + (512 + r) * 8), v3 = *reinterpret_cast<const f32x2*>(red + (768 + r) * 8);
+            const float a = ((v0.x + v1.x) + v2.x) + v3.x, b = ((v0.y + v1.y) + v2.y) + v3.y;
+            const int64_t o = (int64_t)(n0 >> 8) * p.o_ld + m;
+            if (m < M) { p.t_sum[o] = a; p.t_sq[o] = b; }
+        }
+    }
 }
diff --git a/arxiv_rag_amd/csrc/gemm.h b/arxiv_rag_amd/csrc/gemm.h
--- a/arxiv_rag_amd/csrc/gemm.h
+++ b/arxiv_rag_amd/csrc/gemm.h
@@ -187,6 +187,12 @@
     float* o_sum = nullptr;
     float* o_sq = nullptr;
     int64_t o_ld = 0;
+    float* t_sum = nullptr;
+    float* t_sq = nullptr;
+    const float* ap_sum = nullptr;
+    const float* ap_sq = nullptr;
+    int64_t ap_ld = 0;
+    int a_parts = 0;
     float inv_h = 0.f, eps = 0.f;
     float* fin_mean = nullptr;
     float* fin_rstd = nullptr;
@@ -199,8 +205,6 @@
     unsigned long long* stamps = nullptr;
 #endif
 };
-
-
 
 template <int MODE, int NI, int MI>
 __device__ __forceinline__ void epilogue_store(const f32x4 (&acc)[NI][MI], const EpiParams& p, int m_base, int n_base,
diff --git a/arxiv_rag_amd/csrc/gemm8.h b/arxiv_rag_amd/csrc/gemm8.h
--- a/arxiv_rag_amd/csrc/gemm8.h
+++ b/arxiv_rag_amd/csrc/gemm8.h
@@ -44,6 +44,10 @@
 #else
     static constexpr int SMEM_BYTES = STAGE_OFF + 2 * EpiStage::BYTES;
 #endif
+    static constexpr int RED_OFF = SMEM_BYTES;
+    static constexpr int SMEM_BYTES_STATS = SMEM_BYTES + EpiReduce::BYTES;
+    static_assert(SMEM_BYTES_STATS <= 160 * 1024, "one CU's LDS");
+    static constexpr int smem_bytes(int mode) { return (mode == EPI_RESID_STATS || mode == EPI_LNRESID_STATS) ? SMEM_BYTES_STATS : SMEM_BYTES; }
     using vec = typename Mfma<T>::vec;
 
     static __device__ __forceinline__ void fence() { asm volatile("" ::: "memory"); }
@@ -209,7 +213,7 @@
 #ifdef ARX_STAMP
     const unsigned long long ts2 = __builtin_readcyclecounter();
 #endif
-    epilogue_store_v3<MODE>(acc, ep, m0, n0, wid >> 2, wid & 3, lane, M, N, smem + ML::STAGE_OFF);
+    epilogue_store_v3<MODE>(acc, ep, m0, n0, wid >> 2, wid & 3, lane, M, N, smem + ML::STAGE_OFF, smem + ML::RED_OFF);
 #ifdef ARX_STAMP
     const unsigned long long ts3 = __builtin_readcyclecounter();
     asm volatile("s_waitcnt vmcnt(0)" ::: "memory");
@@ -419,6 +423,7 @@
     TileWalk walk;
     const EpiParams& ep;
     int M, N, nk;
+    char* red;
     __device__ __forceinline__ bool tile(int o, int& m0, int& n0, int& ko) const {
         int tm = 0, tn = 0;
         const bool ok = walk.coords(o, tm, tn);
@@ -429,7 +434,7 @@
         epi_stage_issue<MODE>(ep, m0, n0, stage, wid, lane, N);
     }
     __device__ __forceinline__ void epilogue(const f32x4 (&acc)[4][8], int m0, int n0, int wr, int wc, int lane, const char* stage) const {
-        epilogue_store_v3<MODE, (MODE == EPI_RESID_STATS || MODE == EPI_LNRESID_STATS) ? 4 : 8>(acc, ep, m0, n0, wr, wc, lane, M, N, stage);
+        epilogue_store_v3<MODE, (MODE == EPI_RESID_STATS || MODE == EPI_LNRESID_STATS) ? 4 : 8>(acc, ep, m0, n0, wr, wc, lane, M, N, stage, red);
     }
 #ifdef ARX_STAMP
     __device__ __forceinline__ void stamp(int orig, int tid, unsigned long long pts0, unsigned long long pts1, const unsigned long long (&wst)[4], const char* kts) const {
@@ -454,7 +459,7 @@
 #else
     const TileWalk walk(tiles_m, tiles_n, K);
 #endif
-    const EncoderTilePolicy<MODE, KROT> pol{walk, ep, M, N, K >> 6};
+    const EncoderTilePolicy<MODE, KROT> pol{walk, ep, M, N, K >> 6, smem + Gemm8Phase<bf16_t, 0>::RED_OFF};
 #ifdef ARX_DEV_VARIANTS
     if (ep.dev_stagger > 0) {
         const long long wait = (long long)((blockIdx.x >> 3) % ep.dev_slots) * ep.dev_stagger, t0 = clock64();
diff --git a/arxiv_rag_amd/encoder.py b/arxiv_rag_amd/encoder.py
--- a/arxiv_rag_amd/encoder.py
+++ b/arxiv_rag_amd/encoder.py
@@ -19,12 +19,13 @@
 
     def __init__(self, cfg: EncoderConfig, state_dict: Dict[str, np.ndarray], device: Union[str, torch.device] = "cuda:0",
                  max_tokens: int = 32 * 512, max_seqs: int = 32, *, gemm_schedule: int = _lib.GEMM_DEFAULT,
-                 attn_kernel: int = _lib.ATTN_TRANSPOSED, ln_fold: bool = True):
+                 attn_kernel: int = _lib.ATTN_TRANSPOSED, ln_fold: bool = True, ln_stats: int = _lib.LN_STATS_FUSED):
         self.lib = _lib.load()
         if not torch.cuda.is_available():
             raise _lib.ArxError("no HIP device visible: the encoder has no CPU path")
         self.cfg = cfg
         self.gemm_schedule, self.attn_kernel, self.ln_fold = int(gemm_schedule), int(attn_kernel), bool(ln_fold)
+        self.ln_stats = int(ln_stats)
         self.device = torch.device(device)
         torch.cuda.set_device(self.device)
         self._w: List[torch.Tensor] = []
@@ -84,7 +85,7 @@
         max_tokens = max(max_tokens, self._cap[0]); max_seqs = max(max_seqs, self._cap[1])
         self.close()
         h = C.c_void_p(None)
-        opt = _lib.EncoderOptionsC(gemm_schedule=self.gemm_schedule, attn_kernel=self.attn_kernel,
+        opt = _lib.EncoderOptionsC(gemm_schedule=self.gemm_schedule, attn_kernel=self.attn_kernel, ln_stats=self.ln_stats,
                                    flags=0 if self.ln_fold else _lib.ENC_EXPLICIT_LAYERNORM)
         _lib.check(self.lib.arx_encoder_create_opt(C.byref(self._cfg_c), C.byref(self._weights_c), max_tokens, max_seqs,
                                                    C.byref(opt), C.byref(h)), "arx_encoder_create_opt")
diff --git a/include/arx.h b/include/arx.h
--- a/include/arx.h
+++ b/include/arx.h
@@ -80,11 +80,14 @@
 #define ARX_ATTN_RING16      4
 #define ARX_ATTN_STAGED      8
 #define ARX_ENC_EXPLICIT_LAYERNORM 1
+#define ARX_LN_STATS_FUSED   1
+#define ARX_LN_STATS_LAUNCH  2
 typedef struct {
     int32_t struct_bytes;
     int32_t gemm_schedule;
     int32_t attn_kernel;
     int32_t flags;
+    int32_t ln_stats;
 } arx_encoder_options;
 int32_t arx_encoder_create_opt(const arx_encoder_config* cfg, const arx_encoder_weights* w, int32_t max_tokens, int32_t max_seqs,
                                const arx_encoder_options* opt, arx_encoder** out);
@@ -274,6 +277,9 @@
     int64_t part_ld;
     float *out_mean, *out_rstd;
     const int32_t* n_rows;
+    float *tile_sum, *tile_sq;
+    int32_t a_parts;
+    int32_t reserved;
 } arx_gemm_epilogue;
 int32_t arx_gemm_bf16_ex(const void* A, const void* W, void* C, int32_t M, int32_t N, int32_t K, const arx_gemm_epilogue* e, void* stream);
 
```
